# qiaozhijian/VCR-Net

Measured on AMD Instinct MI355X. Metric: point-cloud pairs/sec (N=1024, batch 16 per GPU), higher is better.
Workload: dtype f32; 1 GPU; BASELINE configs[1]: ModelNet40-like whole-to-whole registration, N=1024, batch=16 pairs per GPU, LPDNet(k=20)+Transformer+VcpTopK+SVD, iter=1, fp32; synthetic object clouds with the reference's transform recipe; LPD-pretrained emb_nn + seeded Transformer weights; num_points=1024, batch_per_gpu=16, global_batch=16, k=20, iters=1, parallelism=dp1 (pairs sharded per rank), entry_point=vcrnet_amd.module.vcrnetIter(net, src, tgt, iter) -> vcr_vcrnet_iter_f32

## Files before the change

### include/vcr_hip.h

```cpp
#ifndef VCR_HIP_H
#define VCR_HIP_H

#include <stddef.h>
#include <stdint.h>

#ifdef __cplusplus
extern "C" {
#endif

#define VCR_OK 0
#define VCR_EINVAL (-1)
#define VCR_EWORKSPACE (-2)
#define VCR_EUNSUPPORTED (-3)

typedef void* vcr_stream_t;

const char* vcr_strerror(int code);
#define VCR_ABI_VERSION 27
int vcr_abi_version(void);

typedef struct {
  const float* x_cf; int B, N;
  const float* w1; const float* b1;
  const float* w2; const float* b2;
  float* xyz4; float* feat64; float* sq64;
  const float* x_cf2; int B2;
  const float* pq_w; const float* pq_b; float* pq; int ldpq;
  float* feat64t;
} vcr_pointwise_args;
int vcr_pointwise_f32(const vcr_pointwise_args*, vcr_stream_t);

int vcr_rows4_f32(const float* x_cf, float* xyz4, int B, int N, vcr_stream_t);
int vcr_rows4_pq_f32(const float* x_cf, float* xyz4, int B, int N, const float* wpq, int ldw, const float* bpq, int C,
                     float* pq, int ldpq, vcr_stream_t);

typedef struct {
  uint32_t struct_bytes;
  const float* x; int ldx;
  const float* sq;
  int B, N, C, k;
  int32_t* idx;
  int32_t* tie_scratch; int tie_cap;
  int waves;
  int tie_zeroed;
  int tie_defer;
  void* tie_work; size_t tie_work_bytes;
  int tie_inline;
  const float* xt;
  const int32_t* perm; const float* xp; const float* sqp;
  const float* cen; const float* cen_sq; const float* cen_rad; const float* cen_sqmax;
  const int32_t* ord_ok;
} vcr_knn_args;

typedef struct {
  const float* xyz4;
  const float* feat_t; int ldf; const float* sq;
  int B, N;
  int32_t* perm; float* xyz4_p; float* cen4; float* cen4_rad; float* cen4_sqmax;
  float* feat_p; float* sq_p; float* cen64; float* cen64_sq; float* cen64_rad; float* cen64_sqmax;
  int32_t* ord_ok; float* ord_stat; float guard_ratio;
} vcr_knn_order_args;
int vcr_knn_order_f32(const vcr_knn_order_args*, vcr_stream_t);
int vcr_knn_f32(const vcr_knn_args*, vcr_stream_t);
size_t vcr_knn_tie_work_bytes(int N);
size_t vcr_knn_tie_slot_bytes(int B, int N);
int vcr_knn_ties_inline(const vcr_knn_args*);
int vcr_knn_ties_f32(const vcr_knn_args* a, const vcr_knn_args* b, vcr_stream_t);
int vcr_knn_pair_f32(const vcr_knn_args* a64, const vcr_knn_args* a3, vcr_stream_t);

typedef struct {
  const float* x; int ldx;
  const float* w;
  const float* bias;
  const float* residual; int ldr;
  float* y; int ldy;
  int M, N, K;
  int relu;
  const float* ln_stats_in; int ln_nseg; const float* ln_colsum; float ln_eps;
  float* stats_out;
  float* segmax_out; int ld_segmax; int seg_k;
  int variant;
} vcr_linear_args;
enum {
  VCR_LINEAR_REGSTAGE = 4, VCR_LINEAR_BK32 = 8, VCR_LINEAR_MFMA16 = 16, VCR_LINEAR_BK16 = 64, VCR_LINEAR_MFMA32 = 1024,
  VCR_LINEAR_ROWS96 = 2048, VCR_LINEAR_ROWS128 = 4096, VCR_LINEAR_ROWS64 = 8192, VCR_LINEAR_ROWS32 = 16384
};
int vcr_linear_f32(const vcr_linear_args*, vcr_stream_t);
int vcr_linear_config(const vcr_linear_args*);
int vcr_linear_pair_f32(const vcr_linear_args* a, const vcr_linear_args* b, vcr_stream_t);

int vcr_fold_layernorm_f32(const float* w, const float* bias, const float* ln_a, const float* ln_b, int N, int K,
                           float* w_out, float* colsum, float* bias_out, vcr_stream_t);

int vcr_split_bf16x3_f32(const float* x, void* planes, size_t n, vcr_stream_t);
int vcr_linear_bf16x3_f32(const vcr_linear_args*, const void* w_planes, vcr_stream_t);

typedef struct {
  const float* x; int ldx; const float* a; const float* b; float eps;
  const float* residual; int ldr;
  float* y; int ldy; int M, C;
  const float* xyz4; float* side4;
} vcr_layernorm_args;
int vcr_layernorm_f32(const vcr_layernorm_args*, vcr_stream_t);

typedef struct {
  const float* x; int ldx; int M, C; float scale; float* y; int ldy;
  const float* xyz4; float* side4;
} vcr_rowside_args;
int vcr_rowside_f32(const vcr_rowside_args*, vcr_stream_t);

typedef struct {
  const float* pq; int ldpq; const int32_t* idx; int k; int M; int n_per_cloud;
  const float* w2; const float* b2;
  float* x1; int ldx1; float* x2; int ldx2;
} vcr_edgeconv_args;
int vcr_edgeconv_f32(const vcr_edgeconv_args*, vcr_stream_t);
int vcr_edgeconv_bf16x3_f32(const vcr_edgeconv_args*, vcr_stream_t);

typedef struct {
  const float* pq; int ldpq; int C; const int32_t* idx; int k; int M; int n_per_cloud;
  float* y; int ldy;
  int variant;
  const int32_t* order;
} vcr_gathermax_args;
int vcr_gathermax_f32(const vcr_gathermax_args*, vcr_stream_t);

typedef struct {
  const float* pq; int ldpq; int C; const int32_t* idx; int k; int M; int n_per_cloud; float* h; int ldh;
  float* ymax; int ldymax; int zero_to;
} vcr_edgerows_args;
int vcr_edgerows_f32(const vcr_edgerows_args*, vcr_stream_t);
typedef struct {
  const float* pq; int ldpq; const int32_t* idx; int k; int M; int n_per_cloud;
  const float *w2, *b2, *w3, *b3, *w4, *b4;
  float* out; int ldo;
} vcr_edgechain_args;
int vcr_edgechain_f32(const vcr_edgechain_args*, vcr_stream_t);
typedef struct {
  const float* x; int ldx; int M, k, C; float* y; int ldy;
} vcr_segmax_args;
int vcr_segmax_f32(const vcr_segmax_args*, vcr_stream_t);

typedef struct {
  const float* q; int ldq; const float* k; int ldk; const float* v; int ldv;
  float* out; int ldo;
  int nbatch, heads, nq, nk; float scale; int kv_batch_shift;
  const uint8_t* key_keep; float* rowstat;
  float* score_out; int ld_score;
  int ngroups; long q_group_stride, k_group_stride, v_group_stride, out_group_stride;
  const int32_t* key_index; int nk_src;
  float* split_work; long split_work_floats;
  int variant;
  int plan_nbatch;
} vcr_sdpa_args;
#define VCR_SDPA_MAX_SPLIT 4
int vcr_sdpa_f32(const vcr_sdpa_args*, vcr_stream_t);
int vcr_sdpa_bf16x3_f32(const vcr_sdpa_args*, vcr_stream_t);

typedef struct {
  const float* score; int ld; int nbatch, heads, nq, nk;
  const float* rowstat; int q_batch_shift; float* mass;
} vcr_keymass_args;
int vcr_keymass_f32(const vcr_keymass_args*, vcr_stream_t);

typedef struct {
  const float* q; int ldq; const float* k; int ldk; const float* qside4; const float* kside4;
  float* corr4; int nbatch, nq, nk, E; int mode; float scale;
  float* split_work;
  long split_work_floats;
} vcr_softcorr_args;
int vcr_softcorr_f32(const vcr_softcorr_args*, vcr_stream_t);

typedef struct {
  const float* own; int ld_own; const float* str; int ld_str;
  const float* own_side4; const float* str_side4;
  int nbatch, n_own, n_str, E; int score; float scale; int str_batch_shift; int op;
  float* corr4; float* stat2; int32_t* argmax;
  const float* str_stat2; long str_stat_batch_stride; float* mass; int accumulate;
  float* score_out; int ld_score;
  int variant;
  float* split_work; long split_work_floats;
} vcr_pairscore_args;
#define VCR_PAIRSCORE_MAX_SPLIT 4
int vcr_pairscore_f32(const vcr_pairscore_args*, vcr_stream_t);

typedef struct {
  const float* score; int ld; int nbatch, n_rows, n_cols;
  const float* row_stat2; float* col_stat2; float* col_mass; float* row_mass;
} vcr_scoremass_args;
int vcr_scoremass_f32(const vcr_scoremass_args*, vcr_stream_t);

typedef struct {
  const float* values; int nbatch, n, K; int32_t* order; uint8_t* mask;
  int largest;
  int stride;
} vcr_rankselect_args;
int vcr_rankselect_f32(const vcr_rankselect_args*, vcr_stream_t);

typedef struct {
  const float* in; int ld_in; int n_in; const int32_t* idx; int nbatch, n_out, C; float* out; int ld_out;
  const int32_t* via; int n_via;
} vcr_gather_args;
int vcr_gather_rows_f32(const vcr_gather_args*, vcr_stream_t);

typedef struct {
  const float* src; int lds; const float* corr; int ldc; int B, K;
  float* R; float* t; float* R_ba; float* t_ba; float* H;
} vcr_rigid_svd_args;
int vcr_rigid_svd_f32(const vcr_rigid_svd_args*, vcr_stream_t);

typedef struct {
  const float* src4; const float* dst4; int B, N, M; int max_iterations; float tolerance;
  float* final4; float* R; float* t; float* R_ba; float* t_ba; int* iterations;
} vcr_icp_args;
size_t vcr_icp_workspace_bytes(int B, int N);
int vcr_icp_f32(const vcr_icp_args*, void* workspace, size_t workspace_bytes, vcr_stream_t);

typedef struct {
  const float* cloud; int P;
  const double* R_ab; const double* t_ab;
  const int32_t* pick; const int32_t* perm_src; const int32_t* perm_tgt;
  int B, N, keep;
  float* src_cf; float* tgt_cf;
} vcr_make_pairs_args;
int vcr_make_pairs_f32(const vcr_make_pairs_args*, vcr_stream_t);

typedef struct {
  uint32_t struct_bytes;
  const float* xyz_cf; long cloud_stride;
  int B, N, npoint;
  const int32_t* start;
  int32_t* idx;
  float* out_cf;
  int variant;
} vcr_fps_args;
int vcr_fps_f32(const vcr_fps_args*, vcr_stream_t);
int vcr_fps_form(const vcr_fps_args*, int* form, int* points_per_thread);

typedef struct {
  const float *ln_a, *ln_b;
} vcr_norm_w;
typedef struct {
  const float *wqkv, *bqkv;
  const float *wq, *bq, *wkv, *bkv;
  const float *wo, *bo;
} vcr_mha_w;
typedef struct {
  const float *w1, *b1, *w2, *b2;
} vcr_ffn_w;
typedef struct {
  uint32_t struct_bytes;
  const float *c1_w, *c1_b, *c2_w, *c2_b;
  const float *dg1_wpq, *dg1_bpq;
  const float *dg2_w, *dg2_b;
  const float *sn1_wpq, *sn1_bpq;
  const float *c3_w, *c3_b;
  vcr_norm_w enc_ln0, enc_ln1, enc_norm, dec_ln0, dec_ln1, dec_ln2, dec_norm;
  vcr_mha_w enc_self, dec_self, dec_cross;
  vcr_ffn_w enc_ffn, dec_ffn;
  int E, F, heads, k;
  int has_pointer;
  int head_mode;
  int linear_mode;
  struct {
    const void *dg1_pq, *sn1_pq, *c3, *enc_qkv, *enc_wo, *enc_ffn1, *enc_ffn2, *dec_qkv, *dec_self_wo, *dec_cross_q,
               *dec_cross_kv, *dec_cross_wo, *dec_ffn1, *dec_ffn2;
    const void* encdec_qkv;
  } split;
  struct vcr_folded { const float *w, *colsum, *bias; } fold_enc_qkv, fold_enc_ffn1, fold_dec_qkv, fold_dec_cross_q,
      fold_dec_cross_kv, fold_dec_ffn1;
  struct vcr_folded fold_encdec_qkv;
  int partial;
  double overlap2;
  int emb_kind;
  struct {
    const float *c1_wpq, *c1_bpq, *c2_w, *c2_b, *c3_w, *c3_b, *c4_w, *c4_b, *c5_w, *c5_b;
  } dgcnn;
  struct {
    const float *c3_w, *c3_b, *c4_w, *c4_b, *c5_w, *c5_b;
  } pointnet;
  const float *att_w0, *att_b0, *att_w1, *att_b1;
  int cycle;
  int linear_mfma;
  int linear_bk;
  int linear_bm;
  int knn_waves;
  int xscore_limit_mb;
  int sdpa_variant;
  int iter_reuse;
  int workspace_flat;
} vcr_vcrnet_weights;

typedef struct {
  const float* src_cf; const float* tgt_cf;
  int B, N;
  float* corr4;
  float* src4;
  float* R_ab; float* t_ab; float* R_ba; float* t_ba;
  float* emb_out;
  const int32_t *force_keys, *force_sel_src, *force_sel_tgt, *force_argmax, *force_pairs;
  int32_t *out_keys, *out_sel_src, *out_sel_tgt, *out_argmax, *out_pairs;
} vcr_vcrnet_io;

size_t vcr_vcrnet_workspace_bytes(const vcr_vcrnet_weights*, int B, int N);
size_t vcr_vcrnet_iter_workspace_bytes(const vcr_vcrnet_weights*, int B, int N, int iters);
int vcr_vcrnet_pairs(const vcr_vcrnet_weights*, int N);
int vcr_vcrnet_forward_f32(const vcr_vcrnet_weights*, const vcr_vcrnet_io*, void* workspace,
                           size_t workspace_bytes, vcr_stream_t);

#define VCR_TRACE_MAX 256
typedef struct {
  void** events; int capacity; int count;
  const char* names[VCR_TRACE_MAX];
} vcr_trace;
int vcr_vcrnet_forward_traced_f32(const vcr_vcrnet_weights*, const vcr_vcrnet_io*, void* workspace,
                                  size_t workspace_bytes, vcr_stream_t, vcr_trace*);

int vcr_vcrnet_iter_f32(const vcr_vcrnet_weights*, const vcr_vcrnet_io*, int iters, void* workspace,
                        size_t workspace_bytes, vcr_stream_t, vcr_trace* trace);

typedef struct {
  const float* R_i; const float* t_i;
  int B, N;
  const float* in_cf; float* out_cf;
  int compose;
  float* R_f; float* t_f;
  float* R_ba; float* t_ba;
} vcr_pose_step_args;
int vcr_pose_step_f32(const vcr_pose_step_args*, vcr_stream_t);

int vcr_event_create(void** ev);
int vcr_event_destroy(void* ev);
int vcr_event_record(void* ev, vcr_stream_t stream);
int vcr_event_elapsed_ms(void* start, void* stop, float* ms);

#ifdef __cplusplus
}
#endif
#endif
```

### vcr-net_amd/csrc/edgeconv.hip

```cpp
#include "edge_group.h"
#include "vcr_internal.h"

namespace {

constexpr int HP = 132;

__global__ __launch_bounds__(256, 2) void edgeconv_dg_kernel(vcr_edgeconv_args p) {
  __shared__ __attribute__((aligned(16))) float Hs[2][32][HP];
  const int lane = threadIdx.x & 63, w = threadIdx.x >> 6;
  const int half = lane >> 5, l31 = lane & 31;
  const int rs = lane >> 3, cg = lane & 7;
  const int ch = 32 * w + 4 * cg;

  f32x4 wf[16];
#pragma unroll
  for (int g = 0; g < 16; ++g) wf[g] = ld4(p.w2 + (size_t)(32 * w + l31) * 128 + 8 * g + 4 * half);
  const float bias2 = p.b2[32 * w + l31];

  const int row_tiles = (p.k + 31) / 32;
  const xcd_slice_t sl = xcd_slice(p.M);
  if (sl.count == 0) return;
  const int my_pts = sl.count;
  const int n_items = my_pts * row_tiles;

// ... 222 lines not shown
    for (int t = 0; t < 5; ++t) {
      const float* hcol = &Hs[cur][rowp][colc];
      const float* hrow = &Hs[cur][l31][4 * half];
      f32x16 acc = {0};
      f32x4 af[3];
      float xv[3];
#pragma unroll
      for (int g = 0; g < FRAG_AHEAD; ++g) { af[g] = ld4(hrow + 8 * g); xv[g] = hcol[2 * g * HP]; }
      __builtin_amdgcn_sched_barrier(0);
#pragma unroll
      for (int g = 0; g < 16; ++g) {
        if (g + FRAG_AHEAD < 16) {
          af[(g + FRAG_AHEAD) % 3] = ld4(hrow + 8 * (g + FRAG_AHEAD));
          xv[(g + FRAG_AHEAD) % 3] = hcol[2 * (g + FRAG_AHEAD) * HP];
        }
#pragma unroll
        for (int e = 0; e < 4; ++e) acc = mfma32(af[g % 3][e], wf[g][e], acc);
        cm[(32 * t + 2 * g) / KE] = fmaxf(cm[(32 * t + 2 * g) / KE], xv[g % 3]);
        if (t > 0) edge_fold<KE>(accp[g], t - 1, g, half, VCR_NEG_INF, pm);
        if (g < 4) load_row1(t < 4 ? grp : grp_n, (t + 1) % 5, g);
        else if (g < 8) load_idx1(t < 3 ? grp : grp_n, (t + 2) % 5, g - 4, nbn);
        else if (g >= 10 && g < 14) commit1(cur ^ 1, g - 10);
        __builtin_amdgcn_sched_barrier(0);
      }
#pragma unroll
      for (int i = 0; i < 4; ++i) nb[i] = nbn[i];
      if (t == 4) {
#pragma unroll
        for (int r = 0; r < 16; ++r) edge_fold<KE>(acc[r], 4, r, half, VCR_NEG_INF, pm);
#pragma unroll
        for (int q = 0; q < G; ++q) {
          x2half[half][q][32 * w + l31] = pm[q];
          x1half[rowp][q][colc] = cm[q];
        }
        lds_barrier();
        for (int i = threadIdx.x; i < G * 32; i += 256) {
          const int q = i >> 5, c4 = (i & 31) * 4, pt = grp * G + q;
          if (pt < p.M) {
            const f32x4 lo = ld4(&x1half[0][q][c4]), hi = ld4(&x1half[1][q][c4]);
            st4(p.x1 + (size_t)pt * p.ldx1 + c4, max4(lo, hi));
            const f32x4 a0 = ld4(&x2half[0][q][c4]), a1 = ld4(&x2half[1][q][c4]);
            st4(p.x2 + (size_t)pt * p.ldx2 + c4,
                f32x4{fmaxf(fmaxf(a0[0], a1[0]) + bias4[0], 0.f), fmaxf(fmaxf(a0[1], a1[1]) + bias4[1], 0.f),
                      fmaxf(fmaxf(a0[2], a1[2]) + bias4[2], 0.f), fmaxf(fmaxf(a0[3], a1[3]) + bias4[3], 0.f)});
          }
        }
      }
      accp = acc;
      lds_barrier();
      cur ^= 1;
    }
  }
}

__global__ __launch_bounds__(256) void gathermax_kernel(vcr_gathermax_args p) {
  const int lane = threadIdx.x & 63;
  int pt = xcd_chunk((int)blockIdx.x, (int)gridDim.x) * 4 + (threadIdx.x >> 6);
  if (pt >= p.M) return;
  const int c = lane * 4;
  if (c >= p.C) return;
  const int base = (pt / p.n_per_cloud) * p.n_per_cloud;
  if (p.order) pt = base + p.order[pt];
  const int32_t* id = p.idx + (size_t)pt * p.k;
  f32x4 m;
  int j;
  if (p.k == 20 || p.k == 40) {
    f32x4 a[20];
#pragma unroll
    for (int u = 0; u < 20; ++u) a[u] = ld4(p.pq + (size_t)(base + id[u]) * p.ldpq + c);
    m = a[0];
#pragma unroll
    for (int u = 1; u < 20; ++u) m = max4(m, a[u]);
    j = 20;
    if (p.k == 40) {
#pragma unroll
      for (int u = 0; u < 20; ++u) a[u] = ld4(p.pq + (size_t)(base + id[20 + u]) * p.ldpq + c);
#pragma unroll
      for (int u = 0; u < 20; ++u) m = max4(m, a[u]);
      j = 40;
    }
  } else {
    m = ld4(p.pq + (size_t)(base + id[0]) * p.ldpq + c);
    j = 1;
  }
  for (; j + 3 < p.k; j += 4) {
    const f32x4 a0 = ld4(p.pq + (size_t)(base + id[j]) * p.ldpq + c);
    const f32x4 a1 = ld4(p.pq + (size_t)(base + id[j + 1]) * p.ldpq + c);
    const f32x4 a2 = ld4(p.pq + (size_t)(base + id[j + 2]) * p.ldpq + c);
    const f32x4 a3 = ld4(p.pq + (size_t)(base + id[j + 3]) * p.ldpq + c);
#pragma unroll
    for (int i = 0; i < 4; ++i) m[i] = fmaxf(fmaxf(fmaxf(m[i], a0[i]), fmaxf(a1[i], a2[i])), a3[i]);
  }
  for (; j < p.k; ++j) {
    const f32x4 a0 = ld4(p.pq + (size_t)(base + id[j]) * p.ldpq + c);
    m = max4(m, a0);
  }
  const f32x4 q = ld4(p.pq + (size_t)pt * p.ldpq + p.C + c);
  f32x4 y;
#pragma unroll
  for (int i = 0; i < 4; ++i) y[i] = fmaxf(m[i] + q[i], 0.f);
  st4(p.y + (size_t)pt * p.ldy + c, y);
}

constexpr __host__ __device__ int gm_pitch(int cs) { return cs + 4; }
template <int CS, int KQ>
__global__ __launch_bounds__(512, 1) void gathermax_lds_kernel(vcr_gathermax_args p, int slices) {
  constexpr int PITCH = gm_pitch(CS), LPP = CS / 4;
  extern __shared__ __attribute__((aligned(16))) float gm_smem[];
  const int t = threadIdx.x;
  const int cloud = (int)blockIdx.x / slices, sl = (int)blockIdx.x - cloud * slices;
  const int N = p.n_per_cloud, c0 = sl * CS;
  const size_t base = (size_t)cloud * N;
  const int sub = t % LPP, c4 = 4 * sub;
  if (c0 + c4 >= p.C) {
    __syncthreads();
    return;
  }
  for (int n = t / LPP; n < N; n += 512 / LPP)
    st4(&gm_smem[n * PITCH + c4], ld4(p.pq + (base + n) * p.ldpq + c0 + c4));
  __syncthreads();
  using i32x4 = __attribute__((ext_vector_type(4))) int;
  i32x4 idn[KQ];
  f32x4 qn;
  auto fetch = [&](int n) {
    const i32x4* id = reinterpret_cast<const i32x4*>(p.idx + (base + n) * (4 * KQ));
#pragma unroll
    for (int u = 0; u < KQ; ++u) idn[u] = id[u];
    qn = ld4(p.pq + (base + n) * p.ldpq + p.C + c0 + c4);
  };
  int n = t / LPP;
  if (n < N) fetch(n);
  for (; n < N; n += 512 / LPP) {
    i32x4 idc[KQ];
#pragma unroll
    for (int u = 0; u < KQ; ++u) idc[u] = idn[u];
    const f32x4 q = qn;
    if (n + 512 / LPP < N) fetch(n + 512 / LPP);
    f32x4 m = ld4(&gm_smem[idc[0][0] * PITCH + c4]);
#pragma unroll
    for (int u = 0; u < KQ; ++u)
#pragma unroll
      for (int e = (u == 0 ? 1 : 0); e < 4; ++e) {
        const f32x4 a0 = ld4(&gm_smem[idc[u][e] * PITCH + c4]);
#pragma unroll
        for (int i = 0; i < 4; ++i) m[i] = fmaxf(m[i], a0[i]);
      }
    f32x4 y;
#pragma unroll
    for (int i = 0; i < 4; ++i) y[i] = fmaxf(m[i] + q[i], 0.f);
    st4(p.y + (base + n) * p.ldy + c0 + c4, y);
  }
}

constexpr int EDGECONV_PIPE = 1;
constexpr int EDGECONV_WG_PER_CU = 2;
constexpr int EDGECONV_PADDED_MAX_GRID = 2048;
constexpr int EDGECONV_BF16X3_MAX_GRID = 1024;

constexpr size_t GM_LDS_BUDGET_AUTO32 = 150 * 1024;
constexpr size_t GM_LDS_MAX = 160 * 1024;
constexpr int GM_MIN_WORKGROUPS = 192;
inline size_t gm_lds_bytes(int n_per_cloud, int cs) { return (size_t)n_per_cloud * gm_pitch(cs) * 4; }

enum GathermaxForm { GM_L2, GM_LDS };
struct GathermaxPlan { GathermaxForm form; int cs, slices; size_t lds; int grid; };

int gathermax_check(const vcr_gathermax_args* a) {
  if (!a || !a->pq || !a->idx || !a->y) return VCR_EINVAL;
  if (a->M <= 0 || a->k <= 0 || a->C <= 0 || a->C > 256 || (a->C & 3)) return VCR_EINVAL;
  if (a->n_per_cloud <= 0 || (a->M % a->n_per_cloud) || a->ldpq < 2 * a->C || (a->ldpq & 3) || (a->ldy & 3)) return VCR_EINVAL;
  return VCR_OK;
}

int gathermax_plan(const vcr_gathermax_args& a, GathermaxPlan* p) {
  const int N = a.n_per_cloud, clouds = a.M / N;
  const bool aligned = !(((uintptr_t)a.pq | (uintptr_t)a.y | (uintptr_t)a.idx) & 15) && edge_group_points(a.k) != 0;
  int cs = 0;
  if (a.variant == 0) {
    if (aligned && (long)clouds * ((a.C + 31) / 32) >= GM_MIN_WORKGROUPS)
      cs = gm_lds_bytes(N, 32) <= GM_LDS_BUDGET_AUTO32 ? 32 : gm_lds_bytes(N, 16) <= GM_LDS_MAX ? 16 : 0;
  } else if (a.variant == 32 || a.variant == 16 || a.variant == 8) {
    if (!aligned || gm_lds_bytes(N, a.variant) > GM_LDS_MAX) return VCR_EUNSUPPORTED;
    cs = a.variant;
  } else if (a.variant != 1) {
    return VCR_EINVAL;
  }
  const int slices = cs ? (a.C + cs - 1) / cs : 0;
  *p = cs ? GathermaxPlan{GM_LDS, cs, slices, gm_lds_bytes(N, cs), clouds * slices} : GathermaxPlan{GM_L2, 0, 0, 0, (a.M + 3) / 4};
  return VCR_OK;
}

template <int KQ>
int gathermax_lds_run(const GathermaxPlan& p, const vcr_gathermax_args& a, hipStream_t s) {
  const dim3 grid(p.grid), block(512);
  if (p.cs == 32) return vcr_launch<gathermax_lds_kernel<32, KQ>>(grid, block, p.lds, s, a, p.slices);
  if (p.cs == 16) return vcr_launch<gathermax_lds_kernel<16, KQ>>(grid, block, p.lds, s, a, p.slices);
  return vcr_launch<gathermax_lds_kernel<8, KQ>>(grid, block, p.lds, s, a, p.slices);
}

}

int edgeconv_check(const vcr_edgeconv_args* a, bool bf16x3) {
  if (!a || !a->pq || !a->idx || !a->w2 || !a->b2 || !a->x1 || !a->x2) return VCR_EINVAL;
  if (a->M <= 0 || a->k <= 0 || a->k > 64 || a->n_per_cloud <= 0 || (a->M % a->n_per_cloud)) return VCR_EINVAL;
  if (a->ldpq < 256 || (a->ldpq & 3) || (a->ldx1 & 3) || a->ldx1 < 128 || a->ldx2 < 128) return VCR_EINVAL;
  if (!bf16x3) return VCR_OK;
  if (((uintptr_t)a->w2 | (uintptr_t)a->pq | (uintptr_t)a->x1) & 15) return VCR_EINVAL;
  return edge_group_points(a->k) ? VCR_OK : VCR_EUNSUPPORTED;
}

EdgeconvPlan edgeconv_plan(const vcr_edgeconv_args& a, bool bf16x3) {
  const int G = edge_group_points(a.k);
  if (!G) return {EdgeconvForm::PADDED, a.M < EDGECONV_PADDED_MAX_GRID ? a.M : EDGECONV_PADDED_MAX_GRID};
  const int ngroups = (a.M + G - 1) / G;
  if (bf16x3) return {EdgeconvForm::BF16X3, ngroups < EDGECONV_BF16X3_MAX_GRID ? ngroups : EDGECONV_BF16X3_MAX_GRID};
  const int slots = EDGECONV_WG_PER_CU * vcr_cu_count();
  const bool al16 = !(a.ldx2 & 3) && !(((uintptr_t)a.x1 | (uintptr_t)a.x2 | (uintptr_t)a.b2) & 15);
  return {EDGECONV_PIPE && al16 ? EdgeconvForm::PIPE : EdgeconvForm::PACKED, ngroups < slots ? ngroups : slots};
}

extern "C" int vcr_edgeconv_f32(const vcr_edgeconv_args* a, vcr_stream_t stream) {
  vcr_stream_scope bound(stream);
  if (const int rc = edgeconv_check(a, false)) return rc;
  const EdgeconvPlan p = edgeconv_plan(*a, false);
  const dim3 grid(p.grid), block(256);
  const hipStream_t s = (hipStream_t)stream;
  if (p.form == EdgeconvForm::PADDED) return vcr_launch<edgeconv_dg_kernel>(grid, block, 0, s, *a);
  if (p.form == EdgeconvForm::PIPE)
    return a->k == 20 ? vcr_launch<edgeconv_dg_pipe_kernel<20>>(grid, block, 0, s, *a) : vcr_launch<edgeconv_dg_pipe_kernel<40>>(grid, block, 0, s, *a);
  return a->k == 20 ? vcr_launch<edgeconv_dg_packed_kernel<20>>(grid, block, 0, s, *a) : vcr_launch<edgeconv_dg_packed_kernel<40>>(grid, block, 0, s, *a);
}

extern "C" int vcr_gathermax_f32(const vcr_gathermax_args* a, vcr_stream_t stream) {
  GathermaxPlan p;
  if (const int rc = gathermax_check(a)) return rc;
  if (const int rc = gathermax_plan(*a, &p)) return rc;
  const hipStream_t s = (hipStream_t)stream;
  if (p.form == GM_L2) return vcr_launch<gathermax_kernel>(dim3(p.grid), dim3(256), 0, s, *a);
  return a->k == 20 ? gathermax_lds_run<5>(p, *a, s) : gathermax_lds_run<10>(p, *a, s);
}

extern "C" int vcr_edgeconv_forms_(const vcr_edgeconv_args* a, int bf16x3, int* form, int* grid) {
  if (const int rc = edgeconv_check(a, bf16x3 != 0)) return rc;
  const EdgeconvPlan p = edgeconv_plan(*a, bf16x3 != 0);
  *form = (int)p.form; *grid = p.grid;
  return VCR_OK;
}
extern "C" int vcr_gathermax_forms_(const vcr_gathermax_args* a, int* form, int* cs, int* grid, int* lds_bytes) {
  GathermaxPlan p;
  if (const int rc = gathermax_check(a)) return rc;
  if (const int rc = gathermax_plan(*a, &p)) return rc;
  *form = (int)p.form; *cs = p.cs; *grid = p.grid; *lds_bytes = (int)p.lds;
  return VCR_OK;
}
```

### vcr-net_amd/csrc/forward.hip

```cpp
#include "edge_group.h"
#include "vcr_internal.h"

namespace {

enum Launch : int {
  STEM, KNN, TIE_REPLAY, EDGECONV, SN1_PQ, GATHERMAX, CONV3,
  ENCDEC_QKV, ENCDEC_SELF, WO_PAIR, FFN1_CROSS_Q, MERGED_ENC_FFN2,
  ENC_QKV = ENCDEC_QKV, ENC_SELF, ENC_WO, ENC_FFN1, ENC_FFN2, DEC_QKV, DEC_SELF, DEC_SELF_WO, DEC_CROSS_Q,
  DEC_CROSS_KV, CROSS_ATT, DEC_CROSS_WO, DEC_FFN1, DEC_FFN2, DEC_NORM, HEAD, HEAD2,
  END = HEAD2
};
static_assert(MERGED_ENC_FFN2 < DEC_CROSS_KV, "the merged first sublayers end in front of the positions both forms share");

struct Plan {
  struct Req { void** slot; size_t bytes; int birth, death; size_t off; };
  static constexpr int MAXR = 96;
  Req r[MAXR];
  int n = 0;
  bool overflow = false;
  bool flat = false;
  template <class T> void want(T*& field, size_t count, int birth, int death) {
    field = nullptr;
    if (count == 0) return;
    if (flat) { birth = 0; death = 1 << 30; }
    if (n >= MAXR) { overflow = true; return; }
    r[n++] = Req{reinterpret_cast<void**>(&field), (count * sizeof(T) + 255) & ~(size_t)255, birth, death, 0};
  }
  size_t solve(unsigned char* base) {
    int order[MAXR];
    for (int i = 0; i < n; ++i) order[i] = i;
    for (int i = 1; i < n; ++i) {
      const int x = order[i];
      int j = i - 1;
      while (j >= 0 && r[order[j]].bytes < r[x].bytes) { order[j + 1] = order[j]; --j; }
      order[j + 1] = x;
    }
    size_t total = 0;
    for (int oi = 0; oi < n; ++oi) {
      Req& q = r[order[oi]];
      size_t off = 0;
      for (bool moved = true; moved;) {
        moved = false;
        for (int pj = 0; pj < oi; ++pj) {
          const Req& p = r[order[pj]];
          if (p.death < q.birth || q.death < p.birth) continue;
          if (off < p.off + p.bytes && p.off < off + q.bytes) { off = p.off + p.bytes; moved = true; }
        }
      }
      q.off = off;
      if (off + q.bytes > total) total = off + q.bytes;
    }
    for (int i = 0; i < n; ++i) *r[i].slot = base + r[i].off;
    return total;
  }
};

struct Ws {
  float *xyz4, *feat64, *sq64, *pq1, *cat, *pq3, *emb;
  int32_t *idx1, *idx3, *ties;
  unsigned char* tie_work[2]; size_t tie_work_each;
  float* feat64t;
  float *feat_p, *xyz4_p, *cen64, *cen4, *sq_p, *c64_sq, *c64_rad, *c64_max, *c4_rad, *c4_max;
  int32_t *perm, *ord_ok;
  float *qkv, *att, *attx, *e1, *e2, *hid, *d1, *d2, *d3, *qc, *kvc, *embf, *side4, *csplit, *asplit;
  float* corr_ba;
  long asplit_floats;
  float *st_emb, *st_e1, *st_e2, *st_d1, *st_d2;
  float *rowstat, *keymass; uint8_t* keep;
  float* xsplit;
  float* xscore;
  int32_t* xorder;
  float *rstat, *cstat, *colsum, *rowsum, *score;
  float* rsplit;
  int32_t *sel_s, *sel_t, *amax, *pick;
  float *so_e, *to_e, *so_s, *to_s, *peak;
  float *eh1, *eh2, *eh3;
  float *cur_cf, *Ri, *ti, *Rb, *tb;
  size_t bytes;
};
inline size_t tgt_cache_floats(int B, int N, int E) { return (size_t)2 * B * N * 5 * E; }

inline int overlap_k1(int N, double o2) { return (int)((double)N * 0.84 * o2); }
inline int overlap_k2(int N, double o2) { return (int)((double)overlap_k1(N, o2) * 0.52 * o2); }

constexpr int KNN_ORDERED_MIN_N = 2048;
inline int merged_encdec(const vcr_vcrnet_weights* W) {
  return W->has_pointer == 1 && (W->linear_mode == 0 || W->split.encdec_qkv) && W->fold_encdec_qkv.w && W->fold_encdec_qkv.colsum &&
         W->fold_encdec_qkv.bias;
}

Ws carve(void* base, const vcr_vcrnet_weights* W, int B, int N, int cus, int pass = 0) {
  const int k = W->k, E = W->E, F = W->F, heads = W->heads;
  const bool merged = merged_encdec(W) != 0;
  Plan pl;
  pl.flat = W->workspace_flat != 0;
  const size_t M = (size_t)2 * B * N;
  Ws w{};
  pl.want(w.xyz4, M * 4, STEM, END);   pl.want(w.feat64, M * 64, STEM, EDGECONV);   pl.want(w.sq64, M, STEM, TIE_REPLAY);
  pl.want(w.idx1, M * k, KNN, EDGECONV);   pl.want(w.idx3, M * k, KNN, GATHERMAX);   pl.want(w.ties, 2 * (1 + M), STEM, TIE_REPLAY);
  {
    const size_t slots = vcr_knn_tie_slot_bytes(2 * B, N);
    w.tie_work_each = (k > 20 && slots <= ((size_t)1 << 30)) ? slots : vcr_knn_tie_work_bytes(N);
    w.tie_work_each = (w.tie_work_each + 255) & ~(size_t)255;
  }
  pl.want(w.tie_work[0], w.tie_work_each ? 2 * w.tie_work_each : 0, KNN, TIE_REPLAY);
  pl.want(w.pq1, M * 256, STEM, SN1_PQ);   pl.want(w.cat, M * 512, EDGECONV, CONV3);   pl.want(w.pq3, M * 512, SN1_PQ, GATHERMAX);
  pl.want(w.emb, M * E, STEM, DEC_NORM);
  pl.want(w.qkv, M * 3 * E * (merged ? 2 : 1), merged ? ENCDEC_QKV : ENC_QKV, merged ? ENCDEC_SELF : DEC_SELF);
  pl.want(w.att, M * E * (merged ? 2 : 1), merged ? ENCDEC_SELF : ENC_SELF, merged ? WO_PAIR : DEC_SELF_WO);
  pl.want(w.e1, M * E, merged ? WO_PAIR : ENC_WO, merged ? MERGED_ENC_FFN2 : ENC_FFN2);
  pl.want(w.e2, M * E, merged ? MERGED_ENC_FFN2 : ENC_FFN2, DEC_CROSS_KV);
  pl.want(w.hid, M * F, merged ? FFN1_CROSS_Q : ENC_FFN1, DEC_FFN2);
  pl.want(w.d1, M * E, merged ? WO_PAIR : DEC_SELF_WO, DEC_CROSS_WO);
  pl.want(w.qc, M * E, merged ? FFN1_CROSS_Q : DEC_CROSS_Q, CROSS_ATT);   pl.want(w.kvc, M * 2 * E, DEC_CROSS_KV, CROSS_ATT);
  pl.want(w.attx, M * E, CROSS_ATT, DEC_CROSS_WO);
  pl.want(w.d2, M * E, DEC_CROSS_WO, END);
  pl.want(w.d3, M * E, DEC_FFN2, END);
  pl.want(w.embf, M * E, DEC_NORM, END);  pl.want(w.side4, M * 4, DEC_NORM, END);
  pl.want(w.csplit, VCR_PAIRSCORE_MAX_SPLIT * (M / 2) * 8, HEAD, END);
  pl.want(w.corr_ba, (size_t)B * N * 4, HEAD2, END);
  w.asplit_floats = vcr_sdpa_split_floats_(2 * M, heads, E, 2L * B, N, cus);
  pl.want(w.asplit, (size_t)w.asplit_floats, merged ? ENCDEC_SELF : ENC_SELF, CROSS_ATT);
  const size_t sn = M * (E / 64) * 2;
  pl.want(w.st_emb, sn, CONV3, DEC_QKV);
  pl.want(w.st_e1, sn, merged ? WO_PAIR : ENC_WO, merged ? FFN1_CROSS_Q : ENC_FFN1);
  pl.want(w.st_e2, sn, merged ? MERGED_ENC_FFN2 : ENC_FFN2, DEC_CROSS_KV);
  pl.want(w.st_d1, sn, merged ? WO_PAIR : DEC_SELF_WO, merged ? FFN1_CROSS_Q : DEC_CROSS_Q);
  pl.want(w.st_d2, sn, DEC_CROSS_WO, DEC_FFN1);
  const size_t K1 = (size_t)overlap_k1(N, W->overlap2), K2 = (size_t)overlap_k2(N, W->overlap2), B1 = (size_t)B;
  if (W->partial) {
    pl.want(w.rowstat, M * heads * 2, CROSS_ATT, CROSS_ATT); pl.want(w.keymass, M, CROSS_ATT, CROSS_ATT); pl.want(w.keep, M, CROSS_ATT, CROSS_ATT);
    pl.want(w.xsplit, VCR_SDPA_MAX_SPLIT * M * heads * 2, CROSS_ATT, CROSS_ATT);
    const size_t xs = M * heads * ((N + 31) & ~31);
    const int xmb = W->xscore_limit_mb;
    const size_t xlimit = xmb > 0 ? (size_t)xmb << 20 : xmb < 0 ? 0 : (size_t)4 << 30;
    pl.want(w.xscore, xs * 4 <= xlimit ? xs : 0, CROSS_ATT, CROSS_ATT);
    pl.want(w.xorder, M, CROSS_ATT, CROSS_ATT);
    pl.want(w.rstat, B1 * N * 2, HEAD, END); pl.want(w.cstat, B1 * N * 2, HEAD, END);
    pl.want(w.rsplit, VCR_PAIRSCORE_MAX_SPLIT * B1 * N * 2, HEAD, END);
    pl.want(w.rowsum, 2 * B1 * N, HEAD, END);
    pl.want(w.score, B1 * N * ((N + 31) & ~31), HEAD, END);
    pl.want(w.sel_s, 2 * B1 * K1, HEAD, END);
    pl.want(w.amax, B1 * K1, HEAD, END);     pl.want(w.pick, B1 * (K2 ? K2 : 1), HEAD, END);
    pl.want(w.so_e, 2 * B1 * K1 * E, HEAD, END);
    pl.want(w.so_s, 2 * B1 * K1 * 4, HEAD, END);
    pl.want(w.peak, B1 * K1 * 2, HEAD, END);
  }
  if (W->emb_kind == 1 && k != 20 && k != 40) {
    const size_t Mk = M * k;
    pl.want(w.eh1, Mk * 64, EDGECONV, GATHERMAX); pl.want(w.eh2, Mk * 64, EDGECONV, GATHERMAX);
    pl.want(w.eh3, Mk * 128, EDGECONV, GATHERMAX);
  }
  pl.want(w.cur_cf, (size_t)B * 3 * N, STEM, END);
  pl.want(w.Ri, (size_t)B * 9, STEM, END); pl.want(w.ti, (size_t)B * 3, STEM, END);
  pl.want(w.Rb, (size_t)B * 9, STEM, END); pl.want(w.tb, (size_t)B * 3, STEM, END);
  w.bytes = pl.solve(reinterpret_cast<unsigned char*>(base)) + 256;
  bool bad = pl.overflow;
  w.tie_work[1] = w.tie_work[0] ? w.tie_work[0] + w.tie_work_each : nullptr;
  if (W->partial) {
    w.colsum = w.rowsum + B1 * N;
    w.sel_t = w.sel_s + B1 * K1;
    w.to_e = w.so_e + B1 * K1 * E;
    w.to_s = w.so_s + B1 * K1 * 4;
  }
  if (pass != 0) {
    float* c = reinterpret_cast<float*>(static_cast<unsigned char*>(base) + w.bytes);
    w.emb = c;   c += M * E;
    w.d1 = c;    c += M * E;
    w.qc = c;    c += M * E;
    w.kvc = c;
  }
  w.feat64t = E >= 64 ? w.emb : nullptr;
  {
    const size_t T = (size_t)2 * B * ((N + 15) / 16);
    float* p = w.emb + M * 64;
    auto take = [&p](size_t n) { float* q = p; p += n; return q; };
    w.feat_p = take(M * 64);  w.xyz4_p = take(M * 4);  w.cen64 = take(T * 64);  w.cen4 = take(T * 4);  w.sq_p = take(M);
    w.perm = reinterpret_cast<int32_t*>(take(M));
    w.c64_sq = take(T);  w.c64_rad = take(T);  w.c64_max = take(T);  w.c4_rad = take(T);  w.c4_max = take(T);
    w.ord_ok = reinterpret_cast<int32_t*>(take(2 * B));
    if (pass != 0 && p > w.emb + B1 * N * E) bad = true;
  }
  if (bad) w.bytes = ~(size_t)0;
  return w;
}

__global__ __launch_bounds__(256) void zero_i32_kernel(int32_t* p, long n) {
  const long i = (long)blockIdx.x * 256 + threadIdx.x;
  if (i < n) p[i] = 0;
}

struct Runner {
  hipStream_t stream; vcr_trace* tr; int rc = 0;
  int shape_rows = 0;
  int plan_nbatch = 0;
  bool sdpa_split = false;
  float* pv_split = nullptr; long pv_split_floats = 0;
  int linear_variant = 0;
  int sdpa_variant = 0;
  vcr_knn_args deferred[2];
  int n_deferred = 0;

  void pin_shape(vcr_linear_args& a, vcr_linear_args* b = nullptr, int full_rows = 0) {
    const int fm = full_rows ? full_rows : shape_rows;
    if (!shape_rows || a.M >= fm || (a.variant & (VCR_LINEAR_MFMA16 | VCR_LINEAR_MFMA32))) return;
    vcr_linear_args fa = a, fb = b ? *b : a;
    fa.M = fm; fb.M = fm;
    int form_a[8], form_b[8];
    if (vcr_linear_forms_(&fa, b ? &fb : nullptr, nullptr, form_a, form_b) != VCR_OK) return;
    a.variant |= form_a[3] == 16 ? VCR_LINEAR_MFMA16 : VCR_LINEAR_MFMA32;
    if (b) b->variant |= form_b[3] == 16 ? VCR_LINEAR_MFMA16 : VCR_LINEAR_MFMA32;
  }
  bool ok(int r) { if (rc == 0 && r != 0) rc = r; return rc == 0; }
  template <class F> bool run(const char* name, F&& launch) {
    if (rc) return false;
    if (tr) {
      if (tr->count < VCR_TRACE_MAX) tr->names[tr->count] = name;
      if (tr->events && tr->count < tr->capacity) (void)hipEventRecord((hipEvent_t)tr->events[tr->count], stream);
      ++tr->count;
    }
    return ok(launch());
  }
  void finish() {
    if (tr && tr->events && tr->count < tr->capacity) (void)hipEventRecord((hipEvent_t)tr->events[tr->count], stream);
  }

  vcr_linear_args linear_args(const float* x, int ldx, const float* w, const float* b, float* y, int ldy, int M, int N, int K,
                              int relu, const float* res = nullptr, int ldr = 0, const float* ln_stats = nullptr,
                              const float* ln_colsum = nullptr, float* stats_out = nullptr) {
    vcr_linear_args a{x, ldx, w, b, res, ldr, y, ldy, M, N, K, relu};
    if (ln_stats) { a.ln_stats_in = ln_stats; a.ln_nseg = K / 64; a.ln_colsum = ln_colsum; a.ln_eps = 1e-6f; }
    a.stats_out = stats_out;
    a.variant = linear_variant;
    return a;
  }
  struct Lin { const char* name; vcr_linear_args a; const void* split; };
  bool linear(const Lin& l) {
    return run(l.name, [&] {
      vcr_linear_args a = l.a;
      if (!l.split) pin_shape(a);
      return l.split ? vcr_linear_bf16x3_f32(&a, l.split, stream) : vcr_linear_f32(&a, stream);
    });
  }
  bool linear(const char* nm, const float* x, int ldx, const float* w, const void* wsplit, const float* b, float* y,
              int ldy, int M, int N, int K, int relu, const float* res = nullptr, int ldr = 0,
              const float* ln_stats = nullptr, const float* ln_colsum = nullptr, float* stats_out = nullptr) {
    return linear({nm, linear_args(x, ldx, w, b, y, ldy, M, N, K, relu, res, ldr, ln_stats, ln_colsum, stats_out), wsplit});
  }
  bool linear2(const char* nm, vcr_linear_args a, vcr_linear_args b) {
    return run(nm, [&] {
      pin_shape(a, &b);
      return vcr_linear_pair_f32(&a, &b, stream);
    });
  }
  bool norm(const char* nm, const float* x, const vcr_norm_w& n, float* y, int M, int E,
            const float* res = nullptr, const float* xyz4 = nullptr, float* side4 = nullptr) {
    return run(nm, [&] {
      vcr_layernorm_args a{x, E, n.ln_a, n.ln_b, 1e-6f, res, E, y, E, M, E, xyz4, side4};
      return vcr_layernorm_f32(&a, stream);
// ... 44 lines not shown
      a64.tie_zeroed = a3.tie_zeroed = 1;
      a64.tie_defer = a3.tie_defer = 1;
      n_deferred = 0;
      int inl64 = 0, inl3 = 0;
      (void)vcr_knn_forms_(&a64, &a3, nullptr, &inl64, &inl3);
      if (!inl64) deferred[n_deferred++] = a64;
      if (!inl3) deferred[n_deferred++] = a3;
      return vcr_knn_pair_f32(&a64, &a3, stream);
    });
  }
  void knn_ties() {
    if (n_deferred) run("knn:ties", [&] { return vcr_knn_ties_f32(&deferred[0], n_deferred == 2 ? &deferred[1] : nullptr, stream); });
    n_deferred = 0;
  }
  void copy_idx(const char* nm, int32_t* dst, const int32_t* src, size_t n) {
    run(nm, [&] { return vcr_copy_d2d(dst, src, n * sizeof(int32_t), stream); });
  }

  void cross_attention(const vcr_vcrnet_weights* W, const vcr_vcrnet_io* io, const Ws& w, int B, int N) {
    const int E = W->E, H = W->heads, nb = 2 * B, dk = E / H;
    const uint8_t* keep = nullptr;
    if (W->partial) {
      const int nkeep = (int)((double)N * W->overlap2);
      if (io->force_keys) {
        if (sdpa_split && W->F < 2 * E) { ok(VCR_EUNSUPPORTED); return; }
        copy_idx("select:dec.cross.keys.forced", w.xorder, io->force_keys, (size_t)nb * nkeep);
      } else if (w.xscore) {
        const int ldS = (N + 31) & ~31;
        sdpa("sdpa:dec.cross.stats", w.qc, E, w.kvc, 2 * E, nullptr, 0, nullptr, 0, nb, H, N, N, B, nullptr, w.rowstat,
             w.xscore, ldS, 1, 0, 0, w.xsplit, (long)VCR_SDPA_MAX_SPLIT * nb * H * N * 2);
        run("scoremass:dec.cross.keymass", [&] {
          vcr_keymass_args a{w.xscore, ldS, nb, H, N, N, w.rowstat, B, w.keymass};
          return vcr_keymass_f32(&a, stream);
        });
      } else {
        sdpa("sdpa:dec.cross.stats", w.qc, E, w.kvc, 2 * E, nullptr, 0, nullptr, 0, nb, H, N, N, B, nullptr, w.rowstat, nullptr, 0,
             1, 0, 0, w.xsplit, (long)VCR_SDPA_MAX_SPLIT * nb * H * N * 2);
        for (int h = 0; h < H; ++h) {
          vcr_pairscore_args a{};
          a.own = w.kvc + h * dk; a.ld_own = 2 * E; a.str = w.qc + h * dk; a.ld_str = E;
          a.nbatch = nb; a.n_own = N; a.n_str = N; a.E = dk; a.score = 1; a.scale = 1.0f / sqrtf((float)dk);
          a.str_batch_shift = B; a.op = 2; a.str_stat2 = w.rowstat + (size_t)h * N * 2;
          a.str_stat_batch_stride = (long)H * N * 2; a.mass = w.keymass; a.accumulate = h > 0;
          pairscore("pairscore:dec.cross.keymass", a);
        }
      }
      if (!io->force_keys) rank("select:dec.cross.keys", w.keymass, 1, nb, N, nkeep, w.xorder, w.keep, 1);
      if (io->out_keys) copy_idx("select:dec.cross.keys.out", io->out_keys, w.xorder, (size_t)nb * nkeep);
      vcr_sdpa_args xa{w.qc, E, w.kvc, 2 * E, w.kvc + E, 2 * E, w.attx, E, nb, H, N, nkeep, 1.0f / sqrtf(128.f), B};
      xa.key_index = w.xorder; xa.nk_src = N;
      if (!sdpa_split && vcr_sdpa_forms_(&xa, nullptr, nullptr) == VCR_OK) {
        run("sdpa:dec.cross", [&] { return vcr_sdpa_f32(&xa, stream); });
        return;
      }
      if (W->F >= 2 * E) {
        gather("select:gather.kv", w.kvc, 2 * E, N, w.xorder, nb, nkeep, 2 * E, w.hid);
        sdpa("sdpa:dec.cross", w.qc, E, w.hid, 2 * E, w.hid + E, 2 * E, w.attx, E, nb, H, N, nkeep, B);
        return;
      }
      keep = w.keep;
    }
    sdpa("sdpa:dec.cross", w.qc, E, w.kvc, 2 * E, w.kvc + E, 2 * E, w.attx, E, nb, H, N, N, B, keep);
  }

  void partial_head(const vcr_vcrnet_weights* W, const vcr_vcrnet_io* io, const Ws& w, int B, int N) {
    const int E = W->E, M1 = B * N;
    const int K1 = overlap_k1(N, W->overlap2), K2 = overlap_k2(N, W->overlap2);
    const float *se = w.embf, *te = w.embf + (size_t)M1 * E, *ss = w.side4, *ts = w.side4 + (size_t)M1 * 4;
    auto stats = [&](const char* nm, const float* own, const float* str, const float* os, const float* sd, int no,
                     int ns, float* stat2, int32_t* amax, float* score_out, int ld_score) {
      vcr_pairscore_args a{};
      a.own = own; a.ld_own = E; a.str = str; a.ld_str = E; a.own_side4 = os; a.str_side4 = sd;
      a.nbatch = B; a.n_own = no; a.n_str = ns; a.E = E; a.score = 0; a.scale = 1.f; a.op = 1;
      a.stat2 = stat2; a.argmax = amax; a.score_out = score_out; a.ld_score = ld_score;
      a.split_work = amax ? nullptr : w.rsplit;
      a.split_work_floats = amax ? 0 : (long)VCR_PAIRSCORE_MAX_SPLIT * B * N * 2;
      pairscore(nm, a);
    };
    const int ldS = (N + 31) & ~31;
    const bool forced_sets = io->force_sel_src && io->force_sel_tgt;
    if (!forced_sets) {
      stats("pairscore:head.scores", se, te, ss, ts, N, N, w.rstat, nullptr, w.score, ldS);
      run("scoremass:head", [&] {
        vcr_scoremass_args a{w.score, ldS, B, N, N, w.rstat, w.cstat, w.colsum, w.rowsum};
        return vcr_scoremass_f32(&a, stream);
      });
    }
    if (forced_sets) {
      copy_idx("select:head.tgt.forced", w.sel_t, io->force_sel_tgt, (size_t)B * K1);
      copy_idx("select:head.src.forced", w.sel_s, io->force_sel_src, (size_t)B * K1);
    } else {
      rank("select:head.src+tgt", w.rowsum, 1, 2 * B, N, K1, w.sel_s, nullptr, 1);
    }
    if (io->out_sel_tgt) copy_idx("select:head.tgt.out", io->out_sel_tgt, w.sel_t, (size_t)B * K1);
    if (io->out_sel_src) copy_idx("select:head.src.out", io->out_sel_src, w.sel_s, (size_t)B * K1);
    gather("select:gather.emb", se, E, N, w.sel_s, 2 * B, K1, E, w.so_e);
    gather("select:gather.xyz", ss, 4, N, w.sel_s, 2 * B, K1, 4, w.so_s);
    if (!(io->force_argmax && io->force_pairs))
      stats("pairscore:head.copair", w.so_e, w.to_e, w.so_s, w.to_s, K1, K1, w.peak, w.amax, nullptr, 0);
    if (io->force_argmax) copy_idx("select:head.argmax.forced", w.amax, io->force_argmax, (size_t)B * K1);
    if (io->force_pairs) copy_idx("select:head.pairs.forced", w.pick, io->force_pairs, (size_t)B * K2);
    else rank("select:head.pairs", w.peak + 1, 2, B, K1, K2, w.pick, nullptr, 0);
    if (io->out_argmax) copy_idx("select:head.argmax.out", io->out_argmax, w.amax, (size_t)B * K1);
    if (io->out_pairs) copy_idx("select:head.pairs.out", io->out_pairs, w.pick, (size_t)B * K2);
    gather("select:gather.srcK", w.so_s, 4, K1, w.pick, B, K2, 4, io->src4);
    gather("select:gather.corrK", w.to_s, 4, K1, w.pick, B, K2, 4, io->corr4, w.amax, K1);
    run("rigid_svd:ab", [&] {
      vcr_rigid_svd_args a{io->src4, 4, io->corr4, 4, B, K2, io->R_ab, io->t_ab, io->R_ba, io->t_ba, nullptr};
      return vcr_rigid_svd_f32(&a, stream);
    });
  }
};

int forward_impl(const vcr_vcrnet_weights* W, const vcr_vcrnet_io* io, void* workspace, size_t ws_bytes,
                 vcr_stream_t stream, vcr_trace* tr, bool last = true, int pass = 0) {
  if (!W || !io || !workspace || !io->src_cf || !io->tgt_cf || !io->corr4 || !io->src4 || !io->R_ab || !io->t_ab)
    return VCR_EINVAL;
  const int B = io->B, N = io->N, E = W->E, F = W->F, k = W->k;
  if (B <= 0 || N <= 0 || E != 512 || W->heads * 128 != E || k <= 0 || k + 1 > N) return VCR_EINVAL;
  if (k > 62 || N > 65535) return VCR_EUNSUPPORTED;
  if (W->emb_kind < 0 || W->emb_kind > 2) return VCR_EINVAL;
  if (W->emb_kind == 2 && !(W->c1_w && W->c1_b && W->c2_w && W->c2_b && W->pointnet.c3_w && W->pointnet.c3_b && W->pointnet.c4_w &&
                            W->pointnet.c4_b && W->pointnet.c5_w && W->pointnet.c5_b))
    return VCR_EINVAL;
  if (W->has_pointer == 1 && (F % 128)) return VCR_EINVAL;
  if (W->has_pointer == 1 &&
      !(W->fold_enc_qkv.w && W->fold_enc_ffn1.w && W->fold_dec_qkv.w && W->fold_dec_cross_q.w &&
        W->fold_dec_cross_kv.w && W->fold_dec_ffn1.w))
    return VCR_EINVAL;
  if (((uintptr_t)workspace) & 255) return VCR_EINVAL;
  if (W->head_mode < 0 || W->head_mode > 2 || W->linear_mode < 0 || W->linear_mode > 2) return VCR_EINVAL;
  for (int ms : {W->linear_mfma, W->linear_bk})
    if (ms != 0 && ms != 16 && ms != 32) return VCR_EINVAL;
  if ((W->linear_bm != 0 && W->linear_bm != 96 && W->linear_bm != 128) || (W->linear_bm == 96 && W->linear_mfma == 32)) return VCR_EINVAL;
  if (W->knn_waves != 0 && W->knn_waves != 1 && W->knn_waves != 8) return VCR_EINVAL;
  if (W->partial) {
    if (W->has_pointer != 1 || (W->cycle && W->head_mode == 0)) return VCR_EUNSUPPORTED;
    if (!(W->overlap2 > 0.0 && W->overlap2 <= 1.0) || (int)((double)N * W->overlap2) < 1) return VCR_EINVAL;
    if (W->head_mode == 0 && overlap_k2(N, W->overlap2) < 3) return VCR_EINVAL;
  }
  if (!W->partial && (io->force_keys || io->force_sel_src || io->force_sel_tgt || io->force_argmax || io->force_pairs))
    return VCR_EINVAL;
  if ((io->force_sel_src != nullptr) != (io->force_sel_tgt != nullptr)) return VCR_EINVAL;
  Ws w = carve(workspace, W, B, N, vcr_cu_count(), pass);
  if (ws_bytes < w.bytes) return VCR_EWORKSPACE;
  if (pass != 0 && ws_bytes < w.bytes + tgt_cache_floats(B, N, E) * sizeof(float)) return VCR_EINVAL;
  const int M1 = B * N, M2 = 2 * M1;
  const bool half = pass == 2;
  const int Bq = half ? B : 2 * B, Mq = half ? M1 : M2;
#define NM(site) (half ? site "@src" : site)
  Runner R{(hipStream_t)stream, tr};
  R.shape_rows = half ? M2 : 0;
  R.plan_nbatch = half ? 2 * B : 0;
  hipLaunchKernelGGL(zero_i32_kernel, dim3((unsigned)((M2 + 2 + 255) / 256)), dim3(256), 0, R.stream, w.ties, (long)(M2 + 2));
  R.ok(VCR_LAUNCH_RC());
#define SP(site) (W->linear_mode != 0 ? W->split.site : nullptr)
  R.sdpa_split = W->linear_mode == 2;
  R.sdpa_variant = W->sdpa_variant;
  R.pv_split = w.asplit; R.pv_split_floats = w.asplit_floats;
  R.linear_variant = (W->linear_mfma == 16 ? VCR_LINEAR_MFMA16 : W->linear_mfma == 32 ? VCR_LINEAR_MFMA32 : 0) |
                     (W->linear_bk == 16 ? VCR_LINEAR_BK16 : W->linear_bk == 32 ? VCR_LINEAR_BK32 : 0) |
                     (W->linear_bm == 96 ? VCR_LINEAR_ROWS96 : W->linear_bm == 128 ? VCR_LINEAR_ROWS128 : 0);

  const float* stats_for_ln = W->has_pointer == 1 ? w.st_emb : nullptr;
  if (W->emb_kind == 1) {
    for (int c = 0; c < (half ? 1 : 2); ++c) {
      R.run(c ? "pointwise:tgt" : "pointwise:src", [&] {
        return vcr_rows4_pq_f32(c ? io->tgt_cf : io->src_cf, w.xyz4 + (size_t)c * M1 * 4, B, N, W->dgcnn.c1_wpq, 32,
                                W->dgcnn.c1_bpq, 128, w.pq1 + (size_t)c * M1 * 128, 128, R.stream);
      });
    }
    {
      vcr_knn_args a3{(uint32_t)sizeof(vcr_knn_args), w.xyz4, 4, nullptr, Bq, N, 4, k, w.idx3, w.ties + 1 + M2, M2};
      a3.tie_work = w.tie_work[0]; a3.tie_work_bytes = w.tie_work_each;
      R.knn(NM("knn:xyz"), a3);
    }
    const int Mk = Mq * k;
    auto conv_max = [&](const char* nm, const float* x, int K, const float* wt, const float* bias, float* y, int Nout,
                        int col) {
      R.run(nm, [&] {
        vcr_linear_args a{x, K, wt, bias, nullptr, 0, y, Nout, Mk, Nout, K, 1};
        a.segmax_out = w.cat + col; a.ld_segmax = 512; a.seg_k = k;
        a.variant = R.linear_variant;
        R.pin_shape(a, nullptr, M2 * k);
        return vcr_linear_f32(&a, R.stream);
      });
    };
    if (edge_group_points(k)) {
      R.run(NM("edgeconv:dg_chain"), [&] {
        vcr_edgechain_args a{w.pq1, 128, w.idx3, k, Mq, N, W->dgcnn.c2_w, W->dgcnn.c2_b, W->dgcnn.c3_w, W->dgcnn.c3_b,
                             W->dgcnn.c4_w, W->dgcnn.c4_b, w.cat, 512};
        return vcr_edgechain_f32(&a, R.stream);
      });
    } else {
      R.run(NM("gathermax:dg_c1"), [&] {
        vcr_edgerows_args a{w.pq1, 128, 64, w.idx3, k, Mq, N, w.eh1, 64, w.cat, 512, 512};
        return vcr_edgerows_f32(&a, R.stream);
      });
      conv_max(NM("linear:dg_c2"), w.eh1, 64, W->dgcnn.c2_w, W->dgcnn.c2_b, w.eh2, 64, 64);
      conv_max(NM("linear:dg_c3"), w.eh2, 64, W->dgcnn.c3_w, W->dgcnn.c3_b, w.eh3, 128, 128);
      conv_max(NM("linear:dg_c4"), w.eh3, 128, W->dgcnn.c4_w, W->dgcnn.c4_b, nullptr, 256, 256);
    }
    R.linear(NM("linear:conv3"), w.cat, 512, W->dgcnn.c5_w, nullptr, W->dgcnn.c5_b, w.emb, E, Mq, E, 512, 1, nullptr, 0, nullptr,
             nullptr, const_cast<float*>(stats_for_ln));
  } else if (W->emb_kind == 2) {
    R.run(NM("pointwise:src+tgt"), [&] {
      vcr_pointwise_args a{io->src_cf, B, N, W->c1_w, W->c1_b, W->c2_w, W->c2_b, w.xyz4, w.feat64, w.sq64, half ? nullptr : io->tgt_cf,
                           half ? 0 : B};
      return vcr_pointwise_f32(&a, R.stream);
    });
    R.linear(NM("linear:pn_c3"), w.feat64, 64, W->pointnet.c3_w, nullptr, W->pointnet.c3_b, w.pq1, 64, Mq, 64, 64, 1);
    R.linear(NM("linear:pn_c4"), w.pq1, 64, W->pointnet.c4_w, nullptr, W->pointnet.c4_b, w.cat, 128, Mq, 128, 64, 1);
    R.linear(NM("linear:pn_c5"), w.cat, 128, W->pointnet.c5_w, nullptr, W->pointnet.c5_b, w.emb, E, Mq, E, 128, 1, nullptr, 0, nullptr,
             nullptr, const_cast<float*>(stats_for_ln));
  } else {
  const bool pq_fused = W->linear_mode == 0;
  R.run(pq_fused ? NM("pointwise:src+tgt+dg1_pq") : NM("pointwise:src+tgt"), [&] {
    vcr_pointwise_args a{io->src_cf, B, N, W->c1_w, W->c1_b, W->c2_w, W->c2_b, w.xyz4, w.feat64, w.sq64, half ? nullptr : io->tgt_cf,
                         half ? 0 : B};
    if (pq_fused) { a.pq_w = W->dg1_wpq; a.pq_b = W->dg1_bpq; a.pq = w.pq1; a.ldpq = 256; }
    a.feat64t = w.feat64t;
    return vcr_pointwise_f32(&a, R.stream);
  });
  const int32_t* rank_perm = nullptr;
  {
    vcr_knn_args a64{(uint32_t)sizeof(vcr_knn_args), w.feat64, 64, w.sq64, Bq, N, 64, k, w.idx1, w.ties, M2, W->knn_waves};
    vcr_knn_args a3{(uint32_t)sizeof(vcr_knn_args), w.xyz4, 4, nullptr, Bq, N, 4, k, w.idx3, w.ties + 1 + M2, M2};
    a64.tie_work = w.tie_work[0]; a3.tie_work = w.tie_work[1];
    a64.tie_work_bytes = a3.tie_work_bytes = w.tie_work_each;
    a64.xt = w.feat64t;
    int pair_ordered = 0;
    if (R.rc == 0 && W->E >= 256 && N >= KNN_ORDERED_MIN_N && N <= 8192 && (k == 20 || k == 40) && W->knn_waves == 0 &&
        vcr_knn_forms_(&a64, &a3, &pair_ordered, nullptr, nullptr) == VCR_OK && pair_ordered) {
      R.run(NM("knn:rank"), [&] {
        vcr_knn_order_args o{w.xyz4, w.feat64t, 64, w.sq64, Bq, N, w.perm, w.xyz4_p, w.cen4, w.c4_rad, w.c4_max, w.feat_p, w.sq_p,
                             w.cen64, w.c64_sq, w.c64_rad, w.c64_max, w.ord_ok, nullptr, 0.f};
        return vcr_knn_order_f32(&o, R.stream);
      });
      a64.perm = a3.perm = w.perm;
      a64.ord_ok = w.ord_ok;
      rank_perm = w.perm;
      a64.xp = w.feat_p; a64.sqp = w.sq_p; a64.cen = w.cen64; a64.cen_sq = w.c64_sq; a64.cen_rad = w.c64_rad; a64.cen_sqmax = w.c64_max;
      a3.xp = w.xyz4_p; a3.cen = w.cen4; a3.cen_rad = w.c4_rad; a3.cen_sqmax = w.c4_max;
    }
    R.knn_pair(NM("knn:feat64+xyz"), a64, a3);
  }
  if (!pq_fused) R.linear(NM("linear:dg1_pq"), w.feat64, 64, W->dg1_wpq, SP(dg1_pq), W->dg1_bpq, w.pq1, 256, Mq, 256, 64, 0);
  R.knn_ties();
  R.run(NM("edgeconv:dg1_dg2"), [&] {
    vcr_edgeconv_args a{w.pq1, 256, w.idx1, k, Mq, N, W->dg2_w, W->dg2_b, w.cat, 512, w.cat + 128, 512};
    return W->linear_mode != 0 && edge_group_points(k) ? vcr_edgeconv_bf16x3_f32(&a, R.stream) : vcr_edgeconv_f32(&a, R.stream);
  });
  R.linear(NM("linear:sn1_pq"), w.cat + 128, 512, W->sn1_wpq, SP(sn1_pq), W->sn1_bpq, w.pq3, 512, Mq, 512, 128, 0);
  R.run(NM("gathermax:sn1"), [&] {
    vcr_gathermax_args a{w.pq3, 512, 256, w.idx3, k, Mq, N, w.cat + 256, 512};
    a.order = rank_perm;
    return vcr_gathermax_f32(&a, R.stream);
  });
  R.linear(NM("linear:conv3"), w.cat, 512, W->c3_w, SP(c3), W->c3_b, w.emb, E, Mq, E, 512, 1, nullptr, 0, nullptr, nullptr,
           W->has_pointer == 1 ? w.st_emb : nullptr);

  }
  if (W->has_pointer != 1) { R.shape_rows = 0; R.plan_nbatch = 0; }

  const float* head_emb = w.embf;
  if (W->has_pointer == 1) {
    const int H = W->heads;
    const bool merged = merged_encdec(W) != 0;
    const float* att_dec = merged ? w.att + (size_t)M2 * E : w.att;
    using Lin = Runner::Lin;
    const Lin enc_wo{NM("linear:enc.wo"), R.linear_args(w.att, E, W->enc_self.wo, W->enc_self.bo, w.e1, E, Mq, E, E, 0, w.emb, E,
                                                         nullptr, nullptr, w.st_e1), SP(enc_wo)};
    const Lin dec_self_wo{NM("linear:dec.self.wo"), R.linear_args(att_dec, E, W->dec_self.wo, W->dec_self.bo, w.d1, E, Mq, E, E, 0,
                                                                  w.emb, E, nullptr, nullptr, w.st_d1), SP(dec_self_wo)};
    const Lin enc_ffn1{NM("linear:enc.ffn1"), R.linear_args(w.e1, E, W->fold_enc_ffn1.w, W->fold_enc_ffn1.bias, w.hid, F, Mq, F, E, 1,
                                                            nullptr, 0, w.st_e1, W->fold_enc_ffn1.colsum), SP(enc_ffn1)};
    const Lin dec_cross_q{NM("linear:dec.cross.q"), R.linear_args(w.d1, E, W->fold_dec_cross_q.w, W->fold_dec_cross_q.bias, w.qc, E, Mq,
                                                                  E, E, 0, nullptr, 0, w.st_d1, W->fold_dec_cross_q.colsum),
                          SP(dec_cross_q)};
    const Lin enc_ffn2{NM("linear:enc.ffn2"), R.linear_args(w.hid, F, W->enc_ffn.w2, W->enc_ffn.b2, w.e2, E, Mq, E, F, 0, w.e1, E,
                                                            nullptr, nullptr, w.st_e2), SP(enc_ffn2)};
    if (merged) {
      R.linear(NM("linear:encdec.qkv"), w.emb, E, W->fold_encdec_qkv.w, SP(encdec_qkv), W->fold_encdec_qkv.bias, w.qkv, 6 * E, Mq, 6 * E, E, 0,
               nullptr, 0, w.st_emb, W->fold_encdec_qkv.colsum);
      R.sdpa(NM("sdpa:encdec.self"), w.qkv, 6 * E, w.qkv + E, 6 * E, w.qkv + 2 * E, 6 * E, w.att, E, Bq, H, N, N, 0, nullptr, nullptr,
             nullptr, 0, 2, 3 * E, (long)M2 * E);
      if (W->linear_mode != 0) {
        R.linear(enc_wo); R.linear(dec_self_wo); R.linear(enc_ffn1); R.linear(dec_cross_q); R.linear(enc_ffn2);
      } else {
        R.linear2(NM("linear:enc.wo+dec.self.wo"), enc_wo.a, dec_self_wo.a);
        R.linear2(NM("linear:enc.ffn1+dec.cross.q"), enc_ffn1.a, dec_cross_q.a);
        R.linear(enc_ffn2);
      }
    } else {
      R.linear(NM("linear:enc.qkv"), w.emb, E, W->fold_enc_qkv.w, SP(enc_qkv), W->fold_enc_qkv.bias, w.qkv, 3 * E, Mq, 3 * E, E, 0,
               nullptr, 0, w.st_emb, W->fold_enc_qkv.colsum);
      R.sdpa(NM("sdpa:enc.self"), w.qkv, 3 * E, w.qkv + E, 3 * E, w.qkv + 2 * E, 3 * E, w.att, E, Bq, H, N, N, 0);
      R.linear(enc_wo); R.linear(enc_ffn1); R.linear(enc_ffn2);
      R.linear(NM("linear:dec.qkv"), w.emb, E, W->fold_dec_qkv.w, SP(dec_qkv), W->fold_dec_qkv.bias, w.qkv, 3 * E, Mq, 3 * E, E, 0,
               nullptr, 0, w.st_emb, W->fold_dec_qkv.colsum);
      R.sdpa(NM("sdpa:dec.self"), w.qkv, 3 * E, w.qkv + E, 3 * E, w.qkv + 2 * E, 3 * E, w.att, E, Bq, H, N, N, 0);
      R.linear(dec_self_wo); R.linear(dec_cross_q);
    }
    R.linear(NM("linear:dec.cross.kv"), w.e2, E, W->fold_dec_cross_kv.w, SP(dec_cross_kv), W->fold_dec_cross_kv.bias, w.kvc, 2 * E, Mq, 2 * E, E, 0,
             nullptr, 0, w.st_e2, W->fold_dec_cross_kv.colsum);
    R.shape_rows = 0; R.plan_nbatch = 0;
    R.cross_attention(W, io, w, B, N);
    R.linear("linear:dec.cross.wo", w.attx, E, W->dec_cross.wo, SP(dec_cross_wo), W->dec_cross.bo, w.d2, E, M2, E, E, 0, w.d1, E,
             nullptr, nullptr, w.st_d2);
    R.linear("linear:dec.ffn1", w.d2, E, W->fold_dec_ffn1.w, SP(dec_ffn1), W->fold_dec_ffn1.bias, w.hid, F, M2, F, E, 1, nullptr, 0,
             w.st_d2, W->fold_dec_ffn1.colsum);
    R.linear("linear:dec.ffn2", w.hid, F, W->dec_ffn.w2, SP(dec_ffn2), W->dec_ffn.b2, w.d3, E, M2, E, F, 0, w.d2, E);
    R.norm("layernorm:dec.norm+res", w.d3, W->dec_norm, w.embf, M2, E, w.emb, w.xyz4, w.side4);
  } else {
    R.run("layernorm:rowside", [&] {
      vcr_rowside_args a{w.emb, E, M2, E, W->has_pointer == 2 ? 2.f : 1.f, w.embf, E, w.xyz4, w.side4};
      return vcr_rowside_f32(&a, R.stream);
    });
  }

  const bool hard_pairs = W->partial && W->head_mode == 0;
  const float* side = w.side4;
  if (W->head_mode == 2) {
    if (!W->att_w0 || !W->att_w1) return VCR_EINVAL;
    R.linear("linear:head.att.src", w.embf, E, W->att_w0, nullptr, W->att_b0, w.d3, E, M1, E, E, 0);
    R.linear("linear:head.att.tgt", w.embf + (size_t)M1 * E, E, W->att_w1, nullptr, W->att_b1, w.d3 + (size_t)M1 * E, E,
             M1, E, E, 0);
    R.run("layernorm:rowside.att", [&] {
      vcr_rowside_args a{w.d3, E, M2, E, 1.f, nullptr, E, w.xyz4, w.side4};
      return vcr_rowside_f32(&a, R.stream);
    });
    head_emb = w.d3;
  }
  auto soft_head = [&](const char* nm, size_t q0, size_t k0, float* corr) {
    R.run(nm, [&] {
      vcr_softcorr_args a{head_emb + q0 * E, E, head_emb + k0 * E, E, side + q0 * 4, side + k0 * 4,
                          corr, B, N, N, E, W->head_mode == 1 ? 1 : 0, 1.0f / sqrtf((float)E), w.csplit,
                          (long)VCR_PAIRSCORE_MAX_SPLIT * B * N * 8};
      return vcr_softcorr_f32(&a, R.stream);
    });
  };
  if (hard_pairs) {
    R.partial_head(W, io, w, B, N);
  } else {
    soft_head("softcorr:head", 0, (size_t)M1, io->corr4);
    R.run("rigid_svd:ab", [&] {
      const int c = vcr_copy_d2d(io->src4, w.xyz4, (size_t)M1 * 4 * sizeof(float), R.stream);
      vcr_rigid_svd_args a{w.xyz4, 4, io->corr4, 4, B, N, io->R_ab, io->t_ab, io->R_ba, io->t_ba, nullptr};
      const int s = vcr_rigid_svd_f32(&a, R.stream);
      return c ? c : s;
    });
    if (W->cycle) {
      if (!io->R_ba || !io->t_ba) return VCR_EINVAL;
      if (W->head_mode == 2) {
        R.linear("linear:head.att.ba.src", w.embf, E, W->att_w1, nullptr, W->att_b1, w.d2, E, M1, E, E, 0);
        R.linear("linear:head.att.ba.tgt", w.embf + (size_t)M1 * E, E, W->att_w0, nullptr, W->att_b0, w.d2 + (size_t)M1 * E,
                 E, M1, E, E, 0);
        R.run("layernorm:rowside.att.ba", [&] {
          vcr_rowside_args a{w.d2, E, M2, E, 1.f, nullptr, E, w.xyz4, w.side4};
          return vcr_rowside_f32(&a, R.stream);
        });
        head_emb = w.d2;
      }
      soft_head("softcorr:head.ba", (size_t)M1, 0, w.corr_ba);
      R.run("rigid_svd:ba", [&] {
        vcr_rigid_svd_args a{w.xyz4 + (size_t)M1 * 4, 4, w.corr_ba, 4, B, N, io->R_ba, io->t_ba, nullptr, nullptr, nullptr};
        return vcr_rigid_svd_f32(&a, R.stream);
      });
    }
  }
  if (R.rc == 0 && io->emb_out) R.ok(vcr_copy_d2d(io->emb_out, w.embf, (size_t)M2 * E * sizeof(float), R.stream));
  if (last) R.finish();
#undef SP
#undef NM
  return R.rc;
}

__global__ __launch_bounds__(256) void pose_step_kernel(const float* __restrict__ Ri, const float* __restrict__ ti,
                                                        const float* in_cf, float* out_cf, int N, int compose,
                                                        float* Rf, float* tf, float* Rba, float* tba) {
  const int b = blockIdx.y;
  float r[9], t[3];
  for (int i = 0; i < 9; ++i) r[i] = Ri[b * 9 + i];
  for (int i = 0; i < 3; ++i) t[i] = ti[b * 3 + i];
  if (out_cf) {
    const int n = blockIdx.x * 256 + threadIdx.x;
    if (n < N) {
      const float* p = in_cf + (size_t)b * 3 * N + n;
      const float x = p[0], y = p[N], z = p[2 * (size_t)N];
      float* o = out_cf + (size_t)b * 3 * N + n;
      for (int c = 0; c < 3; ++c) o[(size_t)c * N] = fmaf(r[c * 3 + 2], z, fmaf(r[c * 3 + 1], y, r[c * 3] * x)) + t[c];
    }
  }
  if (compose == 2 && blockIdx.x == 0 && threadIdx.x == 0) {
    for (int i = 0; i < 3; ++i) {
      for (int j = 0; j < 3; ++j) Rba[b * 9 + i * 3 + j] = r[j * 3 + i];
      tba[b * 3 + i] = -fmaf(r[6 + i], t[2], fmaf(r[3 + i], t[1], r[i] * t[0]));
    }
  } else if (compose && blockIdx.x == 0 && threadIdx.x == 0) {
    float f[9], g[3], nf[9], ng[3];
    for (int i = 0; i < 9; ++i) f[i] = Rf[b * 9 + i];
    for (int i = 0; i < 3; ++i) g[i] = tf[b * 3 + i];
    for (int i = 0; i < 3; ++i) {
      for (int j = 0; j < 3; ++j) nf[i * 3 + j] = fmaf(r[i * 3 + 2], f[6 + j], fmaf(r[i * 3 + 1], f[3 + j], r[i * 3] * f[j]));
      ng[i] = fmaf(r[i * 3 + 2], g[2], fmaf(r[i * 3 + 1], g[1], r[i * 3] * g[0])) + t[i];
    }
    for (int i = 0; i < 9; ++i) Rf[b * 9 + i] = nf[i];
    for (int i = 0; i < 3; ++i) tf[b * 3 + i] = ng[i];
    for (int i = 0; i < 3; ++i) {
      for (int j = 0; j < 3; ++j) Rba[b * 9 + i * 3 + j] = nf[j * 3 + i];
      tba[b * 3 + i] = -fmaf(nf[6 + i], ng[2], fmaf(nf[3 + i], ng[1], nf[i] * ng[0]));
    }
  }
}

}

static int weights_take(const vcr_vcrnet_weights* user, vcr_vcrnet_weights* mine) {
  return vcr_take_args(user, mine, offsetof(vcr_vcrnet_weights, fold_encdec_qkv));
}

extern "C" size_t vcr_vcrnet_workspace_bytes(const vcr_vcrnet_weights* UW, int B, int N) {
  vcr_vcrnet_weights Wn;
  const vcr_vcrnet_weights* W = &Wn;
  if (weights_take(UW, &Wn) || B <= 0 || N <= 0) return 0;
  return carve(nullptr, W, B, N, vcr_cu_count()).bytes;
}

static bool iter_reuse_applies(const vcr_vcrnet_weights* W, int iters) { return iters > 1 && W->iter_reuse != 1; }
extern "C" size_t vcr_vcrnet_iter_workspace_bytes(const vcr_vcrnet_weights* UW, int B, int N, int iters) {
  vcr_vcrnet_weights Wn;
  const vcr_vcrnet_weights* W = &Wn;
  if (weights_take(UW, &Wn) || B <= 0 || N <= 0 || iters < 1) return 0;
  const size_t base = carve(nullptr, W, B, N, vcr_cu_count()).bytes;
  return base + (iter_reuse_applies(W, iters) ? tgt_cache_floats(B, N, W->E) * sizeof(float) : 0);
}

extern "C" int vcr_vcrnet_pairs(const vcr_vcrnet_weights* UW, int N) {
  vcr_vcrnet_weights Wn;
  const vcr_vcrnet_weights* W = &Wn;
  if (weights_take(UW, &Wn) || N <= 0) return 0;
  return (W->partial && W->head_mode == 0) ? overlap_k2(N, W->overlap2) : N;
}

extern "C" int vcr_vcrnet_forward_f32(const vcr_vcrnet_weights* UW, const vcr_vcrnet_io* io, void* ws, size_t bytes,
                                      vcr_stream_t stream) {
  vcr_vcrnet_weights Wn;
  if (weights_take(UW, &Wn)) return VCR_EINVAL;
  return forward_impl(&Wn, io, ws, bytes, stream, nullptr);
}

extern "C" int vcr_vcrnet_forward_traced_f32(const vcr_vcrnet_weights* UW, const vcr_vcrnet_io* io, void* ws,
                                             size_t bytes, vcr_stream_t stream, vcr_trace* tr) {
  vcr_vcrnet_weights Wn;
  if (weights_take(UW, &Wn)) return VCR_EINVAL;
  if (tr) tr->count = 0;
  return forward_impl(&Wn, io, ws, bytes, stream, tr);
}

extern "C" int vcr_vcrnet_iter_f32(const vcr_vcrnet_weights* UW, const vcr_vcrnet_io* io, int iters, void* ws,
                                   size_t bytes, vcr_stream_t stream, vcr_trace* tr) {
  vcr_vcrnet_weights Wn;
  const vcr_vcrnet_weights* W = &Wn;
  if (weights_take(UW, &Wn)) return VCR_EINVAL;
  if (!W || !io || iters < 1 || !io->R_ba || !io->t_ba) return VCR_EINVAL;
  if (tr) tr->count = 0;
  const int B = io->B, N = io->N;
  if (B <= 0 || N <= 0) return VCR_EINVAL;
  if (iters == 1) {
    const int rc = forward_impl(W, io, ws, bytes, stream, tr, !W->cycle);
    if (rc || !W->cycle) return rc;
    Runner R{(hipStream_t)stream, tr};
    R.run("pose:inverse", [&] {
      hipLaunchKernelGGL(pose_step_kernel, dim3(1, B), dim3(64), 0, R.stream, io->R_ab, io->t_ab, nullptr, nullptr, N, 2, nullptr,
                         nullptr, io->R_ba, io->t_ba);
      return VCR_LAUNCH_RC();
    });
    R.finish();
    return R.rc;
  }
  const Ws w = carve(ws, W, B, N, vcr_cu_count());
  if (bytes < w.bytes) return VCR_EWORKSPACE;
  const bool reuse = iter_reuse_applies(W, iters) && bytes >= w.bytes + tgt_cache_floats(B, N, W->E) * sizeof(float);
  const size_t nkeys = W->partial ? (size_t)2 * B * (int)((double)N * W->overlap2) : 0;
  const size_t nsel = W->partial ? (size_t)B * overlap_k1(N, W->overlap2) : 0;
  const size_t npair = W->partial ? (size_t)B * overlap_k2(N, W->overlap2) : 0;
  for (int it = 0; it < iters; ++it) {
    vcr_vcrnet_io step = *io;
    if (it > 0) { step.src_cf = w.cur_cf; step.R_ab = w.Ri; step.t_ab = w.ti; step.R_ba = w.Rb; step.t_ba = w.tb; }
    if (it + 1 < iters) step.emb_out = nullptr;
    auto at = [it](auto* p, size_t n) { return p ? p + (size_t)it * n : p; };
    step.force_keys = at(io->force_keys, nkeys);       step.out_keys = at(io->out_keys, nkeys);
    step.force_sel_src = at(io->force_sel_src, nsel);  step.out_sel_src = at(io->out_sel_src, nsel);
    step.force_sel_tgt = at(io->force_sel_tgt, nsel);  step.out_sel_tgt = at(io->out_sel_tgt, nsel);
    step.force_argmax = at(io->force_argmax, nsel);    step.out_argmax = at(io->out_argmax, nsel);
    step.force_pairs = at(io->force_pairs, npair);     step.out_pairs = at(io->out_pairs, npair);
    const bool last = it + 1 == iters;
    const int rc = forward_impl(W, &step, ws, bytes, stream, tr, false, reuse ? (it == 0 ? 1 : 2) : 0);
    if (rc) return rc;
    if (last && it == 0) break;
    Runner R{(hipStream_t)stream, tr};
    R.run("pose:step", [&] {
      hipLaunchKernelGGL(pose_step_kernel, dim3((N + 255) / 256, B), dim3(256), 0, R.stream, step.R_ab, step.t_ab, step.src_cf,
// ... 49 lines not shown
```

### vcr-net_amd/csrc/pointwise.hip

```cpp
#include "common.h"

namespace {

constexpr int PTS = 64;

__global__ __launch_bounds__(256) void pointwise12_kernel(vcr_pointwise_args a) {
  __shared__ float w2t[64][64];
  __shared__ float h1s[PTS][65];
  __shared__ float w1s[64][4];
  __shared__ float b2s[64];
  const int t = threadIdx.x;
  {
    f32x4 wv[4];
#pragma unroll
    for (int u = 0; u < 4; ++u) wv[u] = ld4(a.w2 + 4 * (t + 256 * u));
#pragma unroll
    for (int u = 0; u < 4; ++u) {
      const int i = 4 * (t + 256 * u), c = i >> 6, k = i & 63;
#pragma unroll
      for (int e = 0; e < 4; ++e) w2t[k + e][c] = wv[u][e];
    }
  }
  if (t < 64) {
    w1s[t][0] = a.w1[t * 3 + 0]; w1s[t][1] = a.w1[t * 3 + 1]; w1s[t][2] = a.w1[t * 3 + 2];
    w1s[t][3] = a.b1[t]; b2s[t] = a.b2[t];
  }
  const int b = blockIdx.y;
  const int p = t >> 2, g = t & 3;
  const int n = blockIdx.x * PTS + p;
  const bool live = n < a.N;
  const int nc = live ? n : a.N - 1;
  const float* xb = b < a.B ? a.x_cf + (size_t)b * 3 * a.N : a.x_cf2 + (size_t)(b - a.B) * 3 * a.N;
  const float x = xb[nc], y = xb[a.N + nc], z = xb[2 * a.N + nc];
  __syncthreads();
#pragma unroll
  for (int j = 0; j < 16; ++j) {
    const int c = g * 16 + j;
    const float v = fmaf(w1s[c][2], z, fmaf(w1s[c][1], y, fmaf(w1s[c][0], x, w1s[c][3])));
    h1s[p][c] = fmaxf(v, 0.f);
  }
  __syncthreads();
  float acc[16];
#pragma unroll
  for (int j = 0; j < 16; ++j) acc[j] = b2s[g * 16 + j];
  for (int k = 0; k < 64; ++k) {
    const float h = h1s[p][k];
#pragma unroll
    for (int q = 0; q < 4; ++q) {
      const f32x4 w = ld4(&w2t[k][g * 16 + q * 4]);
      acc[q * 4 + 0] = fmaf(w[0], h, acc[q * 4 + 0]);
      acc[q * 4 + 1] = fmaf(w[1], h, acc[q * 4 + 1]);
      acc[q * 4 + 2] = fmaf(w[2], h, acc[q * 4 + 2]);
      acc[q * 4 + 3] = fmaf(w[3], h, acc[q * 4 + 3]);
    }
  }
  float ss = 0.f;
#pragma unroll
  for (int j = 0; j < 16; ++j) {
    acc[j] = fmaxf(acc[j], 0.f);
    ss = ss + acc[j] * acc[j];
  }
  const int base = (threadIdx.x & 63) & ~3;
  {
    const float b0 = __shfl(ss, base, 64), b1 = __shfl(ss, base + 1, 64);
    const float b2 = __shfl(ss, base + 2, 64), b3 = __shfl(ss, base + 3, 64);
    ss = ((b0 + b1) + b2) + b3;
  }
  const bool tail = live && n >= (a.N & ~31);
  if (__builtin_amdgcn_ballot_w64(tail) != 0) {
    float a4[4] = {0.f, 0.f, 0.f, 0.f};
#pragma unroll
    for (int sgrp = 0; sgrp < 4; ++sgrp) {
      if (g == sgrp) {
#pragma unroll
        for (int j = 0; j < 16; ++j) a4[j & 3] = a4[j & 3] + acc[j] * acc[j];
      }
#pragma unroll
      for (int l = 0; l < 4; ++l) a4[l] = __shfl(a4[l], base + sgrp, 64);
    }
    if (tail) ss = ((a4[0] + a4[1]) + a4[2]) + a4[3];
  }
  if (live) {
    const size_t row = (size_t)b * a.N + n;
    float* o = a.feat64 + row * 64 + g * 16;
#pragma unroll
    for (int q = 0; q < 4; ++q) st4(o + q * 4, f32x4{acc[q * 4], acc[q * 4 + 1], acc[q * 4 + 2], acc[q * 4 + 3]});
    if (a.feat64t) {
      float* ot = a.feat64t + row * 64 + g * 16;
#pragma unroll
      for (int q = 0; q < 4; ++q) st4(ot + q * 4, f32x4{acc[q], acc[4 + q], acc[8 + q], acc[12 + q]});
    }
    if (g == 0) {
      a.sq64[row] = ss;
      st4(a.xyz4 + row * 4, f32x4{x, y, z, (x * x + y * y) + z * z});
    }
  }
}

constexpr int TP = 68;
constexpr int PQW = 8;
__global__ __launch_bounds__(64 * PQW, 1) void pointwise12_pq_kernel(vcr_pointwise_args a, int tiles_per_cloud, int total_tiles) {
  extern __shared__ __attribute__((aligned(16))) float pw_smem[];
  float* wfrag = pw_smem;
  float* w1s = wfrag + 16 * 4 * 64 * 4;
  float* pqb = w1s + 64 * 4;
  float* tiles = pqb + 256;
  const int t = threadIdx.x, lane = t & 63, wave = t >> 6;
  const int q4 = lane >> 4, l15 = lane & 15;
  f32x4 w2c[4][4];
#pragma unroll
  for (int j = 0; j < 4; ++j)
#pragma unroll
    for (int g = 0; g < 4; ++g) w2c[j][g] = ld4(a.w2 + (16 * j + l15) * 64 + 16 * g + 4 * q4);
  float b2r[4];
#pragma unroll
  for (int j = 0; j < 4; ++j) b2r[j] = a.b2[16 * j + l15];
  f32x4 wq[8];
#pragma unroll
  for (int it = 0; it < 8; ++it) wq[it] = ld4(a.pq_w + 4 * (t + 64 * PQW * it));
  if (t >= 256) pqb[t - 256] = a.pq_b[t - 256];
  if (t < 64) {
    w1s[t * 4 + 0] = a.w1[t * 3 + 0]; w1s[t * 4 + 1] = a.w1[t * 3 + 1]; w1s[t * 4 + 2] = a.w1[t * 3 + 2];
    w1s[t * 4 + 3] = a.b1[t];
  }
  float w2r[4][16];
#pragma unroll
  for (int j = 0; j < 4; ++j)
#pragma unroll
    for (int g = 0; g < 4; ++g) {
      int r0 = __float_as_int(w2c[j][g][0]), r1 = __float_as_int(w2c[j][g][1]);
      int r2 = __float_as_int(w2c[j][g][2]), r3 = __float_as_int(w2c[j][g][3]);
      auto s01 = __builtin_amdgcn_permlane16_swap(r0, r1, false, false); r0 = s01[0]; r1 = s01[1];
      auto s23 = __builtin_amdgcn_permlane16_swap(r2, r3, false, false); r2 = s23[0]; r3 = s23[1];
      auto s02 = __builtin_amdgcn_permlane32_swap(r0, r2, false, false); r0 = s02[0]; r2 = s02[1];
      auto s13 = __builtin_amdgcn_permlane32_swap(r1, r3, false, false); r1 = s13[0]; r3 = s13[1];
      w2r[j][4 * g] = __int_as_float(r0); w2r[j][4 * g + 1] = __int_as_float(r1);
      w2r[j][4 * g + 2] = __int_as_float(r2); w2r[j][4 * g + 3] = __int_as_float(r3);
    }
#pragma unroll
  for (int it = 0; it < 8; ++it) {
    const int c = t + 64 * PQW * it, n = c >> 4, st = c & 15, j = n >> 4;
#pragma unroll
    for (int e = 0; e < 4; ++e) wfrag[(((j * 4 + (st >> 2)) * 64) + e * 16 + (n & 15)) * 4 + (st & 3)] = wq[it][e];
  }
  __syncthreads();
  float* T = tiles + wave * 16 * TP;
  const int p = lane >> 2, g = lane & 3;
  for (int tile = (int)blockIdx.x * PQW + wave; tile < total_tiles; tile += (int)gridDim.x * PQW) {
    const int b = tile / tiles_per_cloud, n0 = (tile - b * tiles_per_cloud) * 16;
    const float* xb = b < a.B ? a.x_cf + (size_t)b * 3 * a.N : a.x_cf2 + (size_t)(b - a.B) * 3 * a.N;
    float h[16];
    {
      const int nc = min(n0 + l15, a.N - 1);
      const float x = xb[nc], y = xb[a.N + nc], z = xb[2 * a.N + nc];
#pragma unroll
      for (int st = 0; st < 16; ++st) {
        const f32x4 w = ld4(&w1s[(4 * st + q4) * 4]);
        h[st] = fmaxf(fmaf(w[2], z, fmaf(w[1], y, fmaf(w[0], x, w[3]))), 0.f);
      }
    }
    f32x4 acc[4];
#pragma unroll
    for (int j = 0; j < 4; ++j) acc[j] = f32x4{b2r[j], b2r[j], b2r[j], b2r[j]};
#pragma unroll
    for (int st = 0; st < 16; ++st)
#pragma unroll
      for (int j = 0; j < 4; ++j) acc[j] = mfma16(h[st], w2r[j][st], acc[j]);
#pragma unroll
    for (int j = 0; j < 4; ++j)
#pragma unroll
      for (int r = 0; r < 4; ++r) T[(4 * q4 + r) * TP + 16 * j + l15] = fmaxf(acc[j][r], 0.f);
    __builtin_amdgcn_s_waitcnt(0xc07f);
    __builtin_amdgcn_wave_barrier();
    auto feature_epilogue = [&]() {
      const int n = n0 + p;
      const bool live = n < a.N;
      const int nc = live ? n : a.N - 1;
      const float x = xb[nc], y = xb[a.N + nc], z = xb[2 * a.N + nc];
      float f[16];
#pragma unroll
      for (int q = 0; q < 4; ++q) {
        const f32x4 v = ld4(&T[p * TP + 16 * g + 4 * q]);
        f[4 * q] = v[0]; f[4 * q + 1] = v[1]; f[4 * q + 2] = v[2]; f[4 * q + 3] = v[3];
      }
      float ss = 0.f;
#pragma unroll
      for (int j = 0; j < 16; ++j) ss = ss + f[j] * f[j];
      const int base = lane & ~3;
      {
        const float s0 = __shfl(ss, base, 64), s1 = __shfl(ss, base + 1, 64);
        const float s2 = __shfl(ss, base + 2, 64), s3 = __shfl(ss, base + 3, 64);
        ss = ((s0 + s1) + s2) + s3;
      }
      const bool tail = live && n >= (a.N & ~31);
      if (__builtin_amdgcn_ballot_w64(tail) != 0) {
        float a4[4] = {0.f, 0.f, 0.f, 0.f};
#pragma unroll
        for (int sgrp = 0; sgrp < 4; ++sgrp) {
          if (g == sgrp) {
#pragma unroll
            for (int j = 0; j < 16; ++j) a4[j & 3] = a4[j & 3] + f[j] * f[j];
          }
#pragma unroll
          for (int l = 0; l < 4; ++l) a4[l] = __shfl(a4[l], base + sgrp, 64);
        }
        if (tail) ss = ((a4[0] + a4[1]) + a4[2]) + a4[3];
      }
      if (live) {
        const size_t row = (size_t)b * a.N + n;
        float* o = a.feat64 + row * 64 + g * 16;
#pragma unroll
        for (int q = 0; q < 4; ++q) st4(o + q * 4, f32x4{f[q * 4], f[q * 4 + 1], f[q * 4 + 2], f[q * 4 + 3]});
        if (a.feat64t) {
          float* ot = a.feat64t + row * 64 + g * 16;
#pragma unroll
          for (int q = 0; q < 4; ++q) st4(ot + q * 4, f32x4{f[q], f[4 + q], f[8 + q], f[12 + q]});
        }
        if (g == 0) {
          a.sq64[row] = ss;
          st4(a.xyz4 + row * 4, f32x4{x, y, z, (x * x + y * y) + z * z});
        }
      }
    };
    auto pq_product = [&]() {
    float af[16];
#pragma unroll
    for (int st = 0; st < 16; ++st) af[st] = T[l15 * TP + 4 * st + q4];
#pragma unroll 1
    for (int jg = 0; jg < 4; ++jg) {
      f32x4 pa[4];
#pragma unroll
      for (int jj = 0; jj < 4; ++jj) {
        const float bq = pqb[16 * (4 * jg + jj) + l15];
        pa[jj] = f32x4{bq, bq, bq, bq};
      }
#pragma unroll
      for (int sq = 0; sq < 4; ++sq)
#pragma unroll
        for (int jj = 0; jj < 4; ++jj) {
          const f32x4 wf = ld4(&wfrag[(((4 * jg + jj) * 4 + sq) * 64 + lane) * 4]);
#pragma unroll
          for (int e = 0; e < 4; ++e) pa[jj] = mfma16(af[4 * sq + e], wf[e], pa[jj]);
        }
#pragma unroll
      for (int jj = 0; jj < 4; ++jj)
#pragma unroll
        for (int r = 0; r < 4; ++r) {
          const int n = n0 + 4 * q4 + r;
          if (n < a.N) a.pq[((size_t)b * a.N + n) * a.ldpq + 16 * (4 * jg + jj) + l15] = pa[jj][r];
        }
    }
    };
    if (wave < PQW / 2) {
      feature_epilogue();
      pq_product();
    } else {
      pq_product();
      feature_epilogue();
    }
    __builtin_amdgcn_s_waitcnt(0xc07f);
    __builtin_amdgcn_wave_barrier();
  }
}

__global__ __launch_bounds__(256) void rows4_kernel(const float* x_cf, float* xyz4, int B, int N) {
  const long i = (long)blockIdx.x * 256 + threadIdx.x;
  if (i >= (long)B * N) return;
  const int b = (int)(i / N), n = (int)(i % N);
  const float* xb = x_cf + (size_t)b * 3 * N;
  const float x = xb[n], y = xb[N + n], z = xb[2 * N + n];
  st4(xyz4 + i * 4, f32x4{x, y, z, (x * x + y * y) + z * z});
}

__global__ __launch_bounds__(256) void rows4_pq_kernel(const float* x_cf, float* xyz4, int B, int N, const float* wpq,
                                                       int ldw, const float* bpq, int C, float* pq, int ldpq) {
  const int per = C / 4, cg = threadIdx.x % per;
  const long i = (long)blockIdx.x * (256 / per) + threadIdx.x / per;
  if (i >= (long)B * N) return;
  const int b = (int)(i / N), n = (int)(i % N);
  const float* xb = x_cf + (size_t)b * 3 * N;
  const float x = xb[n], y = xb[N + n], z = xb[2 * N + n];
  if (cg == 0) st4(xyz4 + i * 4, f32x4{x, y, z, (x * x + y * y) + z * z});
  f32x4 o;
#pragma unroll
  for (int e = 0; e < 4; ++e) {
    const float* wr = wpq + (size_t)(4 * cg + e) * ldw;
    o[e] = fmaf(wr[2], z, fmaf(wr[1], y, wr[0] * x)) + bpq[4 * cg + e];
  }
  st4(pq + i * ldpq + 4 * cg, o);
}

}

extern "C" int vcr_rows4_pq_f32(const float* x_cf, float* xyz4, int B, int N, const float* wpq, int ldw, const float* bpq,
                                int C, float* pq, int ldpq, vcr_stream_t stream) {
  if (!x_cf || !xyz4 || !wpq || !bpq || !pq || B <= 0 || N <= 0) return VCR_EINVAL;
  if (C <= 0 || (C % 4) || 256 % (C / 4) || ldw < 3 || ldpq < C || (ldpq & 3) || ((uintptr_t)pq & 15)) return VCR_EINVAL;
  const int pts = 256 / (C / 4);
  hipLaunchKernelGGL(rows4_pq_kernel, dim3((unsigned)(((long)B * N + pts - 1) / pts)), dim3(256), 0, (hipStream_t)stream,
                     x_cf, xyz4, B, N, wpq, ldw, bpq, C, pq, ldpq);
  return VCR_LAUNCH_RC();
}

extern "C" int vcr_rows4_f32(const float* x_cf, float* xyz4, int B, int N, vcr_stream_t stream) {
  if (!x_cf || !xyz4 || B <= 0 || N <= 0) return VCR_EINVAL;
  hipLaunchKernelGGL(rows4_kernel, dim3((unsigned)(((long)B * N + 255) / 256)), dim3(256), 0, (hipStream_t)stream, x_cf,
                     xyz4, B, N);
  return VCR_LAUNCH_RC();
}

extern "C" int vcr_pointwise_f32(const vcr_pointwise_args* a, vcr_stream_t stream) {
  vcr_stream_scope bound(stream);
  if (!a || !a->x_cf || !a->w1 || !a->b1 || !a->w2 || !a->b2 || !a->xyz4 || !a->feat64 || !a->sq64) return VCR_EINVAL;
  if (((uintptr_t)a->w2 | (uintptr_t)a->pq_w) & 15) return VCR_EINVAL;
  if (a->B <= 0 || a->N <= 0 || a->B2 < 0 || (a->B2 > 0 && !a->x_cf2)) return VCR_EINVAL;
  if (a->pq) {
    if (!a->pq_w || !a->pq_b || a->ldpq < 256 || (a->ldpq & 3)) return VCR_EINVAL;
    const int tpc = (a->N + 15) / 16, total = tpc * (a->B + a->B2);
    const int cus = vcr_cu_count(), blocks = (total + PQW - 1) / PQW < cus ? (total + PQW - 1) / PQW : cus;
    const size_t lds = (size_t)(16 * 4 * 64 * 4 + 64 * 4 + 256 + PQW * 16 * TP) * sizeof(float);
    VCR_DYN_LDS(pointwise12_pq_kernel, lds);
    hipLaunchKernelGGL(pointwise12_pq_kernel, dim3(blocks), dim3(64 * PQW), lds, (hipStream_t)stream, *a, tpc, total);
    return VCR_LAUNCH_RC();
  }
  dim3 grid((a->N + PTS - 1) / PTS, a->B + a->B2);
  hipLaunchKernelGGL(pointwise12_kernel, grid, dim3(256), 0, (hipStream_t)stream, *a);
  return VCR_LAUNCH_RC();
}
```

### vcr-net_amd/csrc/rigid_svd.hip

```cpp
#include "common.h"

namespace {

__device__ __forceinline__ double wave_sum_f64(double v) {
#pragma unroll
  for (int o = 32; o >= 1; o >>= 1) v += __shfl_xor(v, o, 64);
  return v;
}
template <int NV>
__device__ __forceinline__ void block_sums(double (&v)[NV], double* red) {
  const int w = threadIdx.x >> 6;
#pragma unroll
  for (int e = 0; e < NV; ++e) v[e] = wave_sum_f64(v[e]);
  __syncthreads();
  if ((threadIdx.x & 63) == 0)
#pragma unroll
    for (int e = 0; e < NV; ++e) red[w * NV + e] = v[e];
  __syncthreads();
#pragma unroll
  for (int e = 0; e < NV; ++e) v[e] = ((red[e] + red[NV + e]) + red[2 * NV + e]) + red[3 * NV + e];
}
__device__ __forceinline__ double quad_xor(double v, int ctrl_is_1) {
  int lo = __double2loint(v), hi = __double2hiint(v);
  if (ctrl_is_1) { lo = __builtin_amdgcn_mov_dpp(lo, 0xB1, 0xF, 0xF, true); hi = __builtin_amdgcn_mov_dpp(hi, 0xB1, 0xF, 0xF, true); }
  else { lo = __builtin_amdgcn_mov_dpp(lo, 0x4E, 0xF, 0xF, true); hi = __builtin_amdgcn_mov_dpp(hi, 0x4E, 0xF, 0xF, true); }
  return __hiloint2double(hi, lo);
}
__device__ __forceinline__ double quad_sum(double v) {
  v += quad_xor(v, 1);
  v += quad_xor(v, 0);
  return v;
}
__device__ __forceinline__ double quad_get(double v, int lane_in_quad) {
  int lo = __double2loint(v), hi = __double2hiint(v);
  const int c = lane_in_quad == 0 ? 0x00 : lane_in_quad == 1 ? 0x55 : 0xAA;
  if (lane_in_quad == 0) { lo = __builtin_amdgcn_mov_dpp(lo, 0x00, 0xF, 0xF, true); hi = __builtin_amdgcn_mov_dpp(hi, 0x00, 0xF, 0xF, true); }
  else if (lane_in_quad == 1) { lo = __builtin_amdgcn_mov_dpp(lo, 0x55, 0xF, 0xF, true); hi = __builtin_amdgcn_mov_dpp(hi, 0x55, 0xF, 0xF, true); }
  else { lo = __builtin_amdgcn_mov_dpp(lo, 0xAA, 0xF, 0xF, true); hi = __builtin_amdgcn_mov_dpp(hi, 0xAA, 0xF, 0xF, true); }
  (void)c;
  return __hiloint2double(hi, lo);
}

__device__ __forceinline__ void jacobi_sweeps_quad(double (&a)[3], double (&v)[3]) {
  for (int sweep = 0; sweep < 40; ++sweep) {
    double off = 0.0;
#pragma unroll
    for (int pq = 0; pq < 3; ++pq) {
      const int p = (pq == 2) ? 1 : 0, q = (pq == 0) ? 1 : 2;
      const double al = quad_sum(a[p] * a[p]), be = quad_sum(a[q] * a[q]), ga = quad_sum(a[p] * a[q]);
      const double ab = sqrt(al) * sqrt(be);
      if (!(fabs(ga) > 1e-17 * ab)) continue;
      off = fmax(off, fabs(ga) / ab);
      const double zeta = (be - al) / (2.0 * ga);
      const double tt = (zeta >= 0 ? 1.0 : -1.0) / (fabs(zeta) + sqrt(1.0 + zeta * zeta));
      const double c = 1.0 / sqrt(1.0 + tt * tt), s = c * tt;
      const double ap = a[p], aq = a[q];
      a[p] = c * ap - s * aq; a[q] = s * ap + c * aq;
      const double vp = v[p], vq = v[q];
      v[p] = c * vp - s * vq; v[q] = s * vp + c * vq;
    }
    if (off < 1e-15) break;
  }
}

__device__ void svd3_finish(const double A[3][3], const double V[3][3], double R[9]) {
  double sig[3];
  int ord[3] = {0, 1, 2};
  for (int j = 0; j < 3; ++j) sig[j] = sqrt(A[0][j] * A[0][j] + A[1][j] * A[1][j] + A[2][j] * A[2][j]);
  for (int i = 0; i < 2; ++i)
    for (int j = 0; j < 2 - i; ++j)
      if (sig[ord[j]] < sig[ord[j + 1]]) { const int tmp = ord[j]; ord[j] = ord[j + 1]; ord[j + 1] = tmp; }
  double U[3][3], W[3][3];
  for (int j = 0; j < 3; ++j) {
    const int c = ord[j];
    const double inv = sig[c] > 0 ? 1.0 / sig[c] : 0.0;
    for (int i = 0; i < 3; ++i) { U[i][j] = A[i][c] * inv; W[i][j] = V[i][c]; }
  }
  const double s0 = sig[ord[0]];
  if (!(s0 > 0)) {
    for (int i = 0; i < 3; ++i) for (int j = 0; j < 3; ++j) U[i][j] = W[i][j];
  } else {
    if (sig[ord[1]] <= 1e-12 * s0) {
      int e = 0;
      for (int i = 1; i < 3; ++i) if (fabs(U[i][0]) < fabs(U[e][0])) e = i;
      double v[3] = {0, 0, 0}, n2 = 0;
      v[e] = 1.0;
      const double d = U[e][0];
      for (int i = 0; i < 3; ++i) { v[i] -= d * U[i][0]; n2 += v[i] * v[i]; }
      const double inv = 1.0 / sqrt(n2);
      for (int i = 0; i < 3; ++i) U[i][1] = v[i] * inv;
    }
    if (sig[ord[2]] <= 1e-12 * s0) {
      U[0][2] = U[1][0] * U[2][1] - U[2][0] * U[1][1];
      U[1][2] = U[2][0] * U[0][1] - U[0][0] * U[2][1];
      U[2][2] = U[0][0] * U[1][1] - U[1][0] * U[0][1];
    }
  }
  auto build = [&]() {
    for (int i = 0; i < 3; ++i)
      for (int j = 0; j < 3; ++j) R[3 * i + j] = W[i][0] * U[j][0] + W[i][1] * U[j][1] + W[i][2] * U[j][2];
  };
  build();
  const double det = R[0] * (R[4] * R[8] - R[5] * R[7]) - R[1] * (R[3] * R[8] - R[5] * R[6]) +
                     R[2] * (R[3] * R[7] - R[4] * R[6]);
  if (det < 0) {
    for (int i = 0; i < 3; ++i) W[i][2] = -W[i][2];
    build();
  }
}

__global__ __launch_bounds__(256) void rigid_svd_kernel(vcr_rigid_svd_args p) {
  __shared__ double red[4 * 9];
  const int b = blockIdx.x, t = threadIdx.x;
  const float* S = p.src + (size_t)b * p.K * p.lds;
  const float* C = p.corr + (size_t)b * p.K * p.ldc;
  double mean[6] = {0, 0, 0, 0, 0, 0};
  for (int i = t; i < p.K; i += 256)
    for (int c = 0; c < 3; ++c) { mean[c] += S[(size_t)i * p.lds + c]; mean[3 + c] += C[(size_t)i * p.ldc + c]; }
  block_sums<6>(mean, red);
  float smf[3], cmf[3];
  for (int c = 0; c < 3; ++c) { smf[c] = (float)(mean[c] / p.K); cmf[c] = (float)(mean[3 + c] / p.K); }
  double H[9] = {0, 0, 0, 0, 0, 0, 0, 0, 0};
  for (int i = t; i < p.K; i += 256) {
    float sc[3], cc[3];
    for (int c = 0; c < 3; ++c) { sc[c] = S[(size_t)i * p.lds + c] - smf[c]; cc[c] = C[(size_t)i * p.ldc + c] - cmf[c]; }
    for (int r = 0; r < 3; ++r)
      for (int c = 0; c < 3; ++c) H[3 * r + c] += (double)sc[r] * (double)cc[c];
  }
  block_sums<9>(H, red);
  if (t >= 64) return;
  const int li = t & 3;
  double a[3], v[3];
#pragma unroll
  for (int j = 0; j < 3; ++j) {
    a[j] = li == 0 ? H[j] : li == 1 ? H[3 + j] : li == 2 ? H[6 + j] : 0.0;
    v[j] = li == j ? 1.0 : 0.0;
  }
  jacobi_sweeps_quad(a, v);
  double A[3][3], V[3][3];
#pragma unroll
  for (int j = 0; j < 3; ++j) {
    A[0][j] = quad_get(a[j], 0); A[1][j] = quad_get(a[j], 1); A[2][j] = quad_get(a[j], 2);
    V[0][j] = quad_get(v[j], 0); V[1][j] = quad_get(v[j], 1); V[2][j] = quad_get(v[j], 2);
  }
  if (t == 0) {
    double R[9];
    svd3_finish(A, V, R);
    bool finite = true;
    for (int e = 0; e < 9; ++e) finite = finite && __builtin_isfinite(H[e]);
    for (int c = 0; c < 6; ++c) finite = finite && __builtin_isfinite(mean[c]);
    if (!finite)
      for (int e = 0; e < 9; ++e) R[e] = __builtin_nan("");
    float* Ro = p.R + (size_t)b * 9;
    float* to = p.t + (size_t)b * 3;
    float Rf[9], tf[3];
    for (int e = 0; e < 9; ++e) { Rf[e] = (float)R[e]; Ro[e] = Rf[e]; }
    for (int r = 0; r < 3; ++r) {
      tf[r] = (float)(-(R[3 * r] * smf[0] + R[3 * r + 1] * smf[1] + R[3 * r + 2] * smf[2]) + cmf[r]);
      to[r] = tf[r];
    }
    if (p.R_ba) for (int r = 0; r < 3; ++r) for (int c = 0; c < 3; ++c) p.R_ba[(size_t)b * 9 + 3 * r + c] = Rf[3 * c + r];
    if (p.t_ba) for (int r = 0; r < 3; ++r)
      p.t_ba[(size_t)b * 3 + r] = -(Rf[r] * tf[0] + Rf[3 + r] * tf[1] + Rf[6 + r] * tf[2]);
    if (p.H) for (int e = 0; e < 9; ++e) p.H[(size_t)b * 9 + e] = (float)H[e];
  }
}

}

extern "C" int vcr_rigid_svd_f32(const vcr_rigid_svd_args* a, vcr_stream_t stream) {
  if (!a || !a->src || !a->corr || !a->R || !a->t) return VCR_EINVAL;
  if (a->B <= 0 || a->K < 3 || a->lds < 3 || a->ldc < 3) return VCR_EINVAL;
  hipLaunchKernelGGL(rigid_svd_kernel, dim3(a->B), dim3(256), 0, (hipStream_t)stream, *a);
  return VCR_LAUNCH_RC();
}
```

### vcr-net_amd/module.py

```python
from __future__ import annotations

import ctypes as C
import os
import threading
from typing import Dict, Optional, Tuple

import torch
import torch.nn as nn

from . import native
from .weights import strip_module_prefix

LINEAR_MODES = {"fp32": 0, "bf16x3": 1, "bf16x3+sdpa": 2}


_CALL = threading.local()


class _call_scope:

    def __enter__(self):
        self.owner = getattr(_CALL, "tensors", None) is None
        if self.owner:
            _CALL.tensors = {}
# ... 53 lines not shown
        super().__init__()
        self.k = 1
        chans = [(3, 64), (64, 64), (64, 64), (64, 128), (128, emb_dims)]
        for i, (ci, co) in enumerate(chans, 1):
            setattr(self, f"conv{i}", nn.Conv1d(ci, co, kernel_size=1, bias=False))
        for i, (_, co) in enumerate(chans, 1):
            setattr(self, f"bn{i}", nn.BatchNorm1d(co))


class _Norm(nn.Module):
    def __init__(self, n):
        super().__init__()
        self.a_2 = nn.Parameter(torch.ones(n))
        self.b_2 = nn.Parameter(torch.zeros(n))
        self.eps = 1e-6


class _Sublayer(nn.Module):
    def __init__(self, n):
        super().__init__()
        self.norm = _Norm(n)


class _MHA(nn.Module):
    def __init__(self, h, d):
        super().__init__()
        self.h, self.d_k = h, d // h
        self.linears = nn.ModuleList([nn.Linear(d, d) for _ in range(4)])


class _FFN(nn.Module):
    def __init__(self, d, f):
        super().__init__()
        self.w_1 = nn.Linear(d, f)
        self.w_2 = nn.Linear(f, d)


class _EncLayer(nn.Module):
    def __init__(self, d, f, h):
        super().__init__()
        self.self_attn = _MHA(h, d)
        self.feed_forward = _FFN(d, f)
        self.sublayer = nn.ModuleList([_Sublayer(d) for _ in range(2)])
        self.size = d


class _DecLayer(nn.Module):
    def __init__(self, d, f, h):
        super().__init__()
        self.size = d
        self.self_attn = _MHA(h, d)
        self.src_attn = _MHA(h, d)
        self.feed_forward = _FFN(d, f)
        self.sublayer = nn.ModuleList([_Sublayer(d) for _ in range(3)])


class _Stack(nn.Module):
    def __init__(self, layers, d):
        super().__init__()
        self.layers = nn.ModuleList(layers)
        self.norm = _Norm(d)


class _EncDec(nn.Module):
    def __init__(self, d, f, h, n):
        super().__init__()
        self.encoder = _Stack([_EncLayer(d, f, h) for _ in range(n)], d)
        self.decoder = _Stack([_DecLayer(d, f, h) for _ in range(n)], d)


class _TransformerParams(nn.Module):

    def __init__(self, args):
        super().__init__()
        self.emb_dims, self.N, self.ff_dims = args.emb_dims, args.n_blocks, args.ff_dims
        self.n_heads, self.overlap2 = args.n_heads, args.overlap2
        self.model = _EncDec(args.emb_dims, args.ff_dims, args.n_heads, args.n_blocks)


class _Identity(nn.Module):
    pass


class _VcpTopK(nn.Module):
    def __init__(self, args):
        super().__init__()
        self.emb_nn, self.partial, self.overlap2 = args.emb_nn, args.partial, args.overlap2


class _VcpByDis(nn.Module):
    def __init__(self, args):
        super().__init__()
        self.emb_nn = args.emb_nn


class _VcpAtt(nn.Module):
    def __init__(self, args):
        super().__init__()
        self.emb_dims = args.emb_dims
        self.linears_emb = nn.ModuleList([nn.Linear(args.emb_dims, args.emb_dims) for _ in range(2)])
        self.linears_3d = nn.ModuleList([nn.Linear(3, 3) for _ in range(2)])


class _SVDHead(nn.Module):
    def __init__(self):
        super().__init__()
        r = torch.eye(3)
        r[2, 2] = -1
        self.reflect = nn.Parameter(r, requires_grad=False)



class VCRNet(nn.Module):

    def __init__(self, args):
        super().__init__()
        self.emb_dims = args.emb_dims
        self.cycle = args.cycle
        if args.emb_nn == "pointnet":
            self.emb_nn = _PointNetParams(emb_dims=self.emb_dims)
        elif args.emb_nn == "dgcnn":
            self.emb_nn = _DGCNNParams(emb_dims=self.emb_dims)
        elif args.emb_nn == "lpdnet":
            self.emb_nn = _LPDNetParams(args)
        else:
            raise Exception("Not implemented")
        if args.pointer == "identity":
            self.pointer = _Identity()
        elif args.pointer == "transformer":
            self.pointer = _TransformerParams(args)
        else:
            self.pointer = None
        if args.vcp_nn == "topK":
            self.head = _VcpTopK(args)
        elif args.vcp_nn == "att":
            self.head = _VcpAtt(args)
        elif args.vcp_nn == "dist":
            self.head = _VcpByDis(args)
        else:
            raise Exception("Not implemented")
        self.svd = _SVDHead()
        self._emb_kind, self._vcp = args.emb_nn, args.vcp_nn
        self._partial = bool(getattr(args, "partial", False))
        self._overlap2 = float(getattr(args, "overlap2", 0.75))
        self._n_heads, self._ff = args.n_heads, args.ff_dims
        self.linear_mode = os.environ.get("VCRNET_LINEAR_MODE", "fp32")
        self.linear_mfma, self.linear_bk, self.knn_waves = 0, 0, 0
        self.linear_bm = 0
        self.merge_encdec = os.environ.get("VCRNET_MERGE_ENCDEC", "1") == "1"
        self.xscore_limit_mb = 0
        self.sdpa_variant = 0
        self.iter_reuse = True
        self.workspace_flat = False
        self._packed: Optional[Dict[str, torch.Tensor]] = None
        self._packed_key = None
        self._cw: Optional[native.VcrnetWeights] = None
        self._shared = _Shared(self)
        self.launch_trace: Optional[native.Trace] = None

    def load_state_dict(self, state_dict, strict: bool = True, **kw):
        return super().load_state_dict(strip_module_prefix(state_dict), strict=strict, **kw)

    def __getstate__(self):
        d = self.__dict__.copy()
        d.pop("_shared", None)
        d["_packed"], d["_packed_key"], d["_cw"] = None, None, None
        return d

    def _tensors(self) -> Dict[str, torch.Tensor]:
        scope = getattr(_CALL, "tensors", None)
        if scope is not None and id(self) in scope:
            return scope[id(self)]
        out: Dict[str, torch.Tensor] = {}
        for prefix, mod in self.named_modules():
            former = mod.__dict__.get("_former_parameters") if getattr(mod, "_is_replica", False) else None
            src = former if former is not None else mod._parameters
            for k, v in list(src.items()) + list(mod._buffers.items()):
                if v is not None:
                    out[(prefix + "." if prefix else "") + k] = v
        if scope is not None:
            scope[id(self)] = out
        return out

    def _device(self) -> torch.device:
        return next(iter(self._tensors().values())).device

    def _master(self):
        sh = self.__dict__.get("_shared")
        m = sh.master() if sh is not None else None
        if m is None or (m is not self and not getattr(self, "_is_replica", False)):
            self._shared = sh = _Shared(self)
            m = self
        return m, sh

    def _fingerprint(self):
        m, _ = self._master()
        ps = list(m._tensors().values())
        dev = self._device()
        return (dev, ps[0].device, tuple(p._version for p in ps), tuple(p.data_ptr() for p in ps[:4]), self.emb_nn.k,
                self.linear_mode, self.linear_mfma, self.linear_bk, self.linear_bm, self.knn_waves, self.xscore_limit_mb,
                self.merge_encdec, bool(self.workspace_flat), int(self.sdpa_variant), bool(self.iter_reuse))

    def _pack(self):
        m, sh = self._master()
        key = self._fingerprint()
        dev = key[0]
        cur = torch.cuda.current_stream(dev)
        with sh.lock:
            hit = sh.packed.get(dev)
            if hit is not None and hit[0] == key:
                self._packed_key, self._packed, self._cw, ev, waited = hit
                if cur.cuda_stream not in waited:
                    cur.wait_event(ev)
                    waited.add(cur.cuda_stream)
                return
            if hit is not None:
                torch.cuda.synchronize(dev)
            self._pack_locked(key, own=m is not self)
            ev = torch.cuda.Event()
            ev.record(cur)
            sh.packed[dev] = (self._packed_key, self._packed, self._cw, ev, {cur.cuda_stream})
            sh.packs += 1

    def _pack_locked(self, key, own):
        sd = {k: v.detach().float() for k, v in self._tensors().items()}
        P: Dict[str, torch.Tensor] = {}
        g = (lambda k: sd[k].contiguous().clone()) if own else (lambda k: sd[k].contiguous())
        cw = native.VcrnetWeights()

        def put(struct, field, key, tensor):
            P[key] = tensor
            setattr(struct, field, native.ptr(tensor))

        def put_wb(struct, prefix, w, b, pair):
            put(struct, w, prefix + w, pair[0]); put(struct, b, prefix + b, pair[1])

        if self._emb_kind == "lpdnet":
            conv = lambda name, *shape: (g(f"emb_nn.{name}.weight").view(*shape).contiguous(), g(f"emb_nn.{name}.bias"))

            def halves(name, c):
                w, b = g(f"emb_nn.{name}.weight").view(2 * c, 2 * c), sd[f"emb_nn.{name}.bias"]
                return torch.cat((w[:, :c], w[:, c:]), 0).contiguous(), torch.cat((torch.zeros_like(b), b))
            put_wb(cw, "", "c1_w", "c1_b", conv("conv1_lpd", 64, 3))
            put_wb(cw, "", "c2_w", "c2_b", conv("conv2_lpd", 64, 64))
            put_wb(cw, "", "dg1_wpq", "dg1_bpq", halves("convDG1.0", 64))
            put_wb(cw, "", "dg2_w", "dg2_b", conv("convDG2.0", 128, 128))
            put_wb(cw, "", "sn1_wpq", "sn1_bpq", halves("convSN1.0", 128))
            put_wb(cw, "", "c3_w", "c3_b", conv("conv3_lpd", self.emb_dims, 512))
        if self._emb_kind == "dgcnn":
            def fold(i, eps=1e-5):
                sc = sd[f"emb_nn.bn{i}.weight"] / torch.sqrt(sd[f"emb_nn.bn{i}.running_var"] + eps)
                wq = sd[f"emb_nn.conv{i}.weight"].reshape(sd[f"emb_nn.conv{i}.weight"].shape[0], -1)
                return ((wq * sc.view(-1, 1)).contiguous(),
                        (sd[f"emb_nn.bn{i}.bias"] - sd[f"emb_nn.bn{i}.running_mean"] * sc).contiguous())
            w1, b1 = fold(1)
            wpq = torch.zeros(128, 32, dtype=torch.float32, device=w1.device)
            wpq[:64, :3], wpq[64:, :3] = w1[:, :3], w1[:, 3:]
            put_wb(cw.dgcnn, "dg.", "c1_wpq", "c1_bpq", (wpq, torch.cat((torch.zeros_like(b1), b1)).contiguous()))
            for i in (2, 3, 4, 5):
                put_wb(cw.dgcnn, "dg.", f"c{i}_w", f"c{i}_b", fold(i))
            cw.emb_kind = 1
        if self._emb_kind == "pointnet":
            from .composed import _fold_bn
            for i in (1, 2, 3, 4, 5):
                put_wb(cw if i < 3 else cw.pointnet, "pn.", f"c{i}_w", f"c{i}_b",
                       _fold_bn(sd, f"emb_nn.conv{i}", f"emb_nn.bn{i}"))
            cw.emb_kind = 2
        if isinstance(self.pointer, _TransformerParams):
            pre = "pointer.model."

            def norm(field, name):
                put(getattr(cw, field), "ln_a", field + ".a", g(name + ".a_2"))
                put(getattr(cw, field), "ln_b", field + ".b", g(name + ".b_2"))

            def mha(field, name, cross):
                W = [g(f"{name}.linears.{i}.weight") for i in range(4)]
                Bv = [g(f"{name}.linears.{i}.bias") for i in range(4)]
                m = getattr(cw, field)
                if cross:
                    put_wb(m, field + ".", "wq", "bq", (W[0], Bv[0]))
                    put_wb(m, field + ".", "wkv", "bkv",
                           (torch.cat((W[1], W[2]), 0).contiguous(), torch.cat((Bv[1], Bv[2])).contiguous()))
                else:
                    put_wb(m, field + ".", "wqkv", "bqkv", (torch.cat(W[:3], 0).contiguous(), torch.cat(Bv[:3]).contiguous()))
                put_wb(m, field + ".", "wo", "bo", (W[3], Bv[3]))

            def ffn(field, name):
                for f, leaf in (("w1", "w_1.weight"), ("b1", "w_1.bias"), ("w2", "w_2.weight"), ("b2", "w_2.bias")):
                    put(getattr(cw, field), f, field + "." + leaf, g(name + "." + leaf))

            def folded(site, f):
                P["fold." + site] = f
                for field, t in zip(("w", "colsum", "bias"), f):
                    put(getattr(cw, "fold_" + site), field, f"fold.{site}.{field}", t)

            e, d = pre + "encoder.layers.0", pre + "decoder.layers.0"
            norm("enc_ln0", e + ".sublayer.0.norm"); norm("enc_ln1", e + ".sublayer.1.norm")
            norm("enc_norm", pre + "encoder.norm")
            norm("dec_ln0", d + ".sublayer.0.norm"); norm("dec_ln1", d + ".sublayer.1.norm")
            norm("dec_ln2", d + ".sublayer.2.norm"); norm("dec_norm", pre + "decoder.norm")
            mha("enc_self", e + ".self_attn", False); mha("dec_self", d + ".self_attn", False)
            mha("dec_cross", d + ".src_attn", True)
            ffn("enc_ffn", e + ".feed_forward"); ffn("dec_ffn", d + ".feed_forward")
            cw.has_pointer = 1
            for site, wk, bk, nk in (("enc_qkv", "enc_self.wqkv", "enc_self.bqkv", "enc_ln0"),
                                     ("enc_ffn1", "enc_ffn.w_1.weight", "enc_ffn.w_1.bias", "enc_ln1"),
                                     ("dec_qkv", "dec_self.wqkv", "dec_self.bqkv", "dec_ln0"),
                                     ("dec_cross_q", "dec_cross.wq", "dec_cross.bq", "dec_ln1"),
                                     ("dec_cross_kv", "dec_cross.wkv", "dec_cross.bkv", "enc_norm"),
                                     ("dec_ffn1", "dec_ffn.w_1.weight", "dec_ffn.w_1.bias", "dec_ln2")):
                folded(site, native.fold_layernorm(P[wk], P[bk], P[nk + ".a"], P[nk + ".b"]))
            if self.merge_encdec:
                folded("encdec_qkv", tuple(torch.cat((a_, b_), 0).contiguous()
                                           for a_, b_ in zip(P["fold.enc_qkv"], P["fold.dec_qkv"])))
        else:
            cw.has_pointer = 2 if isinstance(self.pointer, _Identity) else 0
        if self.linear_mode not in LINEAR_MODES:
            raise ValueError(f"linear_mode {self.linear_mode!r}: one of {sorted(LINEAR_MODES)}")
        cw.linear_mode = LINEAR_MODES[self.linear_mode]
        if cw.linear_mode != 0:
            src = {"dg1_pq": "dg1_wpq", "sn1_pq": "sn1_wpq", "c3": "c3_w", "enc_qkv": "fold.enc_qkv.w",
                   "enc_wo": "enc_self.wo", "enc_ffn1": "fold.enc_ffn1.w", "enc_ffn2": "enc_ffn.w_2.weight",
                   "dec_qkv": "fold.dec_qkv.w", "dec_self_wo": "dec_self.wo", "dec_cross_q": "fold.dec_cross_q.w",
                   "dec_cross_kv": "fold.dec_cross_kv.w", "dec_cross_wo": "dec_cross.wo", "dec_ffn1": "fold.dec_ffn1.w",
                   "dec_ffn2": "dec_ffn.w_2.weight", "encdec_qkv": "fold.encdec_qkv.w"}
            for site, name in src.items():
                if name in P:
                    put(cw.split, site, "split." + site, native.split_bf16x3(P[name]))
        cw.E, cw.F, cw.heads, cw.k = self.emb_dims, self._ff, self._n_heads, int(self.emb_nn.k)
        cw.head_mode = {"topK": 0, "dist": 1, "att": 2}[self._vcp]
        if self._vcp == "att":
            for i in (0, 1):
                put(cw, f"att_w{i}", f"att.w{i}", g(f"head.linears_emb.{i}.weight"))
                put(cw, f"att_b{i}", f"att.b{i}", g(f"head.linears_emb.{i}.bias"))
        cw.cycle = int(bool(self.cycle))
        cw.linear_mfma, cw.linear_bk, cw.linear_bm = int(self.linear_mfma), int(self.linear_bk), int(self.linear_bm)
        cw.knn_waves = int(self.knn_waves)
        cw.xscore_limit_mb = int(self.xscore_limit_mb)
        cw.workspace_flat = int(bool(self.workspace_flat))
        cw.sdpa_variant = int(self.sdpa_variant)
        cw.iter_reuse = 0 if self.iter_reuse else 1
        cw.partial, cw.overlap2 = int(self._partial), self._overlap2
        self._packed, self._packed_key = P, key
        self._cw = cw

    def _take_buffers(self, B: int, N: int, device, iters: int = 1) -> Tuple[Tuple, Dict[str, torch.Tensor]]:
        sh = self._shared
        key = (B, N, device, int(self.emb_nn.k), int(self.xscore_limit_mb), bool(self.merge_encdec), self.linear_mode,
               self._emb_kind, self._vcp, self._partial, self._overlap2, bool(self.workspace_flat),
               bool(self.iter_reuse) and iters > 1)
        with sh.lock:
            idle = sh.pool.get(key)
            if idle:
                return key, idle.pop()
            for k_ in [k_ for k_ in sh.pool if k_[2] == device and k_ != key]:
                for b_ in sh.pool.pop(k_):
                    self._retire(b_)
        nbytes = native.lib().vcr_vcrnet_iter_workspace_bytes(C.byref(self._cw), B, N, int(iters))
        return key, {"ws": torch.empty(nbytes + 256, dtype=torch.uint8, device=device)}

    MAX_IDLE_WORKSPACES = 4

    @staticmethod
    def _retire(bufs):
        st = bufs.get("stream")
        if st is not None:
            bufs["ws"].record_stream(st)

    def _give_buffers(self, key, bufs):
        with self._shared.lock:
            idle = self._shared.pool.setdefault(key, [])
            if len(idle) < self.MAX_IDLE_WORKSPACES:
                idle.append(bufs)
            else:
                self._retire(bufs)

    def fused_supported(self) -> bool:
        if isinstance(self.pointer, _TransformerParams) and self.pointer.N != 1:
            return False
        if self._partial:
            if not isinstance(self.pointer, _TransformerParams):
                return False
            return not (self.cycle and self._vcp == "topK")
        return True

    def _check_call(self, src, tgt):
        if not (src.is_cuda and tgt.is_cuda):
            raise native.VcrHipError("vcrnet_amd.VCRNet runs on the MI355X HIP path only; move inputs to cuda "
                                     "(there is no CPU fallback by design)")
        pdev = self._device()
        if not (src.device == tgt.device == pdev):
            raise native.VcrHipError(f"src ({src.device}), tgt ({tgt.device}) and the parameters ({pdev}) must "
                                     "live on one device")
        if self.training or torch.is_grad_enabled():
            raise native.VcrHipError("inference only: call .eval() and wrap in torch.no_grad() "
                                     "(model/vcrnet_model.py:546); backward kernels are out of scope")
        _check_shapes(src, tgt)

    def forward(self, *input):
        with _call_scope():
            return self._forward(*input)

    def _forward(self, *input):
        src, tgt = input[0], input[1]
        self._check_call(src, tgt)
        with torch.cuda.device(src.device):
            self._pack()
            if not self.fused_supported():
                from .composed import forward_composed
                return forward_composed(self, src, tgt)
            return self._forward_fused(src, tgt, trace=self.launch_trace)

    def selection_sizes(self, N: int) -> Dict[str, int]:
        k1 = int(N * 0.84 * self._overlap2)
        return {"keys": int(N * self._overlap2), "sel_src": k1, "sel_tgt": k1, "argmax": k1,
                "pairs": int(k1 * 0.52 * self._overlap2)}

    def _forward_fused(self, src, tgt, trace: Optional[native.Trace] = None, want_emb: bool = False, iters: int = 1,
                       force: Optional[Dict[str, torch.Tensor]] = None, want_selections: bool = False,
                       iter_api: bool = False):
        with _call_scope(), torch.cuda.device(src.device):
            return self._forward_fused_on(src, tgt, trace, want_emb, iters, force, want_selections, iter_api)

    def _forward_fused_on(self, src, tgt, trace, want_emb, iters, force, want_selections, iter_api):
        _check_shapes(src, tgt)
        self._pack()
        B, _, N = src.shape
        dev = native.same_device(src, tgt, next(iter(self._tensors().values())))
        srcc, tgtc = src.contiguous().float(), tgt.contiguous().float()
        bkey, bufs = self._take_buffers(B, N, dev, iters)
        try:
            return self._forward_with(bufs, srcc, tgtc, src, B, N, dev, trace, want_emb, iters, force, want_selections,
                                      iter_api)
        finally:
            self._give_buffers(bkey, bufs)

    def _forward_with(self, bufs, srcc, tgtc, src, B, N, dev, trace, want_emb, iters, force, want_selections, iter_api):
        ws = bufs["ws"]
        cur = torch.cuda.current_stream(dev)
        prev = bufs.get("stream")
        if prev is not None and prev != cur:
            cur.wait_stream(prev)
        bufs["stream"] = cur
        off = (-ws.data_ptr()) % 256
        f = lambda *s: torch.empty(*s, dtype=torch.float32, device=dev)
        L = native.lib()
        K = L.vcr_vcrnet_pairs(C.byref(self._cw), N)
        corr4, src4 = f(B, K, 4), f(B, K, 4)
        R_ab, t_ab, R_ba, t_ba = f(B, 3, 3), f(B, 3), f(B, 3, 3), f(B, 3)
        emb = f(2 * B * N, self.emb_dims) if want_emb else None
        io = native.VcrnetIo(native.ptr(srcc), native.ptr(tgtc), B, N, native.ptr(corr4), native.ptr(src4),
                             native.ptr(R_ab), native.ptr(t_ab), native.ptr(R_ba), native.ptr(t_ba), native.ptr(emb))
        keepalive, sel = [], {}
        if force or want_selections:
            if not self._partial:
                raise native.VcrHipError("forced / reported selections exist in partial mode only")
            sizes = self.selection_sizes(N)
            for name in native.SELECTION_FIELDS:
                rows = 2 * B if name == "keys" else B
                if force and name in force:
                    t = force[name].to(device=dev, dtype=torch.int32).reshape(iters, rows, sizes[name]).contiguous()
                    keepalive.append(t)
                    setattr(io, "force_" + name, native.ptr(t))
                if want_selections and (self._vcp == "topK" or name == "keys"):
                    sel[name] = torch.empty(iters, rows, sizes[name], dtype=torch.int32, device=dev)
                    setattr(io, "out_" + name, native.ptr(sel[name]))
        stream = C.c_void_p(native.stream_ptr(dev))
        wsp = C.c_void_p(ws.data_ptr() + off)
        if iters != 1 or iter_api:
            rc = L.vcr_vcrnet_iter_f32(C.byref(self._cw), C.byref(io), iters, wsp, ws.numel() - off, stream,
                                       C.byref(trace) if trace is not None else None)
        elif trace is None:
            rc = L.vcr_vcrnet_forward_f32(C.byref(self._cw), C.byref(io), wsp, ws.numel() - off, stream)
        else:
            rc = L.vcr_vcrnet_forward_traced_f32(C.byref(self._cw), C.byref(io), wsp, ws.numel() - off, stream,
                                                 C.byref(trace))
        native.check(rc, "vcr_vcrnet_iter_f32" if (iters != 1 or iter_api) else "vcr_vcrnet_forward_f32")
        rows = lambda x: x[:, :, :3].transpose(1, 2).contiguous()
        hard = self._partial and self._vcp == "topK"
        srcK = rows(src4) if (hard or iters != 1) else src
        out = (srcK, rows(corr4), R_ab, t_ab, R_ba, t_ba)
        if want_emb:
            out = out + (emb,)
        return out + (sel,) if want_selections else out

    def forward_iter(self, src, tgt, iters: int):
        self._check_call(src, tgt)
        if not self.fused_supported():
            return None
        return self._forward_fused(src, tgt, trace=self.launch_trace, iters=int(iters), iter_api=True)


def _check_shapes(src, tgt):
    if src.dim() != 3 or tgt.dim() != 3 or src.shape[1] != 3 or tgt.shape[1] != 3:
        raise native.VcrHipError(f"src and tgt must be [B, 3, N] point clouds, got {tuple(src.shape)} and {tuple(tgt.shape)}")
    if src.shape != tgt.shape:
        raise native.VcrHipError(f"tgt must have the same B and N as src, got src {tuple(src.shape)} and tgt {tuple(tgt.shape)}"
                                 " (clouds of unequal size are not supported)")


class DCP(VCRNet):

    def __init__(self, args):
# ... 76 lines not shown
```

### vcr-net_amd/native.py

```python
from __future__ import annotations

import ctypes as C
import os
from typing import Optional

import torch

_HERE = os.path.dirname(os.path.abspath(__file__))
LIB_PATH = os.path.join(_HERE, "libvcr_hip.so")
VCR_TRACE_MAX = 256

f32p = C.c_void_p


class PointwiseArgs(C.Structure):
    _fields_ = [("x_cf", f32p), ("B", C.c_int), ("N", C.c_int), ("w1", f32p), ("b1", f32p), ("w2", f32p),
                ("b2", f32p), ("xyz4", f32p), ("feat64", f32p), ("sq64", f32p), ("x_cf2", f32p), ("B2", C.c_int),
                ("pq_w", f32p), ("pq_b", f32p), ("pq", f32p), ("ldpq", C.c_int), ("feat64t", f32p)]


class _Sized(C.Structure):

    def __init__(self, *args, **kw):
        super().__init__(C.sizeof(type(self)), *args, **kw)


class KnnArgs(_Sized):
    _fields_ = [("struct_bytes", C.c_uint32), ("x", f32p), ("ldx", C.c_int), ("sq", f32p), ("B", C.c_int), ("N", C.c_int), ("C", C.c_int),
                ("k", C.c_int), ("idx", f32p), ("tie_scratch", f32p), ("tie_cap", C.c_int), ("waves", C.c_int),
                ("tie_zeroed", C.c_int),
                ("tie_defer", C.c_int), ("tie_work", C.c_void_p), ("tie_work_bytes", C.c_size_t), ("tie_inline", C.c_int),
                ("xt", f32p),
                ("perm", f32p), ("xp", f32p), ("sqp", f32p), ("cen", f32p), ("cen_sq", f32p), ("cen_rad", f32p),
                ("cen_sqmax", f32p), ("ord_ok", f32p)]


class KnnOrderArgs(C.Structure):
    _fields_ = [("xyz4", f32p), ("feat_t", f32p), ("ldf", C.c_int), ("sq", f32p), ("B", C.c_int), ("N", C.c_int),
                ("perm", f32p), ("xyz4_p", f32p), ("cen4", f32p), ("cen4_rad", f32p), ("cen4_sqmax", f32p),
                ("feat_p", f32p), ("sq_p", f32p), ("cen64", f32p), ("cen64_sq", f32p), ("cen64_rad", f32p),
                ("cen64_sqmax", f32p), ("ord_ok", f32p), ("ord_stat", f32p), ("guard_ratio", C.c_float)]


class FpsArgs(_Sized):
    _fields_ = [("struct_bytes", C.c_uint32), ("xyz_cf", f32p), ("cloud_stride", C.c_long), ("B", C.c_int), ("N", C.c_int),
                ("npoint", C.c_int), ("start", f32p), ("idx", f32p), ("out_cf", f32p), ("variant", C.c_int)]


class LinearArgs(C.Structure):
    _fields_ = [("x", f32p), ("ldx", C.c_int), ("w", f32p), ("bias", f32p), ("residual", f32p), ("ldr", C.c_int),
                ("y", f32p), ("ldy", C.c_int), ("M", C.c_int), ("N", C.c_int), ("K", C.c_int), ("relu", C.c_int),
                ("ln_stats_in", f32p), ("ln_nseg", C.c_int), ("ln_colsum", f32p), ("ln_eps", C.c_float),
                ("stats_out", f32p), ("segmax_out", f32p), ("ld_segmax", C.c_int), ("seg_k", C.c_int),
                ("variant", C.c_int)]


class LayerNormArgs(C.Structure):
    _fields_ = [("x", f32p), ("ldx", C.c_int), ("a", f32p), ("b", f32p), ("eps", C.c_float), ("residual", f32p),
                ("ldr", C.c_int), ("y", f32p), ("ldy", C.c_int), ("M", C.c_int), ("C", C.c_int), ("xyz4", f32p),
                ("side4", f32p)]


class RowsideArgs(C.Structure):
    _fields_ = [("x", f32p), ("ldx", C.c_int), ("M", C.c_int), ("C", C.c_int), ("scale", C.c_float), ("y", f32p),
                ("ldy", C.c_int), ("xyz4", f32p), ("side4", f32p)]


class EdgeconvArgs(C.Structure):
    _fields_ = [("pq", f32p), ("ldpq", C.c_int), ("idx", f32p), ("k", C.c_int), ("M", C.c_int),
                ("n_per_cloud", C.c_int), ("w2", f32p), ("b2", f32p), ("x1", f32p), ("ldx1", C.c_int),
                ("x2", f32p), ("ldx2", C.c_int)]


class GathermaxArgs(C.Structure):
    _fields_ = [("pq", f32p), ("ldpq", C.c_int), ("C", C.c_int), ("idx", f32p), ("k", C.c_int), ("M", C.c_int),
                ("n_per_cloud", C.c_int), ("y", f32p), ("ldy", C.c_int), ("variant", C.c_int), ("order", f32p)]


class SdpaArgs(C.Structure):
    _fields_ = [("q", f32p), ("ldq", C.c_int), ("k", f32p), ("ldk", C.c_int), ("v", f32p), ("ldv", C.c_int),
                ("out", f32p), ("ldo", C.c_int), ("nbatch", C.c_int), ("heads", C.c_int), ("nq", C.c_int),
                ("nk", C.c_int), ("scale", C.c_float), ("kv_batch_shift", C.c_int), ("key_keep", f32p),
                ("rowstat", f32p), ("score_out", f32p), ("ld_score", C.c_int),
                ("ngroups", C.c_int), ("q_group_stride", C.c_long), ("k_group_stride", C.c_long), ("v_group_stride", C.c_long),
                ("out_group_stride", C.c_long), ("key_index", f32p), ("nk_src", C.c_int), ("split_work", f32p),
                ("split_work_floats", C.c_long), ("variant", C.c_int), ("plan_nbatch", C.c_int)]


class KeymassArgs(C.Structure):
    _fields_ = [("score", f32p), ("ld", C.c_int), ("nbatch", C.c_int), ("heads", C.c_int), ("nq", C.c_int),
                ("nk", C.c_int), ("rowstat", f32p), ("q_batch_shift", C.c_int), ("mass", f32p)]


class SoftcorrArgs(C.Structure):
    _fields_ = [("q", f32p), ("ldq", C.c_int), ("k", f32p), ("ldk", C.c_int), ("qside4", f32p), ("kside4", f32p),
                ("corr4", f32p), ("nbatch", C.c_int), ("nq", C.c_int), ("nk", C.c_int), ("E", C.c_int),
                ("mode", C.c_int), ("scale", C.c_float), ("split_work", f32p), ("split_work_floats", C.c_long)]


class PairscoreArgs(C.Structure):
    _fields_ = [("own", f32p), ("ld_own", C.c_int), ("str", f32p), ("ld_str", C.c_int), ("own_side4", f32p),
                ("str_side4", f32p), ("nbatch", C.c_int), ("n_own", C.c_int), ("n_str", C.c_int), ("E", C.c_int),
                ("score", C.c_int), ("scale", C.c_float), ("str_batch_shift", C.c_int), ("op", C.c_int),
                ("corr4", f32p), ("stat2", f32p), ("argmax", f32p), ("str_stat2", f32p),
                ("str_stat_batch_stride", C.c_long), ("mass", f32p), ("accumulate", C.c_int),
                ("score_out", f32p), ("ld_score", C.c_int), ("variant", C.c_int), ("split_work", f32p),
                ("split_work_floats", C.c_long)]


class MakePairsArgs(C.Structure):
    _fields_ = [("cloud", f32p), ("P", C.c_int), ("R_ab", f32p), ("t_ab", f32p), ("pick", f32p), ("perm_src", f32p),
                ("perm_tgt", f32p), ("B", C.c_int), ("N", C.c_int), ("keep", C.c_int), ("src_cf", f32p),
                ("tgt_cf", f32p)]


class ScoremassArgs(C.Structure):
    _fields_ = [("score", f32p), ("ld", C.c_int), ("nbatch", C.c_int), ("n_rows", C.c_int), ("n_cols", C.c_int),
                ("row_stat2", f32p), ("col_stat2", f32p), ("col_mass", f32p), ("row_mass", f32p)]


class RankselectArgs(C.Structure):
    _fields_ = [("values", f32p), ("nbatch", C.c_int), ("n", C.c_int), ("K", C.c_int), ("order", f32p),
                ("mask", f32p), ("largest", C.c_int), ("stride", C.c_int)]


class GatherArgs(C.Structure):
    _fields_ = [("in_", f32p), ("ld_in", C.c_int), ("n_in", C.c_int), ("idx", f32p), ("nbatch", C.c_int),
                ("n_out", C.c_int), ("C", C.c_int), ("out", f32p), ("ld_out", C.c_int), ("via", f32p), ("n_via", C.c_int)]


class EdgerowsArgs(C.Structure):
    _fields_ = [("pq", f32p), ("ldpq", C.c_int), ("C", C.c_int), ("idx", f32p), ("k", C.c_int), ("M", C.c_int),
                ("n_per_cloud", C.c_int), ("h", f32p), ("ldh", C.c_int), ("ymax", f32p), ("ldymax", C.c_int),
                ("zero_to", C.c_int)]


class EdgechainArgs(C.Structure):
    _fields_ = [("pq", f32p), ("ldpq", C.c_int), ("idx", f32p), ("k", C.c_int), ("M", C.c_int), ("n_per_cloud", C.c_int),
                ("w2", f32p), ("b2", f32p), ("w3", f32p), ("b3", f32p), ("w4", f32p), ("b4", f32p),
                ("out", f32p), ("ldo", C.c_int)]


class SegmaxArgs(C.Structure):
    _fields_ = [("x", f32p), ("ldx", C.c_int), ("M", C.c_int), ("k", C.c_int), ("C", C.c_int), ("y", f32p),
                ("ldy", C.c_int)]


class RigidSvdArgs(C.Structure):
    _fields_ = [("src", f32p), ("lds", C.c_int), ("corr", f32p), ("ldc", C.c_int), ("B", C.c_int), ("K", C.c_int),
                ("R", f32p), ("t", f32p), ("R_ba", f32p), ("t_ba", f32p), ("H", f32p)]


class NormW(C.Structure):
    _fields_ = [("ln_a", f32p), ("ln_b", f32p)]


class MhaW(C.Structure):
    _fields_ = [("wqkv", f32p), ("bqkv", f32p), ("wq", f32p), ("bq", f32p), ("wkv", f32p), ("bkv", f32p),
                ("wo", f32p), ("bo", f32p)]


class FfnW(C.Structure):
    _fields_ = [("w1", f32p), ("b1", f32p), ("w2", f32p), ("b2", f32p)]


SPLIT_SITES = ("dg1_pq", "sn1_pq", "c3", "enc_qkv", "enc_wo", "enc_ffn1", "enc_ffn2", "dec_qkv", "dec_self_wo",
               "dec_cross_q", "dec_cross_kv", "dec_cross_wo", "dec_ffn1", "dec_ffn2", "encdec_qkv")


class SplitW(C.Structure):
    _fields_ = [(s, f32p) for s in SPLIT_SITES]


class FoldedW(C.Structure):
    _fields_ = [("w", f32p), ("colsum", f32p), ("bias", f32p)]


class DgcnnW(C.Structure):
    _fields_ = [(n, f32p) for n in ("c1_wpq", "c1_bpq", "c2_w", "c2_b", "c3_w", "c3_b", "c4_w", "c4_b", "c5_w", "c5_b")]


class PointnetW(C.Structure):
    _fields_ = [(n, f32p) for n in ("c3_w", "c3_b", "c4_w", "c4_b", "c5_w", "c5_b")]


class VcrnetWeights(_Sized):
    _fields_ = [("struct_bytes", C.c_uint32), ("c1_w", f32p), ("c1_b", f32p), ("c2_w", f32p), ("c2_b", f32p),
                ("dg1_wpq", f32p), ("dg1_bpq", f32p), ("dg2_w", f32p), ("dg2_b", f32p),
                ("sn1_wpq", f32p), ("sn1_bpq", f32p), ("c3_w", f32p), ("c3_b", f32p),
                ("enc_ln0", NormW), ("enc_ln1", NormW), ("enc_norm", NormW), ("dec_ln0", NormW),
                ("dec_ln1", NormW), ("dec_ln2", NormW), ("dec_norm", NormW),
                ("enc_self", MhaW), ("dec_self", MhaW), ("dec_cross", MhaW),
                ("enc_ffn", FfnW), ("dec_ffn", FfnW),
                ("E", C.c_int), ("F", C.c_int), ("heads", C.c_int), ("k", C.c_int),
                ("has_pointer", C.c_int), ("head_mode", C.c_int), ("linear_mode", C.c_int), ("split", SplitW),
                ("fold_enc_qkv", FoldedW), ("fold_enc_ffn1", FoldedW), ("fold_dec_qkv", FoldedW),
                ("fold_dec_cross_q", FoldedW), ("fold_dec_cross_kv", FoldedW), ("fold_dec_ffn1", FoldedW),
                ("fold_encdec_qkv", FoldedW),
                ("partial", C.c_int), ("overlap2", C.c_double), ("emb_kind", C.c_int), ("dgcnn", DgcnnW), ("pointnet", PointnetW),
                ("att_w0", f32p), ("att_b0", f32p), ("att_w1", f32p), ("att_b1", f32p), ("cycle", C.c_int),
                ("linear_mfma", C.c_int), ("linear_bk", C.c_int), ("linear_bm", C.c_int), ("knn_waves", C.c_int),
                ("xscore_limit_mb", C.c_int), ("sdpa_variant", C.c_int), ("iter_reuse", C.c_int), ("workspace_flat", C.c_int)]


class VcrnetIo(C.Structure):
    _fields_ = [("src_cf", f32p), ("tgt_cf", f32p), ("B", C.c_int), ("N", C.c_int), ("corr4", f32p), ("src4", f32p),
                ("R_ab", f32p), ("t_ab", f32p), ("R_ba", f32p), ("t_ba", f32p), ("emb_out", f32p),
                ("force_keys", f32p), ("force_sel_src", f32p), ("force_sel_tgt", f32p), ("force_argmax", f32p),
                ("force_pairs", f32p), ("out_keys", f32p), ("out_sel_src", f32p), ("out_sel_tgt", f32p),
                ("out_argmax", f32p), ("out_pairs", f32p)]


SELECTION_FIELDS = ("keys", "sel_src", "sel_tgt", "argmax", "pairs")


class Trace(C.Structure):
    _fields_ = [("events", C.POINTER(C.c_void_p)), ("capacity", C.c_int), ("count", C.c_int),
                ("names", C.c_char_p * VCR_TRACE_MAX)]


class IcpArgs(C.Structure):
    _fields_ = [("src4", f32p), ("dst4", f32p), ("B", C.c_int), ("N", C.c_int), ("M", C.c_int),
                ("max_iterations", C.c_int), ("tolerance", C.c_float), ("final4", f32p), ("R", f32p), ("t", f32p),
                ("R_ba", f32p), ("t_ba", f32p), ("iterations", f32p)]


class PoseStepArgs(C.Structure):
    _fields_ = [("R_i", f32p), ("t_i", f32p), ("B", C.c_int), ("N", C.c_int), ("in_cf", f32p), ("out_cf", f32p),
                ("compose", C.c_int), ("R_f", f32p), ("t_f", f32p), ("R_ba", f32p), ("t_ba", f32p)]



STRUCTS = {
    "vcr_pointwise_args": PointwiseArgs, "vcr_knn_args": KnnArgs, "vcr_knn_order_args": KnnOrderArgs, "vcr_fps_args": FpsArgs,
    "vcr_linear_args": LinearArgs, "vcr_layernorm_args": LayerNormArgs, "vcr_rowside_args": RowsideArgs,
    "vcr_edgeconv_args": EdgeconvArgs, "vcr_gathermax_args": GathermaxArgs, "vcr_edgerows_args": EdgerowsArgs,
    "vcr_edgechain_args": EdgechainArgs, "vcr_segmax_args": SegmaxArgs, "vcr_sdpa_args": SdpaArgs,
    "vcr_keymass_args": KeymassArgs, "vcr_softcorr_args": SoftcorrArgs, "vcr_pairscore_args": PairscoreArgs,
    "vcr_scoremass_args": ScoremassArgs, "vcr_rankselect_args": RankselectArgs, "vcr_gather_args": GatherArgs,
    "vcr_rigid_svd_args": RigidSvdArgs, "vcr_icp_args": IcpArgs, "vcr_make_pairs_args": MakePairsArgs,
    "vcr_pose_step_args": PoseStepArgs, "vcr_vcrnet_weights": VcrnetWeights, "vcr_vcrnet_io": VcrnetIo, "vcr_trace": Trace,
}

_int, _size, _long, _float, _vp = C.c_int, C.c_size_t, C.c_long, C.c_float, C.c_void_p
_P = C.POINTER
_intp = _P(C.c_int)

_ARGS_STREAM = {
    "vcr_pointwise_f32": PointwiseArgs, "vcr_knn_f32": KnnArgs, "vcr_knn_order_f32": KnnOrderArgs, "vcr_linear_f32": LinearArgs,
    "vcr_layernorm_f32": LayerNormArgs, "vcr_rowside_f32": RowsideArgs, "vcr_edgeconv_f32": EdgeconvArgs,
    "vcr_edgeconv_bf16x3_f32": EdgeconvArgs, "vcr_gathermax_f32": GathermaxArgs, "vcr_sdpa_f32": SdpaArgs,
    "vcr_sdpa_bf16x3_f32": SdpaArgs, "vcr_softcorr_f32": SoftcorrArgs, "vcr_rigid_svd_f32": RigidSvdArgs,
    "vcr_pairscore_f32": PairscoreArgs, "vcr_rankselect_f32": RankselectArgs, "vcr_gather_rows_f32": GatherArgs,
    "vcr_scoremass_f32": ScoremassArgs, "vcr_keymass_f32": KeymassArgs, "vcr_make_pairs_f32": MakePairsArgs,
    "vcr_edgerows_f32": EdgerowsArgs, "vcr_segmax_f32": SegmaxArgs, "vcr_edgechain_f32": EdgechainArgs, "vcr_fps_f32": FpsArgs,
    "vcr_pose_step_f32": PoseStepArgs,
}

PUBLIC = {name: (_int, [_P(st), _vp]) for name, st in _ARGS_STREAM.items()}
PUBLIC.update({
    "vcr_strerror": (C.c_char_p, [_int]),
    "vcr_abi_version": (_int, []),
    "vcr_rows4_f32": (_int, [_vp, _vp, _int, _int, _vp]),
    "vcr_rows4_pq_f32": (_int, [_vp, _vp, _int, _int, _vp, _int, _vp, _int, _vp, _int, _vp]),
    "vcr_knn_tie_work_bytes": (_size, [_int]),
    "vcr_knn_tie_slot_bytes": (_size, [_int, _int]),
    "vcr_knn_ties_inline": (_int, [_P(KnnArgs)]),
    "vcr_knn_ties_f32": (_int, [_P(KnnArgs), _P(KnnArgs), _vp]),
    "vcr_knn_pair_f32": (_int, [_P(KnnArgs), _P(KnnArgs), _vp]),
    "vcr_linear_config": (_int, [_P(LinearArgs)]),
    "vcr_linear_pair_f32": (_int, [_P(LinearArgs), _P(LinearArgs), _vp]),
    "vcr_fold_layernorm_f32": (_int, [_vp, _vp, _vp, _vp, _int, _int, _vp, _vp, _vp, _vp]),
    "vcr_split_bf16x3_f32": (_int, [_vp, _vp, _size, _vp]),
    "vcr_linear_bf16x3_f32": (_int, [_P(LinearArgs), _vp, _vp]),
    "vcr_icp_workspace_bytes": (_size, [_int, _int]),
    "vcr_icp_f32": (_int, [_P(IcpArgs), _vp, _size, _vp]),
    "vcr_fps_form": (_int, [_P(FpsArgs), _intp, _intp]),
    "vcr_vcrnet_workspace_bytes": (_size, [_P(VcrnetWeights), _int, _int]),
    "vcr_vcrnet_iter_workspace_bytes": (_size, [_P(VcrnetWeights), _int, _int, _int]),
    "vcr_vcrnet_pairs": (_int, [_P(VcrnetWeights), _int]),
    "vcr_vcrnet_forward_f32": (_int, [_P(VcrnetWeights), _P(VcrnetIo), _vp, _size, _vp]),
    "vcr_vcrnet_forward_traced_f32": (_int, [_P(VcrnetWeights), _P(VcrnetIo), _vp, _size, _vp, _P(Trace)]),
    "vcr_vcrnet_iter_f32": (_int, [_P(VcrnetWeights), _P(VcrnetIo), _int, _vp, _size, _vp, _P(Trace)]),
    "vcr_event_create": (_int, [_P(_vp)]),
    "vcr_event_destroy": (_int, [_vp]),
    "vcr_event_record": (_int, [_vp, _vp]),
    "vcr_event_elapsed_ms": (_int, [_vp, _vp, _P(_float)]),
})

INTERNAL = {
    "vcr_linear_forms_": (_int, [_P(LinearArgs), _P(LinearArgs), _intp, _intp, _intp]),
    "vcr_knn_forms_": (_int, [_P(KnnArgs), _P(KnnArgs), _intp, _intp, _intp]),
    "vcr_sdpa_forms_": (_int, [_P(SdpaArgs), _intp, _intp]),
    "vcr_sdpa_split_floats_": (_long, [_size, _int, _int, _long, _int, _int]),
    "vcr_edgeconv_forms_": (_int, [_P(EdgeconvArgs), _int, _intp, _intp]),
    "vcr_gathermax_forms_": (_int, [_P(GathermaxArgs), _intp, _intp, _intp, _intp]),
}

SIGNATURES = {**PUBLIC, **INTERNAL}

PROBES = {"vcr_dbg_probe_" + stem: (_int, [_vp, _int])
          for stem in ("linear", "linear_bf16x3", "attention", "attention_bf16x3", "knn", "pointwise", "edgeconv")}

_lib: Optional[C.CDLL] = None


ABI_VERSION = 27


class VcrHipError(RuntimeError):
    pass


def lib() -> C.CDLL:
    global _lib
    if _lib is None:
        if not os.path.exists(LIB_PATH):
            raise VcrHipError(f"{LIB_PATH} not built: run `python vcr-net_amd/build.py` "
                              "(or __graft_entry__.build()); the HIP path has no fallback")
        L = C.CDLL(LIB_PATH)
        for name, (res, args) in list(SIGNATURES.items()) + [(n, s) for n, s in PROBES.items() if hasattr(L, n)]:
            fn = getattr(L, name)
            fn.restype, fn.argtypes = res, args
        if L.vcr_abi_version() != ABI_VERSION:
            raise VcrHipError(f"{LIB_PATH} exports ABI {L.vcr_abi_version()}, these bindings are for {ABI_VERSION}: "
                              "rebuild with `python vcr-net_amd/build.py`")
        _lib = L
    return _lib


class LaunchTrace:

    def __init__(self, capacity: int = VCR_TRACE_MAX):
        L = lib()
        self.capacity = capacity
        self._arr = (C.c_void_p * capacity)()
        for i in range(capacity):
            e = C.c_void_p()
            check(L.vcr_event_create(C.byref(e)), "vcr_event_create")
            self._arr[i] = e.value
        self.trace = Trace(C.cast(self._arr, C.POINTER(C.c_void_p)), capacity, 0)

    def launches(self):
        L = lib()
        n = min(self.trace.count, self.capacity - 1, VCR_TRACE_MAX)
        out = []
        for i in range(n):
            ms = C.c_float()
            check(L.vcr_event_elapsed_ms(self._arr[i], self._arr[i + 1], C.byref(ms)), "vcr_event_elapsed_ms")
            out.append((self.trace.names[i].decode(), ms.value))
        return out

    def close(self):
        L = lib()
        for i in range(self.capacity):
# ... 96 lines not shown
        work = torch.empty(need, dtype=torch.uint8, device=device)
        a.tie_work, a.tie_work_bytes = ptr(work), need
        keep.append(work)


@_guarded
def knn_pair(feat, sq, xyz4, k, xt=None, order=None, tie_slots=False, prefill=None):
    out, args, keep = [], [], []
    for x, s_ in ((feat, sq), (xyz4, None)):
        B, N, Cc = x.shape
        idx = _i32(B, N, k, device=x.device, prefill=prefill)
        ties = torch.empty(1 + B * N, dtype=torch.int32, device=x.device)
        args.append(KnnArgs(ptr(x), x.stride(1), ptr(s_), B, N, Cc, k, ptr(idx), ptr(ties), B * N, 0))
        _tie_work(args[-1], N, x.device, keep, slots_for=B if tie_slots else 0)
        out.append(idx); keep.append(ties)
    args[0].xt = ptr(xt)
    if order is not None:
        o = lambda n: ptr(order[n])
        args[0].perm = args[1].perm = o("perm")
        a = args[0]
        a.xp, a.sqp, a.cen, a.cen_sq, a.cen_rad, a.cen_sqmax = o("feat_p"), o("sq_p"), o("cen64"), o("cen64_sq"), o("cen64_rad"), o("cen64_sqmax")
        a.ord_ok = ptr(order.get("ord_ok"))
        a = args[1]
        a.xp, a.cen, a.cen_rad, a.cen_sqmax = o("xyz4_p"), o("cen4"), o("cen4_rad"), o("cen4_sqmax")
    call("vcr_knn_pair_f32", args[0], args[1])
    return out[0], out[1]


@_guarded
def knn_pair_deferred(xa, sqa, xb, sqb, k, prefill=None):
    args, keep = [], []
    for x, sq in ((xa, sqa), (xb, sqb)):
        B, N, Cc = x.shape
        idx = _i32(B, N, k, device=x.device, prefill=prefill)
        ties = torch.zeros(1 + B * N, dtype=torch.int32, device=x.device)
        a = KnnArgs(ptr(x), x.stride(1), ptr(sq), B, N, Cc, k, ptr(idx), ptr(ties), B * N, 0)
        a.tie_zeroed, a.tie_defer = 1, 1
        work = []
        _tie_work(a, N, x.device, work)
        call("vcr_knn_f32", a)
        args.append(a); keep.append((idx, ties, work))
    call("vcr_knn_ties_f32", args[0], args[1])
    return keep[0][0], keep[1][0]


@_guarded
def linear(x, w, bias=None, relu=False, residual=None, out=None, ln=None, want_stats=False, variant=0, segmax=None,
           store=True):
    M, K = x.shape
    N = w.shape[0]
    y = None if not store else out if out is not None else _f32(M, N, device=x.device)
    stats = _f32(M, N // 64, 2, device=x.device) if want_stats else None
    a = LinearArgs(ptr(x), x.stride(0), ptr(w), ptr(bias), ptr(residual),
                   residual.stride(0) if residual is not None else 0, ptr(y), y.stride(0) if y is not None else N,
                   M, N, K, int(relu))
    if segmax is not None:
        a.segmax_out, a.ld_segmax, a.seg_k = ptr(segmax[0]), segmax[0].stride(0), int(segmax[1])
    if ln is not None:
        a.ln_stats_in, a.ln_nseg, a.ln_colsum, a.ln_eps = ptr(ln[0]), ln[0].shape[1], ptr(ln[1]), ln[2]
    a.stats_out = ptr(stats)
    a.variant = variant
    call("vcr_linear_f32", a)
    return (y, stats) if want_stats else y


@_guarded
def fold_layernorm(w, bias, ln_a, ln_b):
    N, K = w.shape
    w = w.contiguous()
    wf, cs, bf = _f32(N, K, device=w.device), _f32(N, device=w.device), _f32(N, device=w.device)
    call("vcr_fold_layernorm_f32", ptr(w), ptr(bias), ptr(ln_a), ptr(ln_b), N, K, ptr(wf), ptr(cs), ptr(bf))
    return wf, cs, bf


@_guarded
def split_bf16x3(w):
    w = w.contiguous().float()
    planes = torch.empty(3, w.numel(), dtype=torch.int16, device=w.device)
    call("vcr_split_bf16x3_f32", ptr(w), ptr(planes), w.numel())
    return planes


@_guarded
def linear_bf16x3(x, w_planes, n_out, bias=None, relu=False, residual=None, out=None, ln=None, want_stats=False):
    M, K = x.shape
    y = out if out is not None else _f32(M, n_out, device=x.device)
    stats = _f32(M, n_out // 64, 2, device=x.device) if want_stats else None
    a = LinearArgs(ptr(x), x.stride(0), None, ptr(bias), ptr(residual),
                   residual.stride(0) if residual is not None else 0, ptr(y), y.stride(0), M, n_out, K, int(relu))
    if ln is not None:
        a.ln_stats_in, a.ln_nseg, a.ln_colsum, a.ln_eps = ptr(ln[0]), ln[0].shape[1], ptr(ln[1]), ln[2]
    a.stats_out = ptr(stats)
    call("vcr_linear_bf16x3_f32", a, ptr(w_planes))
    return (y, stats) if want_stats else y


@_guarded
def layernorm(x, a, b, eps=1e-6, residual=None, xyz4=None):
    M, Cc = x.shape
    y = _f32(M, Cc, device=x.device)
    side4 = _f32(M, 4, device=x.device) if xyz4 is not None else None
    call("vcr_layernorm_f32", LayerNormArgs(ptr(x), x.stride(0), ptr(a), ptr(b), eps, ptr(residual),
                                            residual.stride(0) if residual is not None else 0, ptr(y), Cc, M, Cc,
                                            ptr(xyz4), ptr(side4)))
    return (y, side4) if xyz4 is not None else y


@_guarded
def rowside(x, xyz4, scale=1.0):
    M, Cc = x.shape
    y, side4 = _f32(M, Cc, device=x.device), _f32(M, 4, device=x.device)
    call("vcr_rowside_f32", RowsideArgs(ptr(x), x.stride(0), M, Cc, scale, ptr(y), Cc, ptr(xyz4), ptr(side4)))
    return y, side4


@_guarded
def edgeconv(pq, idx, n_per_cloud, w2, b2, bf16x3=False, out=None):
    M = pq.shape[0]
    k = idx.shape[-1]
    x1, x2 = out if out is not None else (_f32(M, 128, device=pq.device), _f32(M, 128, device=pq.device))
    if out is not None and any(t.shape != (M, 128) or t.stride(1) != 1 or t.dtype != torch.float32 for t in out):
        raise VcrHipError("edgeconv: out = (x1, x2) must be fp32 [M, 128] row views")
    call("vcr_edgeconv_bf16x3_f32" if bf16x3 else "vcr_edgeconv_f32", EdgeconvArgs(ptr(pq), pq.stride(0), ptr(idx), k, M, n_per_cloud, ptr(w2), ptr(b2),
                                          ptr(x1), x1.stride(0), ptr(x2), x2.stride(0)))
    return x1, x2


def knn_order(xyz4, feat_t=None, sq=None, guard=False, guard_ratio=0.0):
    B, N, _ = xyz4.shape
    T = (N + 15) // 16
    e = lambda *s, dt=torch.float32: torch.empty(*s, dtype=dt, device=xyz4.device)
    o = {"perm": e(B, N, dt=torch.int32), "xyz4_p": e(B, N, 4), "cen4": e(B, T, 4), "cen4_rad": e(B, T), "cen4_sqmax": e(B, T)}
    if feat_t is not None:
        o.update(feat_p=e(B, N, 64), sq_p=e(B, N), cen64=e(B, T, 64), cen64_sq=e(B, T), cen64_rad=e(B, T), cen64_sqmax=e(B, T))
        if guard:
            o.update(ord_ok=e(B, dt=torch.int32), ord_stat=e(B))
    g = lambda n: ptr(o.get(n))
    a = KnnOrderArgs(ptr(xyz4), ptr(feat_t), feat_t.stride(1) if feat_t is not None else 0, ptr(sq), B, N, g("perm"), g("xyz4_p"),
                     g("cen4"), g("cen4_rad"), g("cen4_sqmax"), g("feat_p"), g("sq_p"), g("cen64"), g("cen64_sq"), g("cen64_rad"),
                     g("cen64_sqmax"), g("ord_ok"), g("ord_stat"), float(guard_ratio))
    call("vcr_knn_order_f32", a)
    return o


@_guarded
def gathermax(pq, Cc, idx, n_per_cloud, variant=0, order=None):
    M = pq.shape[0]
    k = idx.shape[-1]
    y = _f32(M, Cc, device=pq.device)
    call("vcr_gathermax_f32", GathermaxArgs(ptr(pq), pq.stride(0), Cc, ptr(idx), k, M, n_per_cloud, ptr(y), Cc, variant, ptr(order)))
    return y


@_guarded
def sdpa(q, k, v, nbatch, heads, nq, nk, scale, kv_batch_shift=0, key_keep=None, want_rowstat=False, pv=True,
         score_out=None, bf16x3=False, groups=None, key_index=None, nk_src=0, split=False, variant=0):
    ng = groups[0] if groups else 1
    out = _f32(ng * nbatch * nq, heads * 128, device=q.device) if pv else None
    rs = _f32(nbatch, heads, nq, 2, device=q.device) if want_rowstat else None
    a = SdpaArgs(ptr(q), q.stride(0), ptr(k), k.stride(0), ptr(v) if pv else None, v.stride(0) if pv else 0, ptr(out),
                 heads * 128 if pv else 0, nbatch, heads, nq, nk, scale, kv_batch_shift, ptr(key_keep), ptr(rs),
                 ptr(score_out), score_out.stride(2) if score_out is not None else 0)
    if groups:
        a.ngroups, a.q_group_stride, a.k_group_stride, a.v_group_stride = groups
        a.out_group_stride = nbatch * nq * heads * 128
    if key_index is not None:
        a.key_index, a.nk_src = ptr(key_index), int(nk_src)
    work = _f32(4 * ng * (nbatch * nq * heads * 128 * (1 if pv else 0) + nbatch * heads * nq * 2), device=q.device) if split else None
    a.split_work, a.split_work_floats = ptr(work), (work.numel() if split else 0)
    a.variant = int(variant)
    call("vcr_sdpa_bf16x3_f32" if bf16x3 else "vcr_sdpa_f32", a)
    if groups:
        out = out.view(ng, nbatch * nq, heads * 128)
    return (out, rs) if want_rowstat else out


@_guarded
def keymass(score, rowstat, nk, q_batch_shift):
    nb, h, nq, ld = score.shape
    mass = _f32(nb, nk, device=score.device)
    call("vcr_keymass_f32", KeymassArgs(ptr(score), ld, nb, h, nq, nk, ptr(rowstat), q_batch_shift, ptr(mass)))
    return mass


@_guarded
def softcorr(q, k, qside4, kside4, nbatch, nq, nk, mode=0, scale=1.0, split=False):
    corr4 = _f32(nbatch * nq, 4, device=q.device)
    work = _f32(4 * nbatch * nq * 8, device=q.device) if split else None
    call("vcr_softcorr_f32", SoftcorrArgs(ptr(q), q.stride(0), ptr(k), k.stride(0), ptr(qside4), ptr(kside4),
                                          ptr(corr4), nbatch, nq, nk, q.shape[1], mode, scale, ptr(work),
                                          work.numel() if split else 0))
    return corr4


@_guarded
def rigid_svd(src, corr, want_h=False):
    B, K, _ = src.shape
    dev = src.device
    R, t, Rb, tb = _f32(B, 3, 3, device=dev), _f32(B, 3, device=dev), _f32(B, 3, 3, device=dev), _f32(B, 3, device=dev)
    H = _f32(B, 3, 3, device=dev) if want_h else None
    call("vcr_rigid_svd_f32", RigidSvdArgs(ptr(src), src.stride(1), ptr(corr), corr.stride(1), B, K, ptr(R), ptr(t),
                                           ptr(Rb), ptr(tb), ptr(H)))
    return (R, t, Rb, tb, H) if want_h else (R, t, Rb, tb)


@_guarded
def pairscore(own, strm, nbatch, n_own, n_str, op, score=0, scale=1.0, own_side4=None, str_side4=None,
              shift=0, str_stat2=None, str_stat_stride=None, mass=None, accumulate=False, want_argmax=False,
              score_out=None, variant=0, split=False, prefill=None):
    dev = own.device
    corr4 = _f32(nbatch * n_own, 4, device=dev) if op == 0 else None
    stat2 = _f32(nbatch * n_own, 2, device=dev) if op == 1 else None
    amax = _i32(nbatch * n_own, device=dev, prefill=prefill) if (op == 1 and want_argmax) else None
    if op == 2 and mass is None:
        mass = _f32(nbatch, n_own, device=dev)
    work = _f32(4 * nbatch * n_own * (8 if op == 0 else 2), device=dev) if split else None
    call("vcr_pairscore_f32", PairscoreArgs(
        ptr(own), own.stride(0), ptr(strm), strm.stride(0), ptr(own_side4), ptr(str_side4), nbatch, n_own, n_str,
        own.shape[1], score, scale, shift, op, ptr(corr4), ptr(stat2), ptr(amax), ptr(str_stat2),
        int(str_stat_stride if str_stat_stride is not None else n_str * 2), ptr(mass), int(accumulate),
        ptr(score_out), score_out.stride(1) if score_out is not None else 0, variant, ptr(work),
        work.numel() if split else 0))
    if op == 0:
        return corr4
    if op == 1:
        return stat2, amax
    return mass


@_guarded
def scoremass(score, n_cols, row_stat2):
    nb, n_rows, ld = score.shape
    cs, cm, rm = _f32(nb, n_cols, 2, device=score.device), _f32(nb, n_cols, device=score.device), \
        _f32(nb, n_rows, device=score.device)
    call("vcr_scoremass_f32", ScoremassArgs(ptr(score), ld, nb, n_rows, n_cols, ptr(row_stat2), ptr(cs), ptr(cm), ptr(rm)))
    return cs, cm, rm


@_guarded
def make_pairs(cloud, R_ab, t_ab, pick, perm_src, perm_tgt, keep):
    B, P, _ = cloud.shape
    N = pick.shape[1]
    for x, dt in ((cloud, torch.float32), (R_ab, torch.float64), (t_ab, torch.float64), (pick, torch.int32),
                  (perm_src, torch.int32), (perm_tgt, torch.int32)):
        if x.dtype != dt or not x.is_contiguous():
            raise VcrHipError("make_pairs: wrong dtype or non-contiguous argument")
    src, tgt = _f32(B, 3, keep, device=cloud.device), _f32(B, 3, keep, device=cloud.device)
    call("vcr_make_pairs_f32", MakePairsArgs(ptr(cloud), P, ptr(R_ab), ptr(t_ab), ptr(pick), ptr(perm_src),
                                             ptr(perm_tgt), B, N, keep, ptr(src), ptr(tgt)))
    return src, tgt


FPS_FORMS = {"resident": 1, "streaming": 2}


def fps_form(N, npoint=1, B=1, variant=0):
    a = FpsArgs(0x1000, 3 * N, B, N, npoint, None, 0x2000, None, variant)
    form, ppt = C.c_int(0), C.c_int(0)
    check(lib().vcr_fps_form(C.byref(a), C.byref(form), C.byref(ppt)), "vcr_fps_form")
    return form.value, ppt.value


@_guarded
def fps(xyz, npoint, start=None, want_points=True, variant=0, prefill=None):
    if xyz.dim() != 3 or xyz.shape[1] != 3 or xyz.dtype != torch.float32:
        raise VcrHipError(f"fps: xyz must be a [B, 3, N] float32 cloud, got {tuple(xyz.shape)} {xyz.dtype}")
    B, _, N = xyz.shape
    if N >= 1 and not (xyz.stride(2) == 1 and xyz.stride(1) == N and (B == 1 or xyz.stride(0) >= 3 * N)):
        xyz = xyz.contiguous()
    stride = xyz.stride(0) if B > 1 else 3 * N
    idx = _i32(B, int(npoint), device=xyz.device, prefill=prefill)
    pts = _f32(B, 3, int(npoint), device=xyz.device) if want_points else None
    if start is not None:
        start = start.to(device=xyz.device, dtype=torch.int32).contiguous()
        if start.numel() != B:
            raise VcrHipError(f"fps: start must hold one index per cloud ({B}), got {tuple(start.shape)}")
    call("vcr_fps_f32", FpsArgs(ptr(xyz), stride, B, N, int(npoint), ptr(start), ptr(idx), ptr(pts), int(variant)))
    return idx, pts


def farthest_point_sample(xyz, npoint):
    if not xyz.is_cuda:
        raise VcrHipError("farthest_point_sample runs on the HIP path only; move xyz to cuda (there is no CPU fallback)")
    return fps(xyz.float(), npoint, want_points=False)[0].long()


@_guarded
def to_rows4(x_cf):
    B, _, N = x_cf.shape
    x = x_cf.contiguous().float()
    out = _f32(B, N, 4, device=x.device)
    call("vcr_rows4_f32", ptr(x), ptr(out), B, N)
    return out


@_guarded
def rows4_pq(x_cf, wpq, bpq):
    B, _, N = x_cf.shape
    x = x_cf.contiguous().float()
    Cc = wpq.shape[0]
    out, pq = _f32(B, N, 4, device=x.device), _f32(B * N, Cc, device=x.device)
    call("vcr_rows4_pq_f32", ptr(x), ptr(out), B, N, ptr(wpq), wpq.stride(0), ptr(bpq), Cc, ptr(pq), Cc)
    return out, pq


@_guarded
# ... 86 lines not shown
```

### vcr-net_amd/workmodel.py

```python
from __future__ import annotations

from typing import Dict, Tuple

PEAK_MFMA_F32_TFLOPS = 157.3
PEAK_HBM_GBS = 8000.0
PEAK_MFMA_BF16_TFLOPS = 2500.0

FAMILY_BOUND = {"pointwise": "hbm", "knn": "mfma", "linear": "mfma", "edgeconv": "mfma", "gathermax": "hbm",
                "layernorm": "hbm", "sdpa": "mfma", "softcorr": "mfma", "rigid_svd": "hbm",
                "pairscore": "mfma", "scoremass": "hbm", "select": "hbm", "pose": "hbm"}

_LINEAR_SHAPES = {
    "dg1_pq": (256, 64), "sn1_pq": (512, 128), "conv3": ("E", 512),
    "pn_c3": (64, 64), "pn_c4": (128, 64), "pn_c5": ("E", 128),
    "enc.qkv": ("3E", "E"), "enc.wo": ("E", "E"), "enc.ffn1": ("F", "E"), "enc.ffn2": ("E", "F"),
    "dec.qkv": ("3E", "E"), "encdec.qkv": ("6E", "E"), "dec.self.wo": ("E", "E"), "dec.cross.q": ("E", "E"), "dec.cross.kv": ("2E", "E"),
    "dec.cross.wo": ("E", "E"), "dec.ffn1": ("F", "E"), "dec.ffn2": ("E", "F"),
}


def overlap_sizes(N: int, overlap2: float) -> Tuple[int, int, int]:
    k1 = int(N * 0.84 * overlap2)
    return int(N * overlap2), k1, int(k1 * 0.52 * overlap2)


def launch_work(name: str, B: int, N: int, k: int = 20, E: int = 512, F: int = 1024,
                overlap2: float = 0.765970880926229) -> Tuple[float, float]:
    if name.endswith("@src"):
        fl, by = launch_work(name[:-4], B, N, k, E, F, overlap2)
        return 0.5 * fl, 0.5 * by
    fam, site = name.split(":", 1)
    M1, M2 = B * N, 2 * B * N
    sym = {"E": E, "2E": 2 * E, "3E": 3 * E, "6E": 6 * E, "F": F}
    r = lambda v: sym[v] if isinstance(v, str) else v
    if fam == "pointwise":
        if site == "pad":
            return 0.0, 4.0 * M2 * (4 + 32)
        g = 2 if site.startswith("src+tgt") else 1
        if site.endswith("+dg1_pq"):
            return g * 2.0 * M1 * (3 * 64 + 64 * 64 + 64 * 256), g * 4.0 * M1 * (3 + 4 + 64 + 64 + 1 + 256)
        return g * 2.0 * M1 * (3 * 64 + 64 * 64), g * 4.0 * M1 * (3 + 4 + 64 + 1)
    if fam == "knn":
        if site == "feat64+xyz":
            return 2.0 * (64 + 3) * N * N * 2 * B, 4.0 * M2 * (64 + 1 + 4 + 2 * k)
        if site == "ties":
            return 0.0, 4.0 * M2
        if site == "rank":
            return 0.0, 4.0 * M2 * (4 + 2 * (64 + 1 + 4) + 1 + 6)
        C = 64 if site == "feat64" else 3
        return 2.0 * C * N * N * 2 * B, 4.0 * M2 * ((C if C == 64 else 4) + (1 if C == 64 else 0) + k)
    if fam == "linear":
        if site.startswith("dg_c"):
            n, kk, rows = {"dg_c1_pq": (128, 32, M2), "dg_c2": (64, 64, M2 * k), "dg_c3": (128, 64, M2 * k),
                           "dg_c4": (256, 128, M2 * k)}[site]
            out_rows = M2 if site == "dg_c4" else rows
            return 2.0 * rows * n * kk, 4.0 * (rows * kk + n * kk + out_rows * n)
        if site.startswith("head.att"):
            return 2.0 * M1 * E * E, 4.0 * (2 * M1 * E + E * E)
        if "+" in site:
            parts = [launch_work("linear:" + p, B, N, k, E, F, overlap2) for p in site.split("+")]
            return sum(p[0] for p in parts), sum(p[1] for p in parts)
        n, kk = (r(v) for v in _LINEAR_SHAPES[site])
        return 2.0 * M2 * n * kk, 4.0 * (M2 * kk + n * kk + M2 * n)
    if fam == "edgeconv" and site == "dg_chain":
        return 2.0 * M2 * k * (64 * 64 + 128 * 64 + 256 * 128), 4.0 * M2 * (128 + k + 512)
    if fam == "edgeconv":
        return 2.0 * M2 * k * 128 * 128, 4.0 * M2 * (256 + k + 256)
    if fam == "gathermax":
        if site == "dg_c1":
            return 1.0 * M2 * k * 64, 4.0 * M2 * (128 + k + k * 64 + 512)
        if site.startswith("dg_"):
            C = {"dg_max1": 64, "dg_max2": 64, "dg_max3": 128, "dg_max4": 256}[site]
            return 1.0 * M2 * k * C, 4.0 * M2 * (k * C + C)
        return 1.0 * M2 * k * 256, 4.0 * M2 * (512 + k + 256)
    if fam == "layernorm":
        if site.startswith("rowside"):
            return 2.0 * M2 * E, 4.0 * M2 * E * 2
        extra = 1 if site.endswith("+res") else 0
        return 8.0 * M2 * E, 4.0 * M2 * E * (2 + extra)
    keep, K1, K2 = overlap_sizes(N, overlap2)
    if fam == "sdpa":
        if site == "dec.cross.stats":
            return 2.0 * 2 * B * N * N * E, 4.0 * M2 * E * 2
        g = 2 if site == "encdec.self" else 1
        return g * 4.0 * 2 * B * N * N * E, g * 4.0 * M2 * E * 4
    if fam == "pairscore":
        if site == "dec.cross.keymass":
            return 2.0 * 2 * B * N * N * (E // 4), 4.0 * M2 * (E // 4) * 2
        if site == "head.scores":
            return 2.0 * B * N * N * E + 6.0 * B * N * N, 4.0 * (M2 * E + B * N * N)
        if site == "head.copair":
            return 2.0 * B * K1 * K1 * E, 4.0 * 2 * B * K1 * E
        return 2.0 * B * N * N * E, 4.0 * M2 * E
    if fam == "scoremass":
        if site == "dec.cross.keymass":
            return 4.0 * 2 * B * 4 * N * N, 4.0 * 2 * B * 4 * N * N
        return 8.0 * B * N * N, 4.0 * 2 * B * N * N
    if fam == "select":
        if site.endswith(".forced") or site.endswith(".out"):
            return 0.0, 8.0 * 2 * B * N
        if site.startswith("gather"):
            width = E if site.endswith("emb") else 4
            if site in ("gather.emb", "gather.xyz"):
                return 0.0, 4.0 * 2 * 2 * B * K1 * width
            rows = K1 if ("src_" in site or "tgt_" in site) else K2
            return 0.0, 4.0 * 2 * B * rows * width
        n = K1 if site == "head.pairs" else N
        nb = 2 * B if site in ("dec.cross.keys", "head.src+tgt") else B
        return 1.0 * nb * n * n, 4.0 * nb * n * 2
    if fam == "pose":
        return 18.0 * M1, 4.0 * M1 * 6
    if fam == "softcorr":
        return 2.0 * B * N * N * E + 6.0 * B * N * N, 4.0 * (M2 * E + M2 * 4)
    if fam == "rigid_svd":
        return 18.0 * M1, 4.0 * M1 * 8
    raise KeyError(name)


def gather_bytes(name: str, B: int, N: int, k: int = 20) -> float:
    if name.endswith("@src"):
        return 0.5 * gather_bytes(name[:-4], B, N, k)
    fam, site = name.split(":", 1)
    M2 = 2 * B * N
    if fam == "edgeconv":
        return 4.0 * M2 * k * (64 if site == "dg_chain" else 128)
    if fam == "gathermax" and site == "sn1":
        return 4.0 * M2 * k * 256
    if fam == "gathermax" and site == "dg_c1":
        return 4.0 * M2 * k * 64
    return 0.0


def reference_flops_per_pair(N: int, k: int = 20, E: int = 512, F: int = 1024) -> Dict[str, float]:
    emb = 2 * N * (3 * 64 + 64 * 64) + 2 * 64 * N * N + 2 * (2 * 128 * 128 * N * k) + 6 * N * N \
        + 2 * 256 * 256 * N * k + 2 * 512 * 512 * N
    tr = 2 * (3 * (8 * E * E * N + 4 * E * N * N) + 2 * (4 * E * F * N))
    head = 2 * E * N * N + 6 * N * N
    return {"emb": 2.0 * emb, "transformer": float(tr), "head": float(head), "svd": 18.0 * N,
            "total": 2.0 * emb + tr + head + 18.0 * N}
```

Measured before the change: 3215 pairs/s.

## Fuse sn1 pq projection into LDS gathermax kernel and fold small launches

Adds a gathermax kernel that computes the per-cloud pq projection (x·Wpq + b) with MFMA straight into LDS, then does the kNN gather-max from LDS. This removes the separate sn1_pq linear launch and the M×512 pq3 intermediate round trip through global memory. It also folds the ties zeroing into the pointwise stem kernel and the src4 copy into the rigid SVD kernel, removing two small launches. The trade-off is that each workgroup recomputes the projection for its slice of a cloud, and the fused kernel runs at one 512-thread workgroup per CU with a large LDS footprint.

Result: no change. 3222 pairs/s, median of 6 (+0.2%).

```diff
diff --git a/include/vcr_hip.h b/include/vcr_hip.h
--- a/include/vcr_hip.h
+++ b/include/vcr_hip.h
@@ -27,6 +27,7 @@
   const float* x_cf2; int B2;
   const float* pq_w; const float* pq_b; float* pq; int ldpq;
   float* feat64t;
+  int32_t* zero_i32; long zero_n;
 } vcr_pointwise_args;
 int vcr_pointwise_f32(const vcr_pointwise_args*, vcr_stream_t);
 
@@ -122,6 +123,8 @@
   float* y; int ldy;
   int variant;
   const int32_t* order;
+  const float* x; int ldx; int K; const float* wpq; const float* bpq; int pq_variant;
+  int plan_rows;
 } vcr_gathermax_args;
 int vcr_gathermax_f32(const vcr_gathermax_args*, vcr_stream_t);
 
@@ -206,6 +209,7 @@
 typedef struct {
   const float* src; int lds; const float* corr; int ldc; int B, K;
   float* R; float* t; float* R_ba; float* t_ba; float* H;
+  float* src_out;
 } vcr_rigid_svd_args;
 int vcr_rigid_svd_f32(const vcr_rigid_svd_args*, vcr_stream_t);
 
@@ -289,6 +293,7 @@
   int sdpa_variant;
   int iter_reuse;
   int workspace_flat;
+  int sn1_unfused;
 } vcr_vcrnet_weights;
 
 typedef struct {
diff --git a/vcr-net_amd/csrc/edgeconv.hip b/vcr-net_amd/csrc/edgeconv.hip
--- a/vcr-net_amd/csrc/edgeconv.hip
+++ b/vcr-net_amd/csrc/edgeconv.hip
@@ -398,32 +398,137 @@
   }
 }
 
+constexpr size_t GM_LDS_BUDGET_AUTO32 = 150 * 1024;
+constexpr int GM_PQ_K = 128;
+template <int CS, int KQ>
+__global__ __launch_bounds__(512, 1) void gathermax_pq_lds_kernel(vcr_gathermax_args p, int slices) {
+  static_assert(CS == 32, "one 32x32x2 MFMA tile column per slice");
+  constexpr int PITCH = gm_pitch(CS), LPP = CS / 4, PPR = 512 / LPP;
+  constexpr int NI = ((int)(GM_LDS_BUDGET_AUTO32 / (PITCH * 4)) + PPR - 1) / PPR;
+  extern __shared__ __attribute__((aligned(16))) float gm_smem[];
+  const int t = threadIdx.x, lane = t & 63, w = t >> 6;
+  const int half = lane >> 5, l31 = lane & 31;
+  const int lin = xcd_chunk((int)blockIdx.x, (int)gridDim.x);
+  const int cloud = lin / slices, sl = lin - cloud * slices;
+  const int N = p.n_per_cloud, c0 = sl * CS;
+  const size_t base = (size_t)cloud * N;
+  const int sub = t % LPP, c4 = 4 * sub;
+  const float* xc = p.x + base * p.ldx + 4 * half;
+
+  auto project = [&](int wrow0) {
+    f32x4 wf[16];
+#pragma unroll
+    for (int g = 0; g < 16; ++g) wf[g] = ld4(p.wpq + (size_t)(wrow0 + l31) * GM_PQ_K + 8 * g + 4 * half);
+    const float bias = p.bpq ? p.bpq[wrow0 + l31] : 0.f;
+    int r0 = 32 * w;
+    if (r0 >= N) return;
+    const int r_last = r0 + (N - 1 - r0) / 256 * 256;
+    f32x4 af[16];
+    {
+      const float* xr = xc + (size_t)min(r0 + l31, N - 1) * p.ldx;
+#pragma unroll
+      for (int g = 0; g < 16; ++g) af[g] = ld4(xr + 8 * g);
+    }
+    for (; r0 < N; r0 += 32 * 8) {
+      const float* xn = xc + (size_t)min(min(r0 + 32 * 8, r_last) + l31, N - 1) * p.ldx;
+      f32x16 acc = {0};
+#pragma unroll
+      for (int g = 0; g < 16; ++g) {
+#pragma unroll
+        for (int s = 0; s < 4; ++s) acc = mfma32(af[g][s], wf[g][s], acc);
+        af[g] = ld4(xn + 8 * g);
+        __builtin_amdgcn_sched_barrier(0);
+      }
+#pragma unroll
+      for (int r = 0; r < 16; ++r) {
+        const int row = r0 + acc_row(r, half);
+        if (row < N) gm_smem[row * PITCH + l31] = acc[r] + bias;
+      }
+    }
+  };
+
+  project(p.C + c0);
+  __syncthreads();
+  f32x4 qr[NI];
+  const int n0 = t / LPP;
+#pragma unroll
+  for (int i = 0; i < NI; ++i) qr[i] = n0 + i * PPR < N ? ld4(&gm_smem[(n0 + i * PPR) * PITCH + c4]) : f32x4{0.f, 0.f, 0.f, 0.f};
+  __syncthreads();
+  project(c0);
+  __syncthreads();
+
+  using i32x4 = __attribute__((ext_vector_type(4))) int;
+  i32x4 idn[KQ];
+  auto fetch = [&](int n) {
+    const i32x4* id = reinterpret_cast<const i32x4*>(p.idx + (base + n) * (4 * KQ));
+#pragma unroll
+    for (int u = 0; u < KQ; ++u) idn[u] = id[u];
+  };
+  if (n0 < N) fetch(n0);
+#pragma unroll
+  for (int i = 0; i < NI; ++i) {
+    const int n = n0 + i * PPR;
+    if (n >= N) break;
+    i32x4 idc[KQ];
+#pragma unroll
+    for (int u = 0; u < KQ; ++u) idc[u] = idn[u];
+    if (n + PPR < N) fetch(n + PPR);
+    f32x4 m = ld4(&gm_smem[idc[0][0] * PITCH + c4]);
+#pragma unroll
+    for (int u = 0; u < KQ; ++u)
+#pragma unroll
+      for (int e = (u == 0 ? 1 : 0); e < 4; ++e) {
+        const f32x4 a0 = ld4(&gm_smem[idc[u][e] * PITCH + c4]);
+#pragma unroll
+        for (int j = 0; j < 4; ++j) m[j] = fmaxf(m[j], a0[j]);
+        if (KQ > 5 && u == KQ / 2 - 1 && e == 3) __builtin_amdgcn_sched_barrier(0);
+      }
+    f32x4 y;
+#pragma unroll
+    for (int j = 0; j < 4; ++j) y[j] = fmaxf(m[j] + qr[i][j], 0.f);
+    st4(p.y + (base + n) * p.ldy + c0 + c4, y);
+  }
+}
+
 constexpr int EDGECONV_PIPE = 1;
 constexpr int EDGECONV_WG_PER_CU = 2;
 constexpr int EDGECONV_PADDED_MAX_GRID = 2048;
 constexpr int EDGECONV_BF16X3_MAX_GRID = 1024;
 
-constexpr size_t GM_LDS_BUDGET_AUTO32 = 150 * 1024;
 constexpr size_t GM_LDS_MAX = 160 * 1024;
 constexpr int GM_MIN_WORKGROUPS = 192;
 inline size_t gm_lds_bytes(int n_per_cloud, int cs) { return (size_t)n_per_cloud * gm_pitch(cs) * 4; }
 
-enum GathermaxForm { GM_L2, GM_LDS };
+enum GathermaxForm { GM_L2, GM_LDS, GM_LDS_PQ };
 struct GathermaxPlan { GathermaxForm form; int cs, slices; size_t lds; int grid; };
 
 int gathermax_check(const vcr_gathermax_args* a) {
-  if (!a || !a->pq || !a->idx || !a->y) return VCR_EINVAL;
+  if (!a || (!a->pq && !a->x) || !a->idx || !a->y) return VCR_EINVAL;
   if (a->M <= 0 || a->k <= 0 || a->C <= 0 || a->C > 256 || (a->C & 3)) return VCR_EINVAL;
-  if (a->n_per_cloud <= 0 || (a->M % a->n_per_cloud) || a->ldpq < 2 * a->C || (a->ldpq & 3) || (a->ldy & 3)) return VCR_EINVAL;
+  if (a->n_per_cloud <= 0 || (a->M % a->n_per_cloud) || (a->pq && (a->ldpq < 2 * a->C || (a->ldpq & 3))) || (a->ldy & 3)) return VCR_EINVAL;
+  if (a->plan_rows < 0 || (a->plan_rows && (a->plan_rows < a->M || a->plan_rows % a->n_per_cloud))) return VCR_EINVAL;
+  if (a->x && (!a->wpq || a->K <= 0 || (a->K % 32) || a->ldx < a->K || (a->ldx & 3) || (((uintptr_t)a->x | (uintptr_t)a->wpq) & 15) ||
+               ((uintptr_t)a->bpq & 3)))
+    return VCR_EINVAL;
   return VCR_OK;
+}
+
+bool gathermax_pq_shape(const vcr_gathermax_args& a) {
+  if (a.K != GM_PQ_K || (a.C % 32)) return false;
+  float* const y = a.pq ? const_cast<float*>(a.pq) : a.y;
+  vcr_linear_args l{a.x, a.ldx, a.wpq, a.bpq, nullptr, 0, y, a.pq ? a.ldpq : 2 * a.C, a.plan_rows ? a.plan_rows : a.M, 2 * a.C, a.K, 0};
+  l.variant = a.pq_variant;
+  int f[8];
+  return vcr_linear_forms_(&l, nullptr, nullptr, f, nullptr) == VCR_OK && f[3] == 32;
 }
 
 int gathermax_plan(const vcr_gathermax_args& a, GathermaxPlan* p) {
   const int N = a.n_per_cloud, clouds = a.M / N;
+  const int plan_clouds = a.plan_rows ? a.plan_rows / N : clouds;
   const bool aligned = !(((uintptr_t)a.pq | (uintptr_t)a.y | (uintptr_t)a.idx) & 15) && edge_group_points(a.k) != 0;
   int cs = 0;
   if (a.variant == 0) {
-    if (aligned && (long)clouds * ((a.C + 31) / 32) >= GM_MIN_WORKGROUPS)
+    if (aligned && (long)plan_clouds * ((a.C + 31) / 32) >= GM_MIN_WORKGROUPS)
       cs = gm_lds_bytes(N, 32) <= GM_LDS_BUDGET_AUTO32 ? 32 : gm_lds_bytes(N, 16) <= GM_LDS_MAX ? 16 : 0;
   } else if (a.variant == 32 || a.variant == 16 || a.variant == 8) {
     if (!aligned || gm_lds_bytes(N, a.variant) > GM_LDS_MAX) return VCR_EUNSUPPORTED;
@@ -433,12 +538,14 @@
   }
   const int slices = cs ? (a.C + cs - 1) / cs : 0;
   *p = cs ? GathermaxPlan{GM_LDS, cs, slices, gm_lds_bytes(N, cs), clouds * slices} : GathermaxPlan{GM_L2, 0, 0, 0, (a.M + 3) / 4};
+  if (a.x && !a.order && cs == 32 && p->lds <= GM_LDS_BUDGET_AUTO32 && gathermax_pq_shape(a)) p->form = GM_LDS_PQ;
   return VCR_OK;
 }
 
 template <int KQ>
 int gathermax_lds_run(const GathermaxPlan& p, const vcr_gathermax_args& a, hipStream_t s) {
   const dim3 grid(p.grid), block(512);
+  if (p.form == GM_LDS_PQ) return vcr_launch<gathermax_pq_lds_kernel<32, KQ>>(grid, block, p.lds, s, a, p.slices);
   if (p.cs == 32) return vcr_launch<gathermax_lds_kernel<32, KQ>>(grid, block, p.lds, s, a, p.slices);
   if (p.cs == 16) return vcr_launch<gathermax_lds_kernel<16, KQ>>(grid, block, p.lds, s, a, p.slices);
   return vcr_launch<gathermax_lds_kernel<8, KQ>>(grid, block, p.lds, s, a, p.slices);
@@ -481,6 +588,7 @@
   GathermaxPlan p;
   if (const int rc = gathermax_check(a)) return rc;
   if (const int rc = gathermax_plan(*a, &p)) return rc;
+  if (a->x && p.form != GM_LDS_PQ) return VCR_EUNSUPPORTED;
   const hipStream_t s = (hipStream_t)stream;
   if (p.form == GM_L2) return vcr_launch<gathermax_kernel>(dim3(p.grid), dim3(256), 0, s, *a);
   return a->k == 20 ? gathermax_lds_run<5>(p, *a, s) : gathermax_lds_run<10>(p, *a, s);
diff --git a/vcr-net_amd/csrc/forward.hip b/vcr-net_amd/csrc/forward.hip
--- a/vcr-net_amd/csrc/forward.hip
+++ b/vcr-net_amd/csrc/forward.hip
@@ -89,6 +89,22 @@
          W->fold_encdec_qkv.bias;
 }
 
+inline vcr_gathermax_args sn1_fused_args(const vcr_vcrnet_weights* W, const float* x2, const int32_t* idx, float* y, int rows, int N,
+                                         int plan_rows) {
+  vcr_gathermax_args a{nullptr, 0, 256, idx, W->k, rows, N, y, 512};
+  a.x = x2; a.ldx = 512; a.K = 128; a.wpq = W->sn1_wpq; a.bpq = W->sn1_bpq; a.plan_rows = plan_rows;
+  return a;
+}
+inline bool sn1_fused(const vcr_vcrnet_weights* W, int B, int N) {
+  if (W->sn1_unfused || W->emb_kind != 0 || W->linear_mode != 0 || W->linear_mfma || W->linear_bk || W->linear_bm) return false;
+  if (N >= KNN_ORDERED_MIN_N) return false;
+  float* const al = reinterpret_cast<float*>(256);
+  vcr_gathermax_args a = sn1_fused_args(W, al, reinterpret_cast<const int32_t*>(al), al, 2 * B * N, N, 0);
+  if (!a.wpq) a.wpq = al;
+  int form = 0, cs, grid, lds;
+  return vcr_gathermax_forms_(&a, &form, &cs, &grid, &lds) == VCR_OK && form == 2;
+}
+
 Ws carve(void* base, const vcr_vcrnet_weights* W, int B, int N, int cus, int pass = 0) {
   const int k = W->k, E = W->E, F = W->F, heads = W->heads;
   const bool merged = merged_encdec(W) != 0;
@@ -104,7 +120,7 @@
     w.tie_work_each = (w.tie_work_each + 255) & ~(size_t)255;
   }
   pl.want(w.tie_work[0], w.tie_work_each ? 2 * w.tie_work_each : 0, KNN, TIE_REPLAY);
-  pl.want(w.pq1, M * 256, STEM, SN1_PQ);   pl.want(w.cat, M * 512, EDGECONV, CONV3);   pl.want(w.pq3, M * 512, SN1_PQ, GATHERMAX);
+  pl.want(w.pq1, M * 256, STEM, SN1_PQ);   pl.want(w.cat, M * 512, EDGECONV, CONV3);   pl.want(w.pq3, sn1_fused(W, B, N) ? 0 : M * 512, SN1_PQ, GATHERMAX);
   pl.want(w.emb, M * E, STEM, DEC_NORM);
   pl.want(w.qkv, M * 3 * E * (merged ? 2 : 1), merged ? ENCDEC_QKV : ENC_QKV, merged ? ENCDEC_SELF : DEC_SELF);
   pl.want(w.att, M * E * (merged ? 2 : 1), merged ? ENCDEC_SELF : ENC_SELF, merged ? WO_PAIR : DEC_SELF_WO);
@@ -455,8 +471,10 @@
   Runner R{(hipStream_t)stream, tr};
   R.shape_rows = half ? M2 : 0;
   R.plan_nbatch = half ? 2 * B : 0;
-  hipLaunchKernelGGL(zero_i32_kernel, dim3((unsigned)((M2 + 2 + 255) / 256)), dim3(256), 0, R.stream, w.ties, (long)(M2 + 2));
-  R.ok(VCR_LAUNCH_RC());
+  if (W->emb_kind == 1) {
+    hipLaunchKernelGGL(zero_i32_kernel, dim3((unsigned)((M2 + 2 + 255) / 256)), dim3(256), 0, R.stream, w.ties, (long)(M2 + 2));
+    R.ok(VCR_LAUNCH_RC());
+  }
 #define SP(site) (W->linear_mode != 0 ? W->split.site : nullptr)
   R.sdpa_split = W->linear_mode == 2;
   R.sdpa_variant = W->sdpa_variant;
@@ -523,6 +541,7 @@
                          half ? 0 : B};
     if (pq_fused) { a.pq_w = W->dg1_wpq; a.pq_b = W->dg1_bpq; a.pq = w.pq1; a.ldpq = 256; }
     a.feat64t = w.feat64t;
+    a.zero_i32 = w.ties; a.zero_n = (long)M2 + 2;
     return vcr_pointwise_f32(&a, R.stream);
   });
   const int32_t* rank_perm = nullptr;
@@ -554,12 +573,19 @@
     vcr_edgeconv_args a{w.pq1, 256, w.idx1, k, Mq, N, W->dg2_w, W->dg2_b, w.cat, 512, w.cat + 128, 512};
     return W->linear_mode != 0 && edge_group_points(k) ? vcr_edgeconv_bf16x3_f32(&a, R.stream) : vcr_edgeconv_f32(&a, R.stream);
   });
-  R.linear(NM("linear:sn1_pq"), w.cat + 128, 512, W->sn1_wpq, SP(sn1_pq), W->sn1_bpq, w.pq3, 512, Mq, 512, 128, 0);
-  R.run(NM("gathermax:sn1"), [&] {
-    vcr_gathermax_args a{w.pq3, 512, 256, w.idx3, k, Mq, N, w.cat + 256, 512};
-    a.order = rank_perm;
-    return vcr_gathermax_f32(&a, R.stream);
-  });
+  if (sn1_fused(W, B, N)) {
+    R.run(NM("gathermax:sn1+pq"), [&] {
+      const vcr_gathermax_args a = sn1_fused_args(W, w.cat + 128, w.idx3, w.cat + 256, Mq, N, M2);
+      return vcr_gathermax_f32(&a, R.stream);
+    });
+  } else {
+    R.linear(NM("linear:sn1_pq"), w.cat + 128, 512, W->sn1_wpq, SP(sn1_pq), W->sn1_bpq, w.pq3, 512, Mq, 512, 128, 0);
+    R.run(NM("gathermax:sn1"), [&] {
+      vcr_gathermax_args a{w.pq3, 512, 256, w.idx3, k, Mq, N, w.cat + 256, 512};
+      a.order = rank_perm;
+      return vcr_gathermax_f32(&a, R.stream);
+    });
+  }
   R.linear(NM("linear:conv3"), w.cat, 512, W->c3_w, SP(c3), W->c3_b, w.emb, E, Mq, E, 512, 1, nullptr, 0, nullptr, nullptr,
            W->has_pointer == 1 ? w.st_emb : nullptr);
 
@@ -648,10 +674,8 @@
   } else {
     soft_head("softcorr:head", 0, (size_t)M1, io->corr4);
     R.run("rigid_svd:ab", [&] {
-      const int c = vcr_copy_d2d(io->src4, w.xyz4, (size_t)M1 * 4 * sizeof(float), R.stream);
-      vcr_rigid_svd_args a{w.xyz4, 4, io->corr4, 4, B, N, io->R_ab, io->t_ab, io->R_ba, io->t_ba, nullptr};
-      const int s = vcr_rigid_svd_f32(&a, R.stream);
-      return c ? c : s;
+      vcr_rigid_svd_args a{w.xyz4, 4, io->corr4, 4, B, N, io->R_ab, io->t_ab, io->R_ba, io->t_ba, nullptr, io->src4};
+      return vcr_rigid_svd_f32(&a, R.stream);
     });
     if (W->cycle) {
       if (!io->R_ba || !io->t_ba) return VCR_EINVAL;
diff --git a/vcr-net_amd/csrc/pointwise.hip b/vcr-net_amd/csrc/pointwise.hip
--- a/vcr-net_amd/csrc/pointwise.hip
+++ b/vcr-net_amd/csrc/pointwise.hip
@@ -10,6 +10,8 @@
   __shared__ float w1s[64][4];
   __shared__ float b2s[64];
   const int t = threadIdx.x;
+  if (a.zero_i32)
+    for (long i = ((long)blockIdx.y * gridDim.x + blockIdx.x) * 256 + t; i < a.zero_n; i += (long)gridDim.x * gridDim.y * 256) a.zero_i32[i] = 0;
   {
     f32x4 wv[4];
 #pragma unroll
@@ -107,6 +109,8 @@
   float* tiles = pqb + 256;
   const int t = threadIdx.x, lane = t & 63, wave = t >> 6;
   const int q4 = lane >> 4, l15 = lane & 15;
+  if (a.zero_i32)
+    for (long i = (long)blockIdx.x * (64 * PQW) + t; i < a.zero_n; i += (long)gridDim.x * (64 * PQW)) a.zero_i32[i] = 0;
   f32x4 w2c[4][4];
 #pragma unroll
   for (int j = 0; j < 4; ++j)
@@ -314,6 +318,7 @@
   if (!a || !a->x_cf || !a->w1 || !a->b1 || !a->w2 || !a->b2 || !a->xyz4 || !a->feat64 || !a->sq64) return VCR_EINVAL;
   if (((uintptr_t)a->w2 | (uintptr_t)a->pq_w) & 15) return VCR_EINVAL;
   if (a->B <= 0 || a->N <= 0 || a->B2 < 0 || (a->B2 > 0 && !a->x_cf2)) return VCR_EINVAL;
+  if (a->zero_n < 0 || (a->zero_n > 0 && !a->zero_i32)) return VCR_EINVAL;
   if (a->pq) {
     if (!a->pq_w || !a->pq_b || a->ldpq < 256 || (a->ldpq & 3)) return VCR_EINVAL;
     const int tpc = (a->N + 15) / 16, total = tpc * (a->B + a->B2);
diff --git a/vcr-net_amd/csrc/rigid_svd.hip b/vcr-net_amd/csrc/rigid_svd.hip
--- a/vcr-net_amd/csrc/rigid_svd.hip
+++ b/vcr-net_amd/csrc/rigid_svd.hip
@@ -117,6 +117,14 @@
   double mean[6] = {0, 0, 0, 0, 0, 0};
   for (int i = t; i < p.K; i += 256)
     for (int c = 0; c < 3; ++c) { mean[c] += S[(size_t)i * p.lds + c]; mean[3 + c] += C[(size_t)i * p.ldc + c]; }
+  if (p.src_out) {
+    float* O = p.src_out + (size_t)b * p.K * p.lds;
+    if (p.lds == 4 && !(((uintptr_t)p.src | (uintptr_t)p.src_out) & 15)) {
+      for (int i = t; i < p.K; i += 256) st4(O + (size_t)i * 4, ld4(S + (size_t)i * 4));
+    } else {
+      for (long i = t; i < (long)p.K * p.lds; i += 256) O[i] = S[i];
+    }
+  }
   block_sums<6>(mean, red);
   float smf[3], cmf[3];
   for (int c = 0; c < 3; ++c) { smf[c] = (float)(mean[c] / p.K); cmf[c] = (float)(mean[3 + c] / p.K); }
@@ -170,6 +178,7 @@
 
 extern "C" int vcr_rigid_svd_f32(const vcr_rigid_svd_args* a, vcr_stream_t stream) {
   if (!a || !a->src || !a->corr || !a->R || !a->t) return VCR_EINVAL;
+  if (a->src_out == a->src && a->src_out) return VCR_EINVAL;
   if (a->B <= 0 || a->K < 3 || a->lds < 3 || a->ldc < 3) return VCR_EINVAL;
   hipLaunchKernelGGL(rigid_svd_kernel, dim3(a->B), dim3(256), 0, (hipStream_t)stream, *a);
   return VCR_LAUNCH_RC();
diff --git a/vcr-net_amd/module.py b/vcr-net_amd/module.py
--- a/vcr-net_amd/module.py
+++ b/vcr-net_amd/module.py
@@ -229,6 +229,7 @@
         self.sdpa_variant = 0
         self.iter_reuse = True
         self.workspace_flat = False
+        self.sn1_fused = True
         self._packed: Optional[Dict[str, torch.Tensor]] = None
         self._packed_key = None
         self._cw: Optional[native.VcrnetWeights] = None
@@ -276,7 +277,8 @@
         dev = self._device()
         return (dev, ps[0].device, tuple(p._version for p in ps), tuple(p.data_ptr() for p in ps[:4]), self.emb_nn.k,
                 self.linear_mode, self.linear_mfma, self.linear_bk, self.linear_bm, self.knn_waves, self.xscore_limit_mb,
-                self.merge_encdec, bool(self.workspace_flat), int(self.sdpa_variant), bool(self.iter_reuse))
+                self.merge_encdec, bool(self.workspace_flat), int(self.sdpa_variant), bool(self.iter_reuse),
+                bool(self.sn1_fused))
 
     def _pack(self):
         m, sh = self._master()
@@ -415,6 +417,7 @@
         cw.knn_waves = int(self.knn_waves)
         cw.xscore_limit_mb = int(self.xscore_limit_mb)
         cw.workspace_flat = int(bool(self.workspace_flat))
+        cw.sn1_unfused = 0 if self.sn1_fused else 1
         cw.sdpa_variant = int(self.sdpa_variant)
         cw.iter_reuse = 0 if self.iter_reuse else 1
         cw.partial, cw.overlap2 = int(self._partial), self._overlap2
@@ -425,7 +428,8 @@
         sh = self._shared
         key = (B, N, device, int(self.emb_nn.k), int(self.xscore_limit_mb), bool(self.merge_encdec), self.linear_mode,
                self._emb_kind, self._vcp, self._partial, self._overlap2, bool(self.workspace_flat),
-               bool(self.iter_reuse) and iters > 1)
+               bool(self.iter_reuse) and iters > 1,
+               bool(self.sn1_fused))
         with sh.lock:
             idle = sh.pool.get(key)
             if idle:
diff --git a/vcr-net_amd/native.py b/vcr-net_amd/native.py
--- a/vcr-net_amd/native.py
+++ b/vcr-net_amd/native.py
@@ -16,7 +16,8 @@
 class PointwiseArgs(C.Structure):
     _fields_ = [("x_cf", f32p), ("B", C.c_int), ("N", C.c_int), ("w1", f32p), ("b1", f32p), ("w2", f32p),
                 ("b2", f32p), ("xyz4", f32p), ("feat64", f32p), ("sq64", f32p), ("x_cf2", f32p), ("B2", C.c_int),
-                ("pq_w", f32p), ("pq_b", f32p), ("pq", f32p), ("ldpq", C.c_int), ("feat64t", f32p)]
+                ("pq_w", f32p), ("pq_b", f32p), ("pq", f32p), ("ldpq", C.c_int), ("feat64t", f32p),
+                ("zero_i32", f32p), ("zero_n", C.c_long)]
 
 
 class _Sized(C.Structure):
@@ -74,7 +75,9 @@
 
 class GathermaxArgs(C.Structure):
     _fields_ = [("pq", f32p), ("ldpq", C.c_int), ("C", C.c_int), ("idx", f32p), ("k", C.c_int), ("M", C.c_int),
-                ("n_per_cloud", C.c_int), ("y", f32p), ("ldy", C.c_int), ("variant", C.c_int), ("order", f32p)]
+                ("n_per_cloud", C.c_int), ("y", f32p), ("ldy", C.c_int), ("variant", C.c_int), ("order", f32p),
+                ("x", f32p), ("ldx", C.c_int), ("K", C.c_int), ("wpq", f32p), ("bpq", f32p), ("pq_variant", C.c_int),
+                ("plan_rows", C.c_int)]
 
 
 class SdpaArgs(C.Structure):
@@ -148,7 +151,7 @@
 
 class RigidSvdArgs(C.Structure):
     _fields_ = [("src", f32p), ("lds", C.c_int), ("corr", f32p), ("ldc", C.c_int), ("B", C.c_int), ("K", C.c_int),
-                ("R", f32p), ("t", f32p), ("R_ba", f32p), ("t_ba", f32p), ("H", f32p)]
+                ("R", f32p), ("t", f32p), ("R_ba", f32p), ("t_ba", f32p), ("H", f32p), ("src_out", f32p)]
 
 
 class NormW(C.Structure):
@@ -200,7 +203,8 @@
                 ("partial", C.c_int), ("overlap2", C.c_double), ("emb_kind", C.c_int), ("dgcnn", DgcnnW), ("pointnet", PointnetW),
                 ("att_w0", f32p), ("att_b0", f32p), ("att_w1", f32p), ("att_b1", f32p), ("cycle", C.c_int),
                 ("linear_mfma", C.c_int), ("linear_bk", C.c_int), ("linear_bm", C.c_int), ("knn_waves", C.c_int),
-                ("xscore_limit_mb", C.c_int), ("sdpa_variant", C.c_int), ("iter_reuse", C.c_int), ("workspace_flat", C.c_int)]
+                ("xscore_limit_mb", C.c_int), ("sdpa_variant", C.c_int), ("iter_reuse", C.c_int), ("workspace_flat", C.c_int),
+                ("sn1_unfused", C.c_int)]
 
 
 class VcrnetIo(C.Structure):
@@ -603,6 +607,28 @@
     return y
 
 
+def gathermax_pq_args(x, wpq, bpq, idx, n_per_cloud, y, variant=0, pq_variant=0, plan_rows=0):
+    M, K = x.shape
+    Cc = wpq.shape[0] // 2
+    a = GathermaxArgs(None, 0, Cc, ptr(idx), idx.shape[-1], M, n_per_cloud, ptr(y), y.stride(0), variant, None)
+    a.x, a.ldx, a.K, a.wpq, a.bpq, a.pq_variant, a.plan_rows = ptr(x), x.stride(0), K, ptr(wpq), ptr(bpq), pq_variant, plan_rows
+    return a
+
+
+def gathermax_form(a):
+    o = [C.c_int(-1) for _ in range(4)]
+    return (lib().vcr_gathermax_forms_(C.byref(a), *[C.byref(v) for v in o]),) + tuple(v.value for v in o)
+
+
+@_guarded
+def gathermax_pq(x, wpq, bpq, idx, n_per_cloud, variant=0, pq_variant=0, out=None):
+    M = x.shape[0]
+    Cc = wpq.shape[0] // 2
+    y = out if out is not None else _f32(M, Cc, device=x.device)
+    call("vcr_gathermax_f32", gathermax_pq_args(x, wpq, bpq, idx, n_per_cloud, y, variant, pq_variant))
+    return y
+
+
 @_guarded
 def sdpa(q, k, v, nbatch, heads, nq, nk, scale, kv_batch_shift=0, key_keep=None, want_rowstat=False, pv=True,
          score_out=None, bf16x3=False, groups=None, key_index=None, nk_src=0, split=False, variant=0):
diff --git a/vcr-net_amd/workmodel.py b/vcr-net_amd/workmodel.py
--- a/vcr-net_amd/workmodel.py
+++ b/vcr-net_amd/workmodel.py
@@ -72,6 +72,8 @@
         if site.startswith("dg_"):
             C = {"dg_max1": 64, "dg_max2": 64, "dg_max3": 128, "dg_max4": 256}[site]
             return 1.0 * M2 * k * C, 4.0 * M2 * (k * C + C)
+        if site == "sn1+pq":
+            return 2.0 * M2 * 512 * 128 + 1.0 * M2 * k * 256, 4.0 * (M2 * (128 + k + 256) + 512 * 128 + 512)
         return 1.0 * M2 * k * 256, 4.0 * M2 * (512 + k + 256)
     if fam == "layernorm":
         if site.startswith("rowside"):
@@ -124,7 +126,7 @@
     M2 = 2 * B * N
     if fam == "edgeconv":
         return 4.0 * M2 * k * (64 if site == "dg_chain" else 128)
-    if fam == "gathermax" and site == "sn1":
+    if fam == "gathermax" and site in ("sn1", "sn1+pq"):
         return 4.0 * M2 * k * 256
     if fam == "gathermax" and site == "dg_c1":
         return 4.0 * M2 * k * 64
```
